# u2seg/U2Seg

Measured on AMD Instinct MI355X. Metric: training images/sec (whole node) u2seg_R50_800 @ 800x1333, higher is better.
Workload: dtype bf16

## Files before the change

include/u2seg_hip.h:

```cpp
#ifndef U2SEG_HIP_H
#define U2SEG_HIP_H

#ifdef __cplusplus
extern "C" {
#endif



#define U2_CV_REG_STAGING (1u << 0)
#define U2_CV_BK32 (1u << 2)
#define U2_CV_TILE_256X128 (1u << 3)
#define U2_CV_RING_SHIFT 4
#define U2_CV_RING_MASK 3
#define U2_CV_WIDE_FORCE (1u << 8)
#define U2_CV_WIDE_FORBID (1u << 9)
#define U2_CV_WIDE_STAGGER (1u << 10)
#define U2_CV_WIDE_STAGGER_PARITY (1u << 11)
#define U2_CV_TILE_CFG_SHIFT 12
#define U2_CV_TILE_CFG_MASK 15
#define U2_CV_TILE_CFG_NEVER 15
#define U2_CV_TINY_GRID (1u << 16)
#define U2_CV_STREAM_FORCE (1u << 17)
#define U2_CV_HALO_TILE128 (1u << 17)
#define U2_CV_ABL_SHIFT 18
// ... 5 lines not shown
#define U2_CV_ABL_NO_STATS_FLUSH (1u << 22)
#define U2_CV_HALO_FORCE (1u << 24)
#define U2_CV_HALO_FORBID (1u << 25)
#define U2_CV_STREAM_FORBID (1u << 26)
#define U2_CV_STREAMK_FORCE (1u << 27)
#define U2_CV_STREAMK_FORBID (1u << 28)
#define U2_CV_HALO_SCHED_SHIFT 29
#define U2_CV_HALO_SCHED_MASK 3
#define U2_CV_EXPLICIT_MASK 0xffffu

#define U2_WG_REG_STAGING (1u << 0)
#define U2_WG_SCALAR_GATHER (1u << 1)
#define U2_WG_FEWER_SPLITS_SHIFT 4
#define U2_WG_FEWER_SPLITS_MASK 3
#define U2_WG_XCD_FORCE (1u << 6)
#define U2_WG_XCD_FORBID (1u << 7)
#define U2_WG_WIDE_FORCE (1u << 8)
#define U2_WG_WIDE_FORBID (1u << 11)
#define U2_WG_RING_SHIFT 9
#define U2_WG_RING_MASK 3
#define U2_WG_HALO_FORCE (1u << 12)
#define U2_WG_HALO_FORBID (1u << 13)
#define U2_WG_HALO_ROUNDS_SHIFT 14
#define U2_WG_HALO_ROUNDS_MASK 3
#define U2_WG_ATOMICS (1u << 16)
#define U2_WG_PARTIALS_FORCE (1u << 17)
#define U2_WG_STREAM_FORCE (1u << 18)
#define U2_WG_STREAM_FORBID (1u << 19)
#define U2_WG_STREAM_TINY (1u << 20)
#define U2_WG_STREAM_CFG_SHIFT 21
#define U2_WG_STREAM_CFG_MASK 7
#define U2_WG_STREAM_PER_CU_SHIFT 24
#define U2_WG_STREAM_PER_CU_MASK 3
#define U2_WG_PER_TAP_MASK_STREAM 0xfffu
#define U2_WG_PER_TAP_MASK_HALO 0x7ffu

#define U2_WD_FORCE (1u << 0)
#define U2_WD_TINY (1u << 1)
#define U2_WD_NEVER (1u << 2)
#define U2_WD_BN_TWO_GROUPS (1u << 3)
#define U2_WD_BN_WIDE (1u << 4)

#define U2_K_TILE 100
#define U2_K_IGEMM256 256
#define U2_K_IGEMM256_STAGGER 1024
#define U2_K_HALO 300
#define U2_K_HALO_N64 301
#define U2_K_STREAMK 500
#define U2_K_STREAM 700
#define U2_K_STREAM_TAIL 5
#define U2_K_IGEMM 1000000
#define U2_K_WGRAD 2000
#define U2_K_WGRAD_XCD 100
#define U2_K_WGRAD256 2256
#define U2_K_WGRAD_STREAM 2700
#define U2_K_WDGRAD 2750
#define U2_K_WDGRAD_BN 2760
#define U2_K_WGRAD_HALO 2900

int u2_conv_igemm(const void* in, const void* wt, void* out, const float* bias, float* stats,
                  int B, int Hin, int Win, int C, int in_ld, int Hout, int Wout, int N, int out_ld,
                  int KH, int KW, int pad_h, int pad_w, int mul, int div, int relu, int accumulate,
                  int variant, void* stream);

int u2_conv_wgrad(const void* x, const void* dy, float* dw, int B, int Hin, int Win, int C, int x_ld,
                  int Hout, int Wout, int N, int dy_ld, int KH, int KW, int pad_h, int pad_w,
                  int stride, int variant, void* stream);
int u2_conv_wgrad_into(const void* x, const void* dy, float* dw, int B, int Hin, int Win, int C, int x_ld,
                       int Hout, int Wout, int N, int dy_ld, int KH, int KW, int pad_h, int pad_w,
                       int stride, int n_valid, int c_valid, long long dw_stride_n, int dw_stride_tap,
                       int dw_stride_c, int variant, void* stream);

int u2_conv1x1_bwd_fused(const void* x, const void* dy, const void* wt, void* dx, float* dw, int M, int C, int x_ld, int N, int dy_ld,
                         int wt_ld, int dx_ld, int n_valid, int c_valid, long long dw_stride_n, int dw_stride_c, int variant,
                         void* stream);

int u2_conv1x1_bwd_fused_bn(const void* x, const void* dz, const void* y, const float* k1, const float* k2, const float* k3,
                            const void* wt, void* dx, float* dw, int M, int C, int x_ld, int N, int dy_ld, int wt_ld, int dx_ld,
                            int n_valid, int c_valid, long long dw_stride_n, int dw_stride_c, int variant, void* stream);

int u2_conv_dgrad_tail(const void* in, const void* wt, const void* dout2, const void* y, const void* bits, const float* mean,
                       const float* invstd, void* dz, float* sums, int B, int H, int W, int C, int in_ld, int N, int out_ld,
                       int variant, void* stream);

int u2_conv_last_kernel(void);

int u2_release_scratch(void);

int u2_weight_layout(const float* w, void* out, int N, int Cin, int T, int Cp, int Npad, int mode, void* stream);
typedef struct U2LayoutDesc {
  long long src_offset;
  void* dst;
  int N, Cin, T, Cp, Npad, mode;
  int block_begin;
  int reserved;
} U2LayoutDesc;
int u2_weight_layout_batched(const float* base, const U2LayoutDesc* table, int n_entries, int total_blocks, void* stream);

int u2_colstats(const void* x, float* out , int slots, int rows_per_slot, int C, int ld, void* stream);
int u2_colstats_ordered(const void* x, float* part, float* out, int slots, int rows_per_slot, int C, int ld, int nchunk,
                        void* stream);
int u2_colsum_add(const void* x, float* dst, int rows, int C, int ld, int n_valid, void* stream);
int u2_gn_finalize_fwd(const float* stats, const float* gamma, const float* beta, float n, float eps, int B, int C, int groups,
                       float* mean, float* invstd, float* scale, float* shift, void* stream);
int u2_gn_finalize_bwd(const float* sums, const float* gamma, const float* mean, const float* invstd, float n, int B, int C,
                       int groups, float* k1, float* k2, float* k3, float* dgamma, float* dbeta, int accumulate, void* stream);
int u2_bn_finalize_fwd(const float* sums, float count, const float* count_dev, const float* gamma, const float* beta, float* running_mean,
                       float* running_var, float momentum, float eps, float* mean, float* invstd, float* scale,
                       float* shift, int C, void* stream);
int u2_affine_act(const void* x, const float* scale, const float* shift, const void* resid, void* out, int slots,
                  int rows_per_slot, int C, int ld, int relu, void* relu_bits, void* stream);
int u2_affine_upadd(const void* x, const float* scale, const float* shift, const void* top, void* out, int B, int H, int W,
                    int C, int relu, void* stream);
int u2_norm_bwd_reduce(const void* dout, const void* mask, const void* x, const float* mean, const float* invstd,
                       float* out , int slots, int rows_per_slot, int C, int ld, int relu,
                       const float* mask_scale, const float* mask_shift, const void* dout2, void* dz_out, const void* dout3,
                       int mask_is_bits, void* stream);
int u2_bn_finalize_bwd(const float* sums, float count, const float* count_dev, const float* gamma, const float* mean, const float* invstd,
                       const float* local_sums, float* dgamma, float* dbeta, float* k1, float* k2, float* k3, int C,
                       int accumulate , void* stream);
int u2_norm_bwd_apply(const void* dout, const void* mask, const void* x, const float* k1, const float* k2,
                      const float* k3, void* dx, void* dres, int slots, int rows_per_slot, int C, int ld, int relu,
                      const float* mask_scale, const float* mask_shift, void* stream);
int u2_bn_act_fused(const void* x, const float* sums, float count, const float* count_dev, const float* gamma, const float* beta,
                    float* running_mean, float* running_var, float momentum, float eps, float* mean, float* invstd, float* scale,
                    float* shift, const void* resid, void* out, int rows, int C, int ld, int relu, void* relu_bits, void* stream);
int u2_bn_bwd_apply_fused(const float* sums, float count, const float* count_dev, const float* gamma, const float* mean,
                          const float* invstd, const float* local_sums, float* dgamma, float* dbeta, float* k123, int accumulate,
                          const void* dout, const void* mask, const void* x, void* dx, void* dres, int rows, int C, int ld,
                          int relu, const float* mask_scale, const float* mask_shift, void* stream);
typedef struct {
  float* running_mean;
  float* running_var;
  int offset;
  int channels;
  int stride;
  int reserved;
} U2PreciseBnLayer;
int u2_bn_precise_update(const U2PreciseBnLayer* table, int n_layers, double* acc, double* tot, int total_channels, int n, int h,
                         int w, void* stream);
int u2_bn_precise_finalize(const U2PreciseBnLayer* table, int n_layers, const double* acc, const double* tot, int total_channels,
                           void* stream);
int u2_relu_bwd(const void* dout, const void* out, void* dz, long long numel, void* stream);
int u2_relu_bwd_colsum(const void* dout, const void* out, void* dz, float* dst, const float* zeros, int rows, int C, int ld, int n_valid,
                       void* stream);
int u2_add_n(const void* a, const void* b, const void* c, const void* d, void* out, long long numel, void* stream);

int u2_wgrad_permute_add(const float* scratch, float* grad, int N, int Cin, int T, int Cp, void* stream);

int u2_maxpool3x3s2_fwd(const void* x, void* y, void* idx, int B, int H, int W, int C, void* stream);
int u2_maxpool3x3s2_bwd(const void* dy, const void* idx, void* dx, int B, int H, int W, int C, void* stream);
int u2_affine_relu_maxpool_fwd(const void* x, const float* scale, const float* shift, void* y, void* idx, int B, int H, int W,
                               int C, void* stream);
int u2_affine_relu_maxpool_bwd_reduce(const void* dy, const void* idx, const void* x, const float* mean, const float* invstd,
                                      const float* mask_scale, const float* mask_shift, float* sums, int B, int H, int W, int C,
                                      void* stream);
int u2_affine_relu_maxpool_bwd_apply(const void* dy, const void* idx, const void* x, const float* k1, const float* k2,
                                     const float* k3, const float* mask_scale, const float* mask_shift, void* dx, int B, int H, int W,
                                     int C, void* stream);
int u2_fpn_upsample_add_fwd(const void* lateral, const void* top, void* out, int B, int H, int W, int C, void* stream);
int u2_fpn_upsample_add_bwd(const void* dout, void* dtop, int B, int H, int W, int C, void* stream);
int u2_bilinear_up2_fwd(const void* x, const void* addend , void* out, int B, int H,
                        int W, int C, void* stream);
int u2_bilinear_up2_bwd(const void* dout, void* dx, int B, int H, int W, int C, void* stream);
int u2_stem_im2col(const void* img, int is_uint8, const float* mean, const float* stdv, void* col, int b, int h, int w,
                   int Hpad, int Wpad, int KP, void* stream);
// ... 266 lines not shown
```

u2seg_amd/csrc/common.h:

```cpp
#pragma once
#include <hip/hip_runtime.h>
#include <stdint.h>
#include <atomic>
#include <mutex>

typedef uint16_t bf16_t;
typedef __attribute__((ext_vector_type(8))) short s16x8;
typedef __attribute__((ext_vector_type(4))) short s16x4;
typedef __attribute__((ext_vector_type(4))) float f32x4;

struct PerDeviceOnce {
  std::mutex mu;
  std::atomic<bool> done[64];
  PerDeviceOnce() { for (auto& d : done) d.store(false, std::memory_order_relaxed); }
  struct Guard {
    PerDeviceOnce* o; int d;
    Guard(PerDeviceOnce* o_, int d_) : o(o_), d(d_) {}
    Guard(const Guard&) = delete;
    Guard& operator=(const Guard&) = delete;
    explicit operator bool() const { return o != nullptr; }
    ~Guard() {
      if (!o) return;
      if (d >= 0) o->done[d].store(true, std::memory_order_release);
      o->mu.unlock();
// ... 41 lines not shown
}
__device__ __forceinline__ int wave_isum(int v) {
#pragma unroll
  for (int o = 32; o > 0; o >>= 1) v += __shfl_xor(v, o, 64);
  return v;
}
__device__ __forceinline__ int wave_imin(int v) {
#pragma unroll
  for (int o = 32; o > 0; o >>= 1) v = min(v, __shfl_xor(v, o, 64));
  return v;
}
__device__ __forceinline__ int wave_imax(int v) {
#pragma unroll
  for (int o = 32; o > 0; o >>= 1) v = max(v, __shfl_xor(v, o, 64));
  return v;
}

template <int CTRL> __device__ __forceinline__ float dpp_mov(float v) {
  return __int_as_float(__builtin_amdgcn_update_dpp(0, __float_as_int(v), CTRL, 0xf, 0xf, true));
}
__device__ __forceinline__ float row16_transpose_sum(float (&v)[16], int fr) {
  {
    const bool up = fr & 8;
#pragma unroll
    for (int k = 0; k < 8; ++k) {
      const float keep = up ? v[k + 8] : v[k], send = up ? v[k] : v[k + 8];
      v[k] = keep + dpp_mov<0x128>(send);
    }
  }
  {
    const bool up = fr & 4;
#pragma unroll
    for (int k = 0; k < 4; ++k) {
      const float keep = up ? v[k + 4] : v[k], send = up ? v[k] : v[k + 4];
      v[k] = keep + dpp_mov<0x141>(send);
    }
  }
  {
    const bool up = fr & 2;
#pragma unroll
    for (int k = 0; k < 2; ++k) {
      const float keep = up ? v[k + 2] : v[k], send = up ? v[k] : v[k + 2];
      v[k] = keep + dpp_mov<0x4E>(send);
    }
  }
  const bool up = fr & 1;
  const float keep = up ? v[1] : v[0], send = up ? v[0] : v[1];
  return keep + dpp_mov<0xB1>(send);
}

__device__ __forceinline__ float block_sum_256(float v, float* red) {
  v = wave_sum(v);
  __syncthreads();
  if ((threadIdx.x & 63) == 0) red[threadIdx.x >> 6] = v;
  __syncthreads();
  return red[0] + red[1] + red[2] + red[3];
}

template <int NW>
__device__ __forceinline__ void wg_flush_column_sums(float* stats, int N, int st_n, float st_s, float st_ss, int w, int lane,
                                                     unsigned char* smem) {
  __syncthreads();
  int* rn = reinterpret_cast<int*>(smem);
  float* rs = reinterpret_cast<float*>(smem) + NW * 64;
  float* rq = rs + NW * 64;
  rn[w * 64 + lane] = st_n;
  rs[w * 64 + lane] = st_s;
  rq[w * 64 + lane] = st_ss;
  __syncthreads();
  bool lead = st_n >= 0 && st_n < N;
  float s = 0.f, q = 0.f;
#pragma unroll
  for (int k = 0; k < NW; ++k) {
    const bool same = rn[k * 64 + lane] == st_n;
    if (same && k < w) lead = false;
    s += same ? rs[k * 64 + lane] : 0.f;
    q += same ? rq[k * 64 + lane] : 0.f;
  }
  if (lead) {
    atomicAdd(stats + st_n, s);
    atomicAdd(stats + N + st_n, q);
  }
}


__device__ __forceinline__ int xcd_remap(int bid, int nwg) {
  const int q = nwg >> 3, r = nwg & 7;
  const int xcd = bid & 7, idx = bid >> 3;
  const int base = (xcd < r) ? xcd * (q + 1) : r * (q + 1) + (xcd - r) * q;
  return base + idx;
}

struct BilinearTap {
  int i0, i1;
  float h, l;
};
__device__ __forceinline__ BilinearTap bilinear_tap(float scale, int o, int n_in) {
  const float s = fmaxf(scale * ((float)o + 0.5f) - 0.5f, 0.f);
  BilinearTap t;
  t.i0 = min((int)s, n_in - 1);
  t.i1 = t.i0 + (t.i0 < n_in - 1 ? 1 : 0);
  t.l = s - (float)t.i0;
  t.h = 1.f - t.l;
  return t;
}
__device__ __forceinline__ float bilinear_mix(const BilinearTap& y, const BilinearTap& x, float v00, float v01, float v10, float v11) {
  return y.h * (x.h * v00 + x.l * v01) + y.l * (x.h * v10 + x.l * v11);
}

#define U2_CHECK_LAUNCH() do { hipError_t e__ = hipGetLastError(); if (e__ != hipSuccess) return (int)e__; } while (0)

__global__ static void u2_fill_words_kernel(unsigned* __restrict__ p, size_t n, unsigned v) {
  for (size_t i = (size_t)blockIdx.x * blockDim.x + threadIdx.x; i < n; i += (size_t)gridDim.x * blockDim.x) p[i] = v;
}
static inline void u2_fill_words(void* p, size_t nwords, unsigned v, hipStream_t s) {
  if (nwords == 0) return;
  size_t g = (nwords + 255) / 256;
  if (g > 1024) g = 1024;
  hipLaunchKernelGGL(u2_fill_words_kernel, dim3((unsigned)g), dim3(256), 0, s, (unsigned*)p, nwords, v);
}
static inline void u2_zero_words(void* p, size_t nwords, hipStream_t s) { u2_fill_words(p, nwords, 0u, s); }
```

u2seg_amd/csrc/conv_args.h:

```cpp
#pragma once
#include "common.h"
#include "conv_variant.h"

namespace u2conv {

struct ConvArgs {
  const bf16_t* in;
  const bf16_t* wt;
  bf16_t* out;
  const float* bias;
  float* stats;
  const bf16_t* zero;
  int B, Hin, Win, C, in_ld;
  int Hout, Wout, N, out_ld;
  int mul;
  int relu, accumulate;
  int M, tiles_m, tiles_n;
  int ntaps, wt_taps;
  int KW, pad_h, pad_w;
  short tap_dy[64], tap_dx[64], tap_w[64];
  int tap_pk[64];
  int remap_out, Hfull, Wfull, out_sy, out_sx, out_y0, out_x0;
  int stagger_by_parity;
  float* sk_ws;
  int* sk_flags;
  int abl;
};


template <int BK> __device__ __forceinline__ int swz(int row);
template <> __device__ __forceinline__ int swz<64>(int row) { return row & 7; }
template <> __device__ __forceinline__ int swz<32>(int row) { return (-(row >> 2)) & 3; }

__device__ __forceinline__ void glds16(const bf16_t* src, void* lds_dst_wave_base) {
  __builtin_amdgcn_global_load_lds(U2_GLB_PTR(src), U2_LDS_PTR(lds_dst_wave_base), 16, 0, 0);
}

template <int RB> __device__ __forceinline__ int tr_swz(int pix) {
  if constexpr (RB >= 256) return ((pix & 3) << 1) | (pix & 8);
  else if constexpr (RB == 128) return (((pix >> 1) & 1) | (((pix >> 3) & 1) << 1)) << 1;
  else return ((pix >> 3) & 1) << 1;
}

template <int IMM = 0> __device__ __forceinline__ unsigned long long tr_read(unsigned addr) {
  unsigned long long r;
  asm volatile("ds_read_b64_tr_b16 %0, %1 offset:%2" : "=v"(r) : "v"(addr), "n"(IMM) : "memory");
  return r;
}
union Frag {
  unsigned long long u[2];
  s16x8 v;
};

extern int g_last_conv_kernel;

int launch_conv_tile(ConvArgs& a, int N, int C, const ConvVariant& v, hipStream_t s);

int launch_conv_halo(ConvArgs& a, int N, int C, const ConvVariant& v, hipStream_t s);

int launch_conv_stream(ConvArgs& a, int N, int C, const ConvVariant& v, hipStream_t s);

struct TailArgs {
  const bf16_t* g2 = nullptr;
  const bf16_t* y = nullptr;
  const unsigned char* bits = nullptr;
  const float* mean = nullptr;
  const float* invstd = nullptr;
};
int launch_conv_stream_tail(ConvArgs& a, const TailArgs& t, int N, int C, const ConvVariant& v, hipStream_t s);

int launch_wgrad_halo(const bf16_t* x, const bf16_t* dy, float* dw, long long dw_sn, int dw_st, int dw_sc, int n_valid,
                      int c_valid, const bf16_t* zero, int B, int H, int W, int C, int x_ld, int N, int dy_ld, int rounds,
                      int force, int part_mode, hipStream_t s);

int launch_wgrad_stream(const bf16_t* x, const bf16_t* dy, float* dw, long long dw_sn, int dw_sc, int n_valid, int c_valid,
                        const bf16_t* zero, int M, int C, int x_ld, int N, int dy_ld, int force, int tiny, int cfg, int per_cu,
                        hipStream_t s);

int launch_wdgrad_stream(const bf16_t* x, const bf16_t* dy, const bf16_t* wt, bf16_t* dx, float* dw, long long dw_sn, int dw_sc,
                         int n_valid, int c_valid, const bf16_t* zero, int M, int C, int x_ld, int N, int dy_ld, int wt_ld,
                         int dx_ld, const FusedBwdVariant& v, hipStream_t s, const bf16_t* yn = nullptr, const float* k1 = nullptr,
                         const float* k2 = nullptr, const float* k3 = nullptr);

void* scratch_get(int kind, hipStream_t s, size_t need_bytes, size_t limit_bytes, bool zero_on_alloc);

}
```

u2seg_amd/csrc/conv_halo.hip:

```cpp
#include <stdlib.h>
#include <type_traits>

#include "common.h"
#include "conv_args.h"

namespace u2conv {
namespace {

constexpr int HBUF = 49152;
constexpr int HPIECES = 6;
constexpr int WR = 7, WA = WR - 1;
constexpr int TN = 128, WSLOT = TN * 64;
constexpr int WBASE = 2 * HBUF;
constexpr int LDS_BYTES = WBASE + WR * WSLOT;

template <int PH, int PWD, int OPT = 3, int CW = 2>
__global__ __launch_bounds__(512, 2) void conv_halo_kernel(const ConvArgs a) {
  constexpr int HPITCH = PWD + 4;
  constexpr int FPR = PWD / 16;
  constexpr int PXW = 8 / CW;
  constexpr int RPW = PH / PXW;
  constexpr int NPF = RPW * FPR;
  constexpr int TNC = CW * 64;
  static_assert(PH * PWD == 512 && (PH + 2) * HPITCH <= 768 && RPW * PXW == PH && (NPF == 8 || NPF == 4), "unsupported patch");
// ... 228 lines not shown
      const int hd = (slab_g & 1) ? -HBUF : HBUF;                                                                        \
      pbase[0] += hd; pbase[1] += hd; pbase[2] += hd;                                                                    \
    }                                                                                                                    \
    if (g + 1 < G) {                                                                                                     \
      wfA[0] = ldw(nslot, 0); wfA[1] = ldw(nslot, 1);                                                                    \
      _Pragma("unroll") for (int j = 0; j < NPF / 2; ++j) pf[j] = U2_H_LDP(((T) + 1) % 9, j);                            \
    }                                                                                                                    \
    if constexpr (!(OPT & 2)) __builtin_amdgcn_sched_barrier(0);                                                                                   \
    if constexpr (!(OPT & 1)) __builtin_amdgcn_s_setprio(1);                                                                                       \
    _Pragma("unroll") for (int j = NPF / 2; j < NPF; ++j) { U2_H_MFMA(2, wfB[0], j); U2_H_MFMA(3, wfB[1], j); }          \
    if constexpr (!(OPT & 1)) __builtin_amdgcn_s_setprio(0);                                                                                       \
    ++g;                                                                                                                 \
    slot = nslot;                                                                                                        \
  }

  for (int ti = 0; ti < my_tiles; ++ti) {
#pragma unroll
    for (int i = 0; i < 4; ++i)
#pragma unroll
      for (int j = 0; j < NPF; ++j) acc[i][j] = f32x4{0.f, 0.f, 0.f, 0.f};
    for (int s = 0; s < nslab; ++s) {
      tail = slab_g + 2 >= total_slabs;
      U2_H_STEP(0, 7)
      U2_H_STEP(1, 7)
      U2_H_STEP(2, 8)
      U2_H_STEP(3, 9)
      U2_H_STEP(4, 10)
      U2_H_STEP(5, 10)
      U2_H_STEP(6, 9)
      U2_H_STEP(7, 8)
      U2_H_STEP(8, 4)
      ++slab_g;
    }
    epilogue(first_tile + ti * stride);
  }
  if (a.stats) wg_flush_column_sums<8>(a.stats, a.N, st_base < 0 ? -1 : st_base + fg * 8 + (fr >> 3) * 32 + (fr & 7), st_s, st_ss, w, lane, smem);
#undef U2_H_STEP
#undef U2_H_LDP
#undef U2_H_MFMA
}

template <int PH, int PWD, int OPT = 3, int CW = 2>
int launch_halo_cfg(ConvArgs& a, int N, int tiny, hipStream_t s) {
  const long long patches = (long long)a.B * ((a.Hout + PH - 1) / PH) * ((a.Wout + PWD - 1) / PWD);
  a.tiles_m = (int)patches;
  a.tiles_n = (N + CW * 64 - 1) / (CW * 64);
  const long long T = patches * a.tiles_n;
  if (T >= (1 << 30)) return 0;
  long long G = T < (tiny ? 8 : 256) ? T : (tiny ? 8 : 256);
  G = (G + 7) & ~7LL;
  static PerDeviceOnce attr_set;
  if (auto once_guard = attr_set.first()) {
    (void)hipFuncSetAttribute((const void*)conv_halo_kernel<PH, PWD, OPT, CW>, hipFuncAttributeMaxDynamicSharedMemorySize, 160 * 1024);
  }
  hipLaunchKernelGGL((conv_halo_kernel<PH, PWD, OPT, CW>), dim3((unsigned)G), dim3(512), LDS_BYTES, s, a);
  hipError_t e = hipGetLastError();
  if (e != hipSuccess) return -1000 - (int)e;
  return 1;
}

double patch_fill(int H, int W, int ph, int pw) {
  return (double)H * W / ((double)((H + ph - 1) / ph * ph) * ((W + pw - 1) / pw * pw));
}

}

int launch_conv_halo(ConvArgs& a, int N, int C, const ConvVariant& v, hipStream_t s) {
  if (v.halo == Choice::Never) return 0;
  if (v.tile_cfg != 0) return 0;
  const bool forced = v.halo == Choice::Force;
  if (a.remap_out || a.accumulate || a.ntaps != 9 || a.KW != 3 || a.wt_taps != 9 || a.pad_h != 1 || a.pad_w != 1 || a.mul != 1 ||
      a.Hin != a.Hout || a.Win != a.Wout)
    return 0;
  if ((C & 31) || (N & 7) || (a.out_ld & 7) || a.M < 1) return 0;
  if ((unsigned long long)a.B * a.Hin * a.Win * a.in_ld * 2ull >= 0xffffffffull || (unsigned long long)N * 9 * C * 2ull >= 0xfffffff0ull)
    return 0;
  const double fill = patch_fill(a.Hout, a.Wout, 16, 32);
  if (!forced) {
    const int tnc = N <= 64 ? 64 : TN;
    const long long tiles = (long long)a.B * ((a.Hout + 15) / 16) * ((a.Wout + 31) / 32) * ((N + tnc - 1) / tnc);
    if (tiles < 512) return 0;
    if (!(fill >= 0.88 || (N <= 128 && fill >= 0.70))) return 0;
  }
  const int tiny = v.tiny;
  if (N <= 64 && !v.halo_tile128) {
    g_last_conv_kernel = U2_K_HALO_N64;
    return launch_halo_cfg<16, 32, 3, 1>(a, N, tiny, s);
  }
  g_last_conv_kernel = U2_K_HALO;
  switch (v.halo_sched) {
    case 1: return launch_halo_cfg<16, 32, 2>(a, N, tiny, s);
    case 2: return launch_halo_cfg<16, 32, 1>(a, N, tiny, s);
    case 3: return launch_halo_cfg<16, 32, 0>(a, N, tiny, s);
    default: return launch_halo_cfg<16, 32, 3>(a, N, tiny, s);
  }
}

}
```

u2seg_amd/csrc/conv_igemm.hip:

```cpp
#include <stdlib.h>
#include <mutex>
#include <vector>

#include "common.h"
#include "conv_args.h"
#include "u2seg_hip.h"

using namespace u2conv;
namespace {

template <int BK, bool GLDS, int TM, int TN, int NST>
__global__ __launch_bounds__((TM / 64) * (TN / 64) * 64, 2) void conv_igemm_kernel(const ConvArgs a) {
  constexpr int NW = (TM / 64) * (TN / 64);
  constexpr int NT = NW * 64;
  constexpr int CPR = BK / 8;
  constexpr int NCHP = (TM * CPR) / NT;
  constexpr int NCHW = (TN * CPR) / NT;
  static_assert(NCHP >= 1 && NCHW >= 1, "tile too small for the thread count");
  constexpr int ROWS_PER_WAVE_INSTR = 64 / CPR;
  constexpr int PTILE_BYTES = TM * BK * 2;
  constexpr int WTILE_BYTES = TN * BK * 2;
  constexpr int STAGE_BYTES = PTILE_BYTES + WTILE_BYTES;
  constexpr int OPITCH = TN + 8;
  constexpr int WM = TM / 64;
  extern __shared__ __attribute__((aligned(16))) unsigned char smem[];

  const int tid = threadIdx.x;
  const int lane = tid & 63;
  const int w = __builtin_amdgcn_readfirstlane(tid >> 6);
  const int nwg = a.tiles_m * a.tiles_n;
  const int tile = xcd_remap(blockIdx.x, nwg);
  const int tile_m = tile / a.tiles_n;
  const int tile_n = tile - tile_m * a.tiles_n;
  const int m0 = tile_m * TM;
  const int n0 = tile_n * TN;

  int p_img[NCHP], p_by[NCHP], p_bx[NCHP];
  bool p_ok[NCHP];
  const bf16_t* w_row[NCHW];
  int cc;
  {
    const int row_in_instr = lane / CPR;
    const int slot = lane % CPR;
    cc = slot ^ swz<BK>(row_in_instr);
    const int hw = a.Hout * a.Wout;
#pragma unroll
    for (int i = 0; i < NCHP; ++i) {
      const int row = (i * NW + w) * ROWS_PER_WAVE_INSTR + row_in_instr;
      const int m = m0 + row;
      p_ok[i] = m < a.M;
      const int mm = p_ok[i] ? m : 0;
      const int img = mm / hw;
      const int rem = mm - img * hw;
      const int oy = rem / a.Wout;
      const int ox = rem - oy * a.Wout;
      p_img[i] = img;
      p_by[i] = oy * a.mul;
      p_bx[i] = ox * a.mul;
    }
#pragma unroll
    for (int i = 0; i < NCHW; ++i) {
      const int n = n0 + (i * NW + w) * ROWS_PER_WAVE_INSTR + row_in_instr;
      w_row[i] = (n < a.N) ? a.wt + (size_t)n * ((size_t)a.wt_taps * a.C) + cc * 8 : nullptr;
    }
  }

  const int kc_per_tap = a.C / BK;
  const int nk = a.ntaps * kc_per_tap;

  uint4 stage_regs[GLDS ? 1 : NCHP + NCHW];

  const bf16_t* p_src[NCHP];
  int p_inc[NCHP];
  const bf16_t* w_src[NCHW];
#pragma unroll
  for (int i = 0; i < NCHW; ++i) w_src[i] = w_row[i] ? w_row[i] : a.zero;
  int kc_in_tap = 0, tap_cur = 0, reg_kh = 0, reg_kw = 0;

  auto issue = [&](int kt, int buf) {
    (void)kt;
    if (kc_in_tap == 0) {
      int dy, dx, wtap;
      if (a.remap_out) {
        dy = a.tap_dy[tap_cur]; dx = a.tap_dx[tap_cur]; wtap = a.tap_w[tap_cur];
      } else {
        dy = reg_kh - a.pad_h; dx = reg_kw - a.pad_w; wtap = tap_cur;
        if (++reg_kw == a.KW) { reg_kw = 0; ++reg_kh; }
      }
#pragma unroll
      for (int i = 0; i < NCHP; ++i) {
        const int sy = p_by[i] + dy, sx = p_bx[i] + dx;
        const bool ok = p_ok[i] && sy >= 0 && sx >= 0 && sy < a.Hin && sx < a.Win;
        p_src[i] = ok ? a.in + ((size_t)(p_img[i] * a.Hin + sy) * a.Win + sx) * a.in_ld + cc * 8 : a.zero;
        p_inc[i] = ok ? BK : 0;
// ... 83 lines not shown
    for (int kt = 0; kt < nk; ++kt) {
      issue(kt, 0);
      __syncthreads();
      commit(0);
      __syncthreads();
      compute(0);
    }
  }

  __syncthreads();
  bf16_t* otile = reinterpret_cast<bf16_t*>(smem);
  float* red = reinterpret_cast<float*>(smem + TM * OPITCH * 2);
#pragma unroll
  for (int i = 0; i < 4; ++i) {
    const int nl = wr * 64 + i * 16 + fg * 4;
    float b0 = 0.f, b1 = 0.f, b2 = 0.f, b3 = 0.f;
    if (a.bias) {
      const int n = n0 + nl;
      b0 = (n + 0 < a.N) ? a.bias[n + 0] : 0.f;
      b1 = (n + 1 < a.N) ? a.bias[n + 1] : 0.f;
      b2 = (n + 2 < a.N) ? a.bias[n + 2] : 0.f;
      b3 = (n + 3 < a.N) ? a.bias[n + 3] : 0.f;
    }
#pragma unroll
    for (int j = 0; j < 4; ++j) {
      const int ml = wc * 64 + j * 16 + fr;
      float v0 = acc[i][j][0] + b0, v1 = acc[i][j][1] + b1, v2 = acc[i][j][2] + b2, v3 = acc[i][j][3] + b3;
      if (a.relu && !a.accumulate) {
        v0 = fmaxf(v0, 0.f); v1 = fmaxf(v1, 0.f); v2 = fmaxf(v2, 0.f); v3 = fmaxf(v3, 0.f);
      }
      uint2 pk;
      pk.x = (uint32_t)f2bf(v0) | ((uint32_t)f2bf(v1) << 16);
      pk.y = (uint32_t)f2bf(v2) | ((uint32_t)f2bf(v3) << 16);
      *reinterpret_cast<uint2*>(otile + ml * OPITCH + nl) = pk;
    }
  }
  __syncthreads();

  constexpr int CPO = TN / 8;
  constexpr int RPI = NT / CPO;
  const int cchunk = tid % CPO;
  const int rbase = tid / CPO;
  float s[8], ss[8];
#pragma unroll
  for (int e = 0; e < 8; ++e) { s[e] = 0.f; ss[e] = 0.f; }
  const bool vec_ok = ((a.out_ld & 7) == 0) && (n0 + cchunk * 8 + 8 <= a.N);
  const bool nt_out = !a.accumulate && (size_t)a.M * a.out_ld * 2 > ((size_t)160 << 20) && (a.abl & 8);
#pragma unroll
  for (int it = 0; it < TM / RPI; ++it) {
    const int row = it * RPI + rbase;
    const int m = m0 + row;
    if (m >= a.M) continue;
    uint4 v = *reinterpret_cast<const uint4*>(otile + row * OPITCH + cchunk * 8);
    bf16_t e8[8];
    *reinterpret_cast<uint4*>(e8) = v;
    size_t orow = (size_t)m;
    if (a.remap_out) {
      const int hw = a.Hout * a.Wout;
      const int img = m / hw;
      const int rem = m - img * hw;
      const int qy = rem / a.Wout;
      const int qx = rem - qy * a.Wout;
      orow = ((size_t)img * a.Hfull + qy * a.out_sy + a.out_y0) * a.Wfull + qx * a.out_sx + a.out_x0;
    }
    bf16_t* dst = a.out + orow * a.out_ld + n0 + cchunk * 8;
    if (a.accumulate) {
#pragma unroll
      for (int e = 0; e < 8; ++e) {
        if (n0 + cchunk * 8 + e < a.N) {
          float f = bf2f(e8[e]) + bf2f(dst[e]);
          if (a.relu) f = fmaxf(f, 0.f);
          e8[e] = f2bf(f);
        }
      }
    }
    if (a.stats) {
#pragma unroll
      for (int e = 0; e < 8; ++e) {
        const float f = bf2f(e8[e]);
        s[e] += f;
        ss[e] += f * f;
      }
    }
    if (vec_ok) {
      if (nt_out) {
        typedef __attribute__((ext_vector_type(4))) unsigned int u32x4_t;
        const uint4 v = *reinterpret_cast<const uint4*>(e8);
        u32x4_t t = {v.x, v.y, v.z, v.w};
        __builtin_nontemporal_store(t, reinterpret_cast<u32x4_t*>(dst));
      } else {
        *reinterpret_cast<uint4*>(dst) = *reinterpret_cast<const uint4*>(e8);
      }
    } else {
#pragma unroll
      for (int e = 0; e < 8; ++e)
        if (n0 + cchunk * 8 + e < a.N) dst[e] = e8[e];
    }
  }
  if (a.stats) {
#pragma unroll
    for (int e = 0; e < 8; ++e) {
#pragma unroll
      for (int o = CPO; o < 64; o <<= 1) {
        s[e] += __shfl_xor(s[e], o, 64);
        ss[e] += __shfl_xor(ss[e], o, 64);
      }
    }
    if (lane < CPO) {
#pragma unroll
      for (int e = 0; e < 8; ++e) {
        red[(0 * NW + w) * TN + lane * 8 + e] = s[e];
        red[(1 * NW + w) * TN + lane * 8 + e] = ss[e];
      }
    }
    __syncthreads();
    if (tid < TN && n0 + tid < a.N) {
      float t0 = 0.f, t1 = 0.f;
#pragma unroll
      for (int ww = 0; ww < NW; ++ww) {
        t0 += red[(0 * NW + ww) * TN + tid];
        t1 += red[(1 * NW + ww) * TN + tid];
      }
      atomicAdd(a.stats + n0 + tid, t0);
      atomicAdd(a.stats + a.N + n0 + tid, t1);
    }
  }
}

constexpr int C256_THREADS = 512;
constexpr int C256_HALF_BYTES = 256 * 64;
constexpr int C256_BUF_BYTES = 2 * C256_HALF_BYTES;
constexpr int C256_OPITCH = 256 + 8;
constexpr int C256_LDS_BYTES = 256 * C256_OPITCH * 2 + 2 * 8 * 256 * 4;
static_assert(C256_LDS_BYTES >= 4 * C256_BUF_BYTES, "ring must fit in the epilogue allocation");

template <bool STAGGER>
__global__ __launch_bounds__(C256_THREADS, 2) void conv_igemm256_kernel(const ConvArgs a) {
  extern __shared__ __attribute__((aligned(16))) unsigned char smem[];
  const int tid = threadIdx.x;
  const int lane = tid & 63;
  const int w = __builtin_amdgcn_readfirstlane(tid >> 6);
  const int nwg = a.tiles_m * a.tiles_n;
  const int tile = xcd_remap(blockIdx.x, nwg);
  const int tile_m = tile / a.tiles_n;
  const int tile_n = tile - tile_m * a.tiles_n;
  const int m0 = tile_m * 256;
  const int n0 = tile_n * 256;

  int p_img[2], p_by[2], p_bx[2];
  bool p_ok[2];
  const bf16_t* w_src[2];
  int w_inc[2];
  const int row_in = lane >> 2;
  const int cc = (lane & 3) ^ swz<32>(row_in);
  {
    const int hw = a.Hout * a.Wout;
#pragma unroll
    for (int i = 0; i < 2; ++i) {
      const int row = (i * 8 + w) * 16 + row_in;
      const int m = m0 + row;
      p_ok[i] = m < a.M;
      const int mm = p_ok[i] ? m : 0;
      const int img = mm / hw;
      const int rem = mm - img * hw;
      const int oy = rem / a.Wout;
      p_img[i] = img;
      p_by[i] = oy * a.mul;
      p_bx[i] = (rem - oy * a.Wout) * a.mul;
      const int n = n0 + row;
      w_src[i] = (n < a.N) ? a.wt + (size_t)n * ((size_t)a.wt_taps * a.C) + cc * 8 : a.zero;
      w_inc[i] = (n < a.N) ? 32 : 0;
    }
  }
  const int kh_per_tap = a.C >> 5;
  const int nkh = a.ntaps * kh_per_tap;
  const bf16_t* p_src[2];
  int p_inc[2];
  int kc_in_tap = 0, reg_kh = 0, reg_kw = 0;
  auto stage_pixels = [&](int hb) {
    if (kc_in_tap == 0) {
      const int dy = reg_kh - a.pad_h, dx = reg_kw - a.pad_w;
      if (++reg_kw == a.KW) { reg_kw = 0; ++reg_kh; }
#pragma unroll
      for (int i = 0; i < 2; ++i) {
        const int sy = p_by[i] + dy, sx = p_bx[i] + dx;
        const bool ok = p_ok[i] && sy >= 0 && sx >= 0 && sy < a.Hin && sx < a.Win;
        p_src[i] = ok ? a.in + ((size_t)(p_img[i] * a.Hin + sy) * a.Win + sx) * a.in_ld + cc * 8 : a.zero;
        p_inc[i] = ok ? 32 : 0;
      }
    }
    if (++kc_in_tap == kh_per_tap) kc_in_tap = 0;
    unsigned char* pbase = smem + hb * C256_BUF_BYTES;
#pragma unroll
    for (int i = 0; i < 2; ++i) {
      glds16(p_src[i], pbase + (i * 8 + w) * 1024);
      p_src[i] += p_inc[i];
    }
  };
  auto stage_weights = [&](int hb) {
    unsigned char* wbase = smem + hb * C256_BUF_BYTES + C256_HALF_BYTES;
#pragma unroll
    for (int i = 0; i < 2; ++i) {
      glds16(w_src[i], wbase + (i * 8 + w) * 1024);
      w_src[i] += w_inc[i];
    }
  };

// ... 699 lines not shown
int g_scratch_used = 0;
std::mutex g_scratch_mu;
struct RetiredEnt { int device; void* buf; };
std::vector<RetiredEnt> g_retired;
}

void* scratch_get(int kind, hipStream_t s, size_t need_bytes, size_t limit_bytes, bool zero_on_alloc) {
  if (need_bytes == 0 || need_bytes > limit_bytes) return nullptr;
  int dev = 0;
  if (hipGetDevice(&dev) != hipSuccess) return nullptr;
  std::lock_guard<std::mutex> lock(g_scratch_mu);
  ScratchEnt* e = nullptr;
  for (int i = 0; i < g_scratch_used; ++i)
    if (g_scratch[i].device == dev && g_scratch[i].stream == s && g_scratch[i].kind == kind) { e = &g_scratch[i]; break; }
  if (e && e->cap >= need_bytes) return e->buf;
  if (!e) {
    if (g_scratch_used == 128) return nullptr;
    e = &g_scratch[g_scratch_used];
    *e = ScratchEnt{dev, s, kind, nullptr, 0};
  }
  size_t cap = need_bytes > e->cap + e->cap / 2 ? need_bytes : e->cap + e->cap / 2;
  cap = (cap + ((size_t)2 << 20) - 1) & ~(((size_t)2 << 20) - 1);
  if (cap > limit_bytes) cap = limit_bytes;
  if (e->buf) {
    g_retired.push_back(RetiredEnt{dev, e->buf});
    e->buf = nullptr; e->cap = 0;
  }
  void* p = nullptr;
  if (hipMalloc(&p, cap) != hipSuccess) return nullptr;
  if (zero_on_alloc && hipMemset(p, 0, cap) != hipSuccess) { (void)hipFree(p); return nullptr; }
  e->buf = p; e->cap = cap;
  if (e == &g_scratch[g_scratch_used]) ++g_scratch_used;
  return p;
}
}

extern "C" int u2_release_scratch(void) {
  int cur = 0;
  (void)hipGetDevice(&cur);
  std::lock_guard<std::mutex> lock(u2conv::g_scratch_mu);
  int freed = 0;
  for (int i = 0; i < u2conv::g_scratch_used; ++i) {
    u2conv::ScratchEnt& e = u2conv::g_scratch[i];
    if (!e.buf) continue;
    (void)hipSetDevice(e.device);
    (void)hipStreamSynchronize(e.stream);
    (void)hipFree(e.buf);
    ++freed;
  }
  u2conv::g_scratch_used = 0;
  for (const u2conv::RetiredEnt& r : u2conv::g_retired) {
    (void)hipSetDevice(r.device);
    (void)hipDeviceSynchronize();
    (void)hipFree(r.buf);
    ++freed;
  }
  u2conv::g_retired.clear();
  (void)hipSetDevice(cur);
  return freed;
}
extern "C" int u2_conv_last_kernel(void) { return u2conv::g_last_conv_kernel; }
namespace {

const bf16_t* zero_page_ptr() {
  static const bf16_t* p = nullptr;
  if (!p) {
    void* q = nullptr;
    if (hipGetSymbolAddress(&q, HIP_SYMBOL(g_zero_page)) != hipSuccess) return nullptr;
    p = reinterpret_cast<const bf16_t*>(q);
  }
  return p;
}

}

namespace {

int env_variant(const char* name, int variant) {
  if (variant != 0) return variant;
  const char* e = getenv(name);
  return e ? (int)strtol(e, nullptr, 0) : 0;
}

int launch_conv(ConvArgs& a, int N, int C, int variant, hipStream_t s) {
  const ConvVariant v = decode_conv_variant((unsigned)env_variant("U2_CONV_VARIANT", variant));
  a.abl = v.abl;
  {
    const int rc = launch_conv_stream(a, N, C, v, s);
    if (rc == 1) return 0;
    if (rc < 0) return rc;
  }
  {
    const int rc = launch_conv_halo(a, N, C, v, s);
    if (rc == 1) return 0;
    if (rc < 0) return rc;
  }
  {
    const int rc = launch_conv_tile(a, N, C, v, s);
    if (rc == 1) return 0;
    if (rc < 0) return rc;
  }
  const bool wide_ok = !a.remap_out && C % 64 == 0 && a.ntaps * (C / 32) >= 4;
  const bool wide_auto = N % 256 == 0 && a.ntaps * C >= 1024 && (long long)a.M * N >= 256LL * 256 * 512;
  if (wide_ok && v.wide != Choice::Never && (v.wide == Choice::Force || wide_auto)) {
    a.tiles_m = (a.M + 255) / 256;
    a.tiles_n = (N + 255) / 256;
    static PerDeviceOnce attr_set;
    if (auto once_guard = attr_set.first()) {
      (void)hipFuncSetAttribute((const void*)conv_igemm256_kernel<false>, hipFuncAttributeMaxDynamicSharedMemorySize, 160 * 1024);
      (void)hipFuncSetAttribute((const void*)conv_igemm256_kernel<true>, hipFuncAttributeMaxDynamicSharedMemorySize, 160 * 1024);
    }
    a.stagger_by_parity = v.wide_stagger_parity ? 1 : 0;
    g_last_conv_kernel = U2_K_IGEMM256 + (v.wide_stagger ? U2_K_IGEMM256_STAGGER : 0);
    if (v.wide_stagger)
      hipLaunchKernelGGL(conv_igemm256_kernel<true>, dim3(a.tiles_m * a.tiles_n), dim3(C256_THREADS), C256_LDS_BYTES, s, a);
    else
      hipLaunchKernelGGL(conv_igemm256_kernel<false>, dim3(a.tiles_m * a.tiles_n), dim3(C256_THREADS), C256_LDS_BYTES, s, a);
    U2_CHECK_LAUNCH();
    return 0;
  }
  const bool narrow = N <= 64;
  const bool big = !narrow && v.tile_256x128;
  const int TM = (narrow || big) ? 256 : 128, TN = narrow ? 64 : 128;
  a.tiles_m = (a.M + TM - 1) / TM;
  a.tiles_n = (N + TN - 1) / TN;
  const dim3 grid(a.tiles_m * a.tiles_n), block(big ? 512 : 256);
  const bool glds = !v.reg_staging;
  const bool shallow = (long long)a.ntaps * C <= 256;
  const int bk = (C % 64 == 0 && !v.bk32 && !shallow) ? 64 : 32;
  int nst = v.ring;
  if (nst == 0) nst = (bk == 64 || shallow) ? 2 : 4;
  else nst += 1;
  if (!glds) nst = 2;
  size_t lds = (size_t)nst * (TM + TN) * bk * 2;
  const size_t epi = (size_t)TM * (TN + 8) * 2 + 2 * 8 * TN * 4;
  if (lds < epi) lds = epi;
  if (lds > 160 * 1024) return -3;
#define U2_LAUNCH_CONV(BK_, GL_, TM_, TN_, NST_)                                                                 \
  do {                                                                                                           \
    g_last_conv_kernel = U2_K_IGEMM + BK_ * 10000 + (TM_ / 64) * 1000 + (TN_ / 64) * 100 + NST_ * 10 + (GL_ ? 1 : 0); \
    static PerDeviceOnce attr_set;                                                                                \
    if (auto once_guard = attr_set.first()) {                                                                                             \
      (void)hipFuncSetAttribute((const void*)conv_igemm_kernel<BK_, GL_, TM_, TN_, NST_>,                        \
                                hipFuncAttributeMaxDynamicSharedMemorySize, 160 * 1024);                         \
    }                                                                                                            \
    hipLaunchKernelGGL((conv_igemm_kernel<BK_, GL_, TM_, TN_, NST_>), grid, block, lds, s, a);                   \
  } while (0)
#define U2_PICK_NST(BK_, TM_, TN_)                                                                               \
  do {                                                                                                           \
    if (!glds) U2_LAUNCH_CONV(BK_, false, TM_, TN_, 2);                                                          \
    else if (nst == 2) U2_LAUNCH_CONV(BK_, true, TM_, TN_, 2);                                                   \
    else if (nst == 3) U2_LAUNCH_CONV(BK_, true, TM_, TN_, 3);                                                   \
    else U2_LAUNCH_CONV(BK_, true, TM_, TN_, 4);                                                                 \
  } while (0)
  if (narrow) {
    if (bk == 64) U2_PICK_NST(64, 256, 64); else U2_PICK_NST(32, 256, 64);
  } else if (big) {
    if (bk == 64) U2_PICK_NST(64, 256, 128); else U2_PICK_NST(32, 256, 128);
  } else {
    if (bk == 64) U2_PICK_NST(64, 128, 128); else U2_PICK_NST(32, 128, 128);
  }
#undef U2_PICK_NST
#undef U2_LAUNCH_CONV
  U2_CHECK_LAUNCH();
  return 0;
}

inline int floor_div(int a, int b) { return (a >= 0) ? a / b : -((-a + b - 1) / b); }

__global__ __launch_bounds__(256) void parity_zero_fill_kernel(bf16_t* __restrict__ out, long long pixels, int H, int W, int ld, int chunks,
                                                               int div, unsigned classes) {
  const long long total = pixels * chunks;
  for (long long i = (long long)blockIdx.x * 256 + threadIdx.x; i < total; i += (long long)gridDim.x * 256) {
    const long long p = i / chunks;
    const int c = (int)(i - p * chunks);
    const int x = (int)(p % W), y = (int)((p / W) % H);
    if ((classes >> ((y % div) * div + (x % div))) & 1u)
      *reinterpret_cast<uint4*>(out + (size_t)p * ld + c * 8) = make_uint4(0u, 0u, 0u, 0u);
  }
}

}

extern "C" int u2_conv_igemm(const void* in, const void* wt, void* out, const float* bias, float* stats,
                             int B, int Hin, int Win, int C, int in_ld, int Hout, int Wout, int N, int out_ld,
                             int KH, int KW, int pad_h, int pad_w, int mul, int div, int relu, int accumulate,
                             int variant, void* stream) {
  if (C % 32 != 0 || (in_ld & 7) != 0 || KH * KW > 64 || (div > 1 && mul != 1)) return -1;
  if (B <= 0 || Hout <= 0 || Wout <= 0 || N <= 0) return 0;
  ConvArgs a;
  a.in = (const bf16_t*)in; a.wt = (const bf16_t*)wt; a.out = (bf16_t*)out; a.bias = bias; a.stats = stats;
  a.zero = zero_page_ptr();
  if (!a.zero) return -2;
  a.abl = 0; a.stagger_by_parity = 0; a.sk_ws = nullptr; a.sk_flags = nullptr;
  a.B = B; a.Hin = Hin; a.Win = Win; a.C = C; a.in_ld = in_ld;
  a.N = N; a.out_ld = out_ld; a.mul = mul; a.relu = relu; a.accumulate = accumulate;
  a.wt_taps = KH * KW;
  a.KW = KW; a.pad_h = pad_h; a.pad_w = pad_w;
  a.Hfull = Hout; a.Wfull = Wout;
  hipStream_t s = (hipStream_t)stream;
  if (div <= 1) {
    a.Hout = Hout; a.Wout = Wout; a.M = B * Hout * Wout;
    a.ntaps = KH * KW;
    for (int kh = 0; kh < KH; ++kh)
      for (int kw = 0; kw < KW; ++kw) {
        const int t = kh * KW + kw;
        a.tap_dy[t] = (short)(kh - pad_h); a.tap_dx[t] = (short)(kw - pad_w); a.tap_w[t] = (short)t;
        a.tap_pk[t] = ((kh - pad_h) & 0xff) | (((kw - pad_w) & 0xff) << 8) | (t << 16);
      }
    a.remap_out = 0; a.out_sy = a.out_sx = 1; a.out_y0 = a.out_x0 = 0;
    return launch_conv(a, N, C, variant, s);
  }
  unsigned empty = 0;
  if (!bias && !stats && !accumulate && div * div <= 32 && (N & 7) == 0) {
    for (int py = 0; py < div; ++py)
      for (int px = 0; px < div; ++px) {
        bool any = false;
        for (int kh = 0; kh < KH && !any; ++kh)
          for (int kw = 0; kw < KW && !any; ++kw)
            any = ((((py - pad_h + kh) % div) + div) % div) == 0 && ((((px - pad_w + kw) % div) + div) % div) == 0;
        if (!any && py < Hout && px < Wout) empty |= 1u << (py * div + px);
      }
    if (empty) {
      const long long pixels = (long long)B * Hout * Wout;
      long long g = (pixels * (N / 8) + 255) / 256;
      if (g > 256 * 32) g = 256 * 32;
      hipLaunchKernelGGL(parity_zero_fill_kernel, dim3((unsigned)g), dim3(256), 0, s, a.out, pixels, Hout, Wout, out_ld, N / 8, div, empty);
      U2_CHECK_LAUNCH();
    }
  }
  for (int py = 0; py < div; ++py)
    for (int px = 0; px < div; ++px) {
      if ((empty >> (py * div + px)) & 1u) continue;
      const int Hq = (Hout - py + div - 1) / div, Wq = (Wout - px + div - 1) / div;
      if (Hq <= 0 || Wq <= 0) continue;
      int nt = 0;
      for (int kh = 0; kh < KH; ++kh) {
        const int vy = py - pad_h + kh;
        if (((vy % div) + div) % div) continue;
        for (int kw = 0; kw < KW; ++kw) {
          const int vx = px - pad_w + kw;
          if (((vx % div) + div) % div) continue;
          a.tap_dy[nt] = (short)floor_div(vy, div); a.tap_dx[nt] = (short)floor_div(vx, div);
          a.tap_w[nt] = (short)(kh * KW + kw);
          a.tap_pk[nt] = (a.tap_dy[nt] & 0xff) | ((a.tap_dx[nt] & 0xff) << 8) | ((kh * KW + kw) << 16);
          ++nt;
        }
      }
      a.ntaps = nt;
      a.Hout = Hq; a.Wout = Wq; a.M = B * Hq * Wq;
      a.remap_out = 1; a.out_sy = a.out_sx = div; a.out_y0 = py; a.out_x0 = px;
      const int rc = launch_conv(a, N, C, variant, s);
      if (rc) return rc;
    }
  return 0;
}

extern "C" int u2_conv_dgrad_tail(const void* in, const void* wt, const void* dout2, const void* y, const void* bits,
                                  const float* mean, const float* invstd, void* dz, float* sums, int B, int H, int W, int C,
                                  int in_ld, int N, int out_ld, int variant, void* stream) {
  if (B <= 0 || H <= 0 || W <= 0 || N <= 0 || C <= 0) return 1;
  ConvArgs a;
  a.in = (const bf16_t*)in; a.wt = (const bf16_t*)wt; a.out = (bf16_t*)dz; a.bias = nullptr; a.stats = sums;
  a.zero = zero_page_ptr();
  if (!a.zero) return -2;
  a.abl = 0; a.stagger_by_parity = 0; a.sk_ws = nullptr; a.sk_flags = nullptr;
  a.B = B; a.Hin = H; a.Win = W; a.C = C; a.in_ld = in_ld;
  a.N = N; a.out_ld = out_ld; a.mul = 1; a.relu = 0; a.accumulate = 0;
  a.wt_taps = 1; a.ntaps = 1;
  a.KW = 1; a.pad_h = 0; a.pad_w = 0;
  a.Hfull = H; a.Wfull = W; a.Hout = H; a.Wout = W; a.M = B * H * W;
  a.tap_dy[0] = a.tap_dx[0] = a.tap_w[0] = 0; a.tap_pk[0] = 0;
  a.remap_out = 0; a.out_sy = a.out_sx = 1; a.out_y0 = a.out_x0 = 0;
  TailArgs t;
  t.g2 = (const bf16_t*)dout2; t.y = (const bf16_t*)y; t.bits = (const unsigned char*)bits; t.mean = mean; t.invstd = invstd;
  const int rc = launch_conv_stream_tail(a, t, N, C, decode_conv_variant((unsigned)env_variant("U2_CONV_VARIANT", variant)),
                                         (hipStream_t)stream);
  if (rc == 1) return 0;
  return rc < 0 ? rc : 1;
}

extern "C" int u2_conv1x1_bwd_fused(const void* x, const void* dy, const void* wt, void* dx, float* dw, int M, int C, int x_ld,
                                    int N, int dy_ld, int wt_ld, int dx_ld, int n_valid, int c_valid, long long dw_stride_n,
                                    int dw_stride_c, int variant, void* stream) {
  if (n_valid > N || c_valid > C) return -1;
  const bf16_t* zero = zero_page_ptr();
  if (!zero) return -2;
  if (M <= 0) return 0;
  const FusedBwdVariant v = decode_fused_bwd_variant((unsigned)env_variant("U2_WDGRAD_VARIANT", variant));
  if (v.never) return 1;
  const int rc = launch_wdgrad_stream((const bf16_t*)x, (const bf16_t*)dy, (const bf16_t*)wt, (bf16_t*)dx, dw, dw_stride_n,
                                      dw_stride_c, n_valid, c_valid, zero, M, C, x_ld, N, dy_ld, wt_ld, dx_ld, v,
                                      (hipStream_t)stream);
  if (rc == 1) return 0;
  return rc < 0 ? rc : 1;
}

extern "C" int u2_conv1x1_bwd_fused_bn(const void* x, const void* dz, const void* y, const float* k1, const float* k2,
                                       const float* k3, const void* wt, void* dx, float* dw, int M, int C, int x_ld, int N, int dy_ld,
                                       int wt_ld, int dx_ld, int n_valid, int c_valid, long long dw_stride_n, int dw_stride_c,
                                       int variant, void* stream) {
  if (n_valid > N || c_valid > C || !y || !k1 || !k2 || !k3) return -1;
  const bf16_t* zero = zero_page_ptr();
  if (!zero) return -2;
  if (M <= 0) return 0;
  const FusedBwdVariant v = decode_fused_bwd_variant((unsigned)env_variant("U2_WDGRAD_VARIANT", variant));
  if (v.never) return 1;
  const int rc = launch_wdgrad_stream((const bf16_t*)x, (const bf16_t*)dz, (const bf16_t*)wt, (bf16_t*)dx, dw, dw_stride_n,
                                      dw_stride_c, n_valid, c_valid, zero, M, C, x_ld, N, dy_ld, wt_ld, dx_ld, v,
                                      (hipStream_t)stream, (const bf16_t*)y, k1, k2, k3);
  if (rc == 1) return 0;
  return rc < 0 ? rc : 1;
}

extern "C" int u2_conv_wgrad(const void* x, const void* dy, float* dw, int B, int Hin, int Win, int C, int x_ld,
                             int Hout, int Wout, int N, int dy_ld, int KH, int KW, int pad_h, int pad_w,
                             int stride, int variant, void* stream) {
  return u2_conv_wgrad_into(x, dy, dw, B, Hin, Win, C, x_ld, Hout, Wout, N, dy_ld, KH, KW, pad_h, pad_w, stride, N, C,
                            (long long)KH * KW * C, C, 1, variant, stream);
}

extern "C" int u2_conv_wgrad_into(const void* x, const void* dy, float* dw, int B, int Hin, int Win, int C, int x_ld,
                                  int Hout, int Wout, int N, int dy_ld, int KH, int KW, int pad_h, int pad_w,
                                  int stride, int n_valid, int c_valid, long long dw_stride_n, int dw_stride_tap,
                                  int dw_stride_c, int variant, void* stream) {
  if ((C & 7) != 0 || (x_ld & 7) != 0 || (dy_ld & 7) != 0 || (N & 7) != 0) return -1;
  if (n_valid > N || c_valid > C) return -1;
  if (B <= 0 || Hout <= 0 || Wout <= 0) return 0;
  WgradArgs a;
  a.x = (const bf16_t*)x; a.dy = (const bf16_t*)dy; a.dw = dw; a.zero = zero_page_ptr();
  if (!a.zero) return -2;
  a.dw_sn = dw_stride_n; a.dw_st = dw_stride_tap; a.dw_sc = dw_stride_c; a.n_valid = n_valid; a.c_valid = c_valid;
  a.B = B; a.Hin = Hin; a.Win = Win; a.C = C; a.x_ld = x_ld;
  a.Hout = Hout; a.Wout = Wout; a.N = N; a.dy_ld = dy_ld;
  a.KH = KH; a.KW = KW; a.pad_h = pad_h; a.pad_w = pad_w; a.stride = stride;
  a.M = B * Hout * Wout;
  const WgradVariant v = decode_wgrad_variant((unsigned)env_variant("U2_WGRAD_VARIANT", variant));
  if (KH * KW == 1 && stride == 1 && pad_h == 0 && pad_w == 0 && Hin == Hout && Win == Wout && v.stream != Choice::Never &&
      !v.per_tap_stream) {
    const int rc = launch_wgrad_stream(a.x, a.dy, dw, dw_stride_n, dw_stride_c, n_valid, c_valid, a.zero, a.M, C, x_ld, N, dy_ld,
                                       v.stream == Choice::Force, v.stream_tiny, v.stream_cfg, v.stream_per_cu,
                                       (hipStream_t)stream);
    if (rc == 1) return 0;
    if (rc < 0) return rc;
  }
  const bool halo_ok = KH == 3 && KW == 3 && stride == 1 && pad_h == 1 && pad_w == 1 && Hin == Hout && Win == Wout;
// ... 75 lines not shown
```

u2seg_amd/csrc/conv_stream.hip:

```cpp
#include <stdlib.h>

#include "common.h"
#include "conv_args.h"

namespace u2conv {
namespace {

template <int RB> __device__ __forceinline__ int row_swz(int row) {
  if constexpr (RB == 64) return swz<32>(row);
  else if constexpr (RB == 128) return (row >> 1) & 7;
  else return row & 15;
}

template <int NF, int RB, int J = 0> __device__ __forceinline__ void lds_read_frags(s16x8 (&pf)[NF], unsigned addr) {
  if constexpr (J < NF) {
    asm volatile("ds_read_b128 %0, %1 offset:%2" : "=v"(pf[J]) : "v"(addr), "n"(J * 16 * RB) : "memory");
    lds_read_frags<NF, RB, J + 1>(pf, addr);
  }
}
template <int CNT, int NF> __device__ __forceinline__ void lds_wait_frags(s16x8 (&pf)[NF]) {
  asm volatile("s_waitcnt lgkmcnt(%0)" ::"n"(CNT) : "memory");
#pragma unroll
  for (int j = 0; j < NF; ++j) asm volatile("" : "+v"(pf[j])::"memory");
}

template <int E> __device__ __forceinline__ float row_bcast(float v) {
  return __int_as_float(__builtin_amdgcn_update_dpp(0, __float_as_int(v), 0x150 + E, 0xf, 0xf, true));
}

__device__ __forceinline__ f32x2_t row_bcast_pair(float v, int e) {
  switch (e) {
    case 0: return f32x2_t{row_bcast<0>(v), row_bcast<1>(v)};
    case 1: return f32x2_t{row_bcast<2>(v), row_bcast<3>(v)};
    case 2: return f32x2_t{row_bcast<4>(v), row_bcast<5>(v)};
    case 3: return f32x2_t{row_bcast<6>(v), row_bcast<7>(v)};
    case 4: return f32x2_t{row_bcast<8>(v), row_bcast<9>(v)};
    case 5: return f32x2_t{row_bcast<10>(v), row_bcast<11>(v)};
    case 6: return f32x2_t{row_bcast<12>(v), row_bcast<13>(v)};
    default: return f32x2_t{row_bcast<14>(v), row_bcast<15>(v)};
  }
}

typedef __attribute__((ext_vector_type(4))) unsigned int u32x4_t;
typedef __attribute__((ext_vector_type(2))) unsigned int u32x2_t;
struct TailRow {
  u32x4_t ga, gb, ya, yb;
  u32x2_t mk;
};

template <int KS, int TM, int PSW, int NWV, int KSS = KS, bool TAIL = false>
__global__ __launch_bounds__(NWV * 64, 2) void conv_stream_kernel(const ConvArgs a, int ring, const TailArgs t) {
  constexpr int RB = KSS * 64, CPR = KSS * 4, STAGE = TM * RB;
  constexpr int RPP = 16 / KSS;
  constexpr int PT = TM * KSS / 16;
  constexpr int PPW = PT / NWV;
  constexpr int S = KS / KSS;
  constexpr int CBW = NWV / PSW, WPX = TM / PSW, NF = WPX / 16;
  static_assert(PT % NWV == 0 && PPW >= 1 && PPW <= 8 && NF >= 1 && (KSS == 1 || KSS == 2 || KSS == 4 || KSS == 8) && KS % KSS == 0 && (S & (S - 1)) == 0, "unsupported configuration");
  static_assert(!TAIL || (S == 1 && NF % 2 == 0), "the tail epilogue takes whole tiles per step and batches of 1, 2 or 4 rows");
  extern __shared__ __attribute__((aligned(16))) unsigned char smem[];
  const int tid = threadIdx.x, lane = tid & 63;
  const int w = __builtin_amdgcn_readfirstlane(tid >> 6);
  const int cbw = w % CBW, psw = w / CBW;
  const int fr = lane & 15, fg = lane >> 4;

  const int TP = a.tiles_m, tiles_n = a.tiles_n;
  const int xcd = blockIdx.x & 7, idx = blockIdx.x >> 3, gx = gridDim.x >> 3;
  const int q8 = TP >> 3, r8 = TP & 7;
  const int xbase = (xcd < r8) ? xcd * (q8 + 1) : r8 * (q8 + 1) + (xcd - r8) * q8;
  const int xcnt = q8 + (xcd < r8 ? 1 : 0);
  const int nwalk = gx / tiles_n;
  const int nt = idx % tiles_n, walker = idx / tiles_n;
  if (walker >= nwalk || walker >= xcnt) return;
  const int my_tiles = (xcnt - walker + nwalk - 1) / nwalk;
  const int first_tile = xbase + walker;
  const int n0 = nt * (CBW * 64) + cbw * 64;

  s16x8 wr[KS][4];
#pragma unroll
  for (int i = 0; i < 4; ++i) {
    const int n = n0 + (i >> 1) * 32 + (fr >> 2) * 8 + (i & 1) * 4 + (fr & 3);
    const bf16_t* src = a.wt + (size_t)(n < a.N ? n : 0) * a.C + fg * 8;
#pragma unroll
    for (int ks = 0; ks < KS; ++ks) {
      s16x8 v = *reinterpret_cast<const s16x8*>(src + ks * 32);
      if (n >= a.N) v = s16x8{0, 0, 0, 0, 0, 0, 0, 0};
      wr[ks][i] = v;
    }
  }
  float t_mu = 0.f, t_is = 0.f;
  if constexpr (TAIL) {
    const int tn = n0 + fg * 8 + (fr >> 3) * 32 + (fr & 7);
    t_mu = t.mean[tn];
    t_is = t.invstd[tn];
  }
  asm volatile("s_waitcnt vmcnt(0)" ::: "memory");
  if constexpr (TAIL) asm volatile("" : "+v"(t_mu), "+v"(t_is));
#pragma unroll
  for (int ks = 0; ks < KS; ++ks)
#pragma unroll
    for (int i = 0; i < 4; ++i) asm volatile("" : "+v"(wr[ks][i]));

  unsigned d_off[PPW];
  int d_row[PPW];
#pragma unroll
  for (int q = 0; q < PPW; ++q) {
    const int row = (q * NWV + w) * RPP + lane / CPR;
    const int pos = lane % CPR;
    const int chunk = (pos & ~15) | ((pos ^ row_swz<RB>(row)) & (CPR < 16 ? CPR - 1 : 15));
    d_row[q] = row;
    d_off[q] = (unsigned)(((size_t)row * a.in_ld + chunk * 8) * 2);
  }
  const unsigned char* in_bytes = reinterpret_cast<const unsigned char*>(a.in);
  auto issue = [&](int g, int slot) {
    const int ti = g / S, st = g % S;
    const int m0 = (first_tile + ti * nwalk) * TM;
    const unsigned char* tbase = in_bytes + (size_t)m0 * a.in_ld * 2 + st * RB;
#pragma unroll
    for (int q = 0; q < PPW; ++q) {
      const unsigned char* src = (m0 + d_row[q] < a.M) ? tbase + d_off[q] : reinterpret_cast<const unsigned char*>(a.zero);
      glds16(reinterpret_cast<const bf16_t*>(src), smem + slot * STAGE + (q * NWV + w) * 1024);
    }
  };

  const unsigned lds0 = (unsigned)(size_t)U2_LDS_PTR(smem);
  const int pfrag0 = (psw * WPX + fr) * RB;
  const int pchunk0 = fg ^ row_swz<RB>(fr);

  f32x4 acc[4][NF];
  float st_s = 0.f, st_ss = 0.f;
  const int st_n = n0 + fg * 8 + (fr >> 3) * 32 + (fr & 7);

  const int nslice = n0;
  const int nb = nslice + fg * 8;
  const bool okA = nb < a.N, okB = nb + 32 < a.N;
  f32x4 bia[4] = {f32x4{0.f, 0.f, 0.f, 0.f}, f32x4{0.f, 0.f, 0.f, 0.f}, f32x4{0.f, 0.f, 0.f, 0.f}, f32x4{0.f, 0.f, 0.f, 0.f}};
  if (a.bias) {
    if (okA)
      asm volatile("global_load_dwordx4 %0, %2, off\n\tglobal_load_dwordx4 %1, %2, off offset:16\n\ts_waitcnt vmcnt(0)"
                   : "=&v"(bia[0]), "=&v"(bia[1]) : "v"(a.bias + nb) : "memory");
    if (okB)
      asm volatile("global_load_dwordx4 %0, %2, off\n\tglobal_load_dwordx4 %1, %2, off offset:16\n\ts_waitcnt vmcnt(0)"
// ... 46 lines not shown
  constexpr bool EARLY = NF <= 4;
  constexpr int TR = NF >= 8 ? 4 : NF >= 4 ? 2 : 1;
  TailRow tr[TR];
  auto tail_issue = [&](int ti, int b) {
    const int m0 = (first_tile + ti * nwalk) * TM + psw * WPX;
#pragma unroll
    for (int r = 0; r < TR; ++r) {
      int m = m0 + (TR * b + r) * 16 + fr;
      m = m < a.M ? m : a.M - 1;
      const unsigned off = ((unsigned)m * (unsigned)a.out_ld + (unsigned)nb) * 2u;
      const unsigned moff = (unsigned)m * (unsigned)(a.N >> 3) + (unsigned)(n0 >> 3);
      asm volatile("global_load_dwordx4 %0, %2, %3\n\tglobal_load_dwordx4 %1, %2, %3 offset:64"
                   : "=&v"(tr[r].ga), "=&v"(tr[r].gb) : "v"(off), "s"(t.g2) : "memory");
      asm volatile("global_load_dwordx4 %0, %2, %3\n\tglobal_load_dwordx4 %1, %2, %3 offset:64"
                   : "=&v"(tr[r].ya), "=&v"(tr[r].yb) : "v"(off), "s"(t.y) : "memory");
      asm volatile("global_load_dwordx2 %0, %1, %2" : "=&v"(tr[r].mk) : "v"(moff), "s"(t.bits) : "memory");
    }
  };
  auto tail_epilogue = [&](int ti, bool step_issued) {
    const int m0 = (first_tile + ti * nwalk) * TM + psw * WPX;
    f32x2_t s2[8], ss2[8];
#pragma unroll
    for (int e = 0; e < 8; ++e) { s2[e] = f32x2_t{0.f, 0.f}; ss2[e] = f32x2_t{0.f, 0.f}; }
    uint32_t g1p[NF][8];
#pragma unroll
    for (int j = 0; j < NF; ++j)
#pragma unroll
      for (int i = 0; i < 4; ++i) {
        g1p[j][2 * i] = pack_bf16(acc[i][j][0], acc[i][j][1]);
        g1p[j][2 * i + 1] = pack_bf16(acc[i][j][2], acc[i][j][3]);
      }
#pragma unroll
    for (int j = 0; j < NF; ++j)
      asm volatile("" : "+v"(g1p[j][0]), "+v"(g1p[j][1]), "+v"(g1p[j][2]), "+v"(g1p[j][3]), "+v"(g1p[j][4]), "+v"(g1p[j][5]),
                        "+v"(g1p[j][6]), "+v"(g1p[j][7]));
#pragma unroll
    for (int b = 0; b < NF / TR; ++b) {
      if (b > 0 || !EARLY) tail_issue(ti, b);
      if (EARLY && b == 0 && !step_issued) wait_vm<0>();
      if (EARLY && b == 0) wait_vm<PPW>();
      else wait_vm<0>();
#pragma unroll
      for (int r = 0; r < TR; ++r)
        asm volatile("" : "+v"(tr[r].ga), "+v"(tr[r].gb), "+v"(tr[r].ya), "+v"(tr[r].yb), "+v"(tr[r].mk)::"memory");
#pragma unroll
      for (int r = 0; r < TR; ++r) {
        const int j = TR * b + r;
        const int m = m0 + j * 16 + fr;
        const bool row_ok = m < a.M;
        const uint32_t bitsA = row_ok ? (tr[r].mk[0] >> (fg * 8)) & 0xffu : 0u;
        const uint32_t bitsB = row_ok ? (tr[r].mk[1] >> (fg * 8)) & 0xffu : 0u;
        uint32_t pk[8];
#pragma unroll
        for (int e = 0; e < 8; ++e) {
          const uint32_t gw = e < 4 ? tr[r].ga[e & 3] : tr[r].gb[e & 3];
          const uint32_t yw = e < 4 ? tr[r].ya[e & 3] : tr[r].yb[e & 3];
          const uint32_t bt = ((e < 4 ? bitsA : bitsB) >> (2 * (e & 3))) & 3u;
          const f32x2_t g1 = {__uint_as_float(g1p[j][e] << 16), __uint_as_float(g1p[j][e] & 0xffff0000u)};
          const f32x2_t g2 = {__uint_as_float(gw << 16), __uint_as_float(gw & 0xffff0000u)};
          const f32x2_t sum = g1 + g2;
          pk[e] = pack_bf16(sum[0], sum[1]) & (((bt & 1u) ? 0xffffu : 0u) | ((bt & 2u) ? 0xffff0000u : 0u));
          const f32x2_t dz = {__uint_as_float(pk[e] << 16), __uint_as_float(pk[e] & 0xffff0000u)};
          const f32x2_t yv = {__uint_as_float(yw << 16), __uint_as_float(yw & 0xffff0000u)};
          const f32x2_t mu = row_bcast_pair(t_mu, e), is = row_bcast_pair(t_is, e);
          s2[e] += dz;
          ss2[e] += dz * (yv - mu) * is;
          asm volatile("" : "+v"(s2[e]), "+v"(ss2[e]), "+v"(t_mu), "+v"(t_is));
        }
        if (row_ok) {
          const unsigned off = ((unsigned)m * (unsigned)a.out_ld + (unsigned)nb) * 2u;
          const u32x4_t va = {pk[0], pk[1], pk[2], pk[3]}, vb = {pk[4], pk[5], pk[6], pk[7]};
          asm volatile("global_store_dwordx4 %0, %1, %2\n\ts_nop 1" ::"v"(off), "v"(va), "s"(a.out) : "memory");
          asm volatile("global_store_dwordx4 %0, %1, %2 offset:64\n\ts_nop 1" ::"v"(off), "v"(vb), "s"(a.out) : "memory");
        }
      }
    }
    float s[16], ss[16];
#pragma unroll
    for (int e = 0; e < 8; ++e) { s[2 * e] = s2[e][0]; s[2 * e + 1] = s2[e][1]; ss[2 * e] = ss2[e][0]; ss[2 * e + 1] = ss2[e][1]; }
    st_s += row16_transpose_sum(s, fr);
    st_ss += row16_transpose_sum(ss, fr);
  };

  const int G = my_tiles * S;
  for (int sl = 0; sl < ring - 1 && sl < G; ++sl) issue(sl, sl);
  int slot = 0, g = 0;
  for (int ti = 0; ti < my_tiles; ++ti) {
#pragma unroll
    for (int i = 0; i < 4; ++i)
#pragma unroll
      for (int j = 0; j < NF; ++j) acc[i][j] = f32x4{0.f, 0.f, 0.f, 0.f};
#pragma unroll
   for (int st = 0; st < S; ++st, ++g) {
    {
      int nd = G - 1 - g;
      if (nd > ring - 2) nd = ring - 2;
      switch (nd) {
        case 0: wait_vm<0>(); break;
        case 1: wait_vm<PPW>(); break;
        case 2: wait_vm<2 * PPW>(); break;
        case 3: wait_vm<3 * PPW>(); break;
        case 4: wait_vm<4 * PPW>(); break;
        case 5: wait_vm<5 * PPW>(); break;
        default: wait_vm<6 * PPW>(); break;
      }
    }
    asm volatile("s_waitcnt lgkmcnt(0)" ::: "memory");
    __builtin_amdgcn_s_barrier();
    asm volatile("" ::: "memory");
    if constexpr (TAIL && EARLY) tail_issue(ti, 0);
    const bool step_issued = g + ring - 1 < G;
    if (step_issued) {
      int s2 = slot - 1;
      if (s2 < 0) s2 += ring;
      issue(g + ring - 1, s2);
    }
    const unsigned char* sb = smem + slot * STAGE + pfrag0;
    constexpr bool DB = NF <= 4 && KSS > 1;
    s16x8 pf[DB ? 2 : 1][NF];
    if constexpr (DB) {
      const unsigned sba = lds0 + (unsigned)(slot * STAGE + pfrag0);
      lds_read_frags<NF, RB>(pf[0], sba + (unsigned)(pchunk0 << 4));
#pragma unroll
      for (int ks = 0; ks < KSS; ++ks) {
        const int cur = ks & 1;
        if (ks + 1 < KSS) {
          lds_read_frags<NF, RB>(pf[cur ^ 1], sba + (unsigned)((((ks + 1) * 4) ^ pchunk0) << 4));
          lds_wait_frags<NF, NF>(pf[cur]);
        } else {
          lds_wait_frags<0, NF>(pf[cur]);
        }
#pragma unroll
        for (int j = 0; j < NF; ++j)
#pragma unroll
          for (int i = 0; i < 4; ++i) acc[i][j] = __builtin_amdgcn_mfma_f32_16x16x32_bf16(wr[st * KSS + ks][i], pf[cur][j], acc[i][j], 0, 0, 0);
      }
    } else {
#pragma unroll
      for (int ks = 0; ks < KSS; ++ks) {
#pragma unroll
        for (int j = 0; j < NF; ++j)
          pf[0][j] = *reinterpret_cast<const s16x8*>(sb + j * 16 * RB + (((ks * 4) ^ pchunk0) << 4));
#pragma unroll
        for (int j = 0; j < NF; ++j)
#pragma unroll
          for (int i = 0; i < 4; ++i) acc[i][j] = __builtin_amdgcn_mfma_f32_16x16x32_bf16(wr[st * KSS + ks][i], pf[0][j], acc[i][j], 0, 0, 0);
      }
    }
    slot = slot + 1 == ring ? 0 : slot + 1;
   }
    if constexpr (TAIL) tail_epilogue(ti, g + ring - 2 < G);
    else if (!(a.abl & 4)) epilogue(ti);
  }
  if (do_stats) wg_flush_column_sums<NWV>(a.stats, a.N, st_n, st_s, st_ss, w, lane, smem);
}

template <int KS, int TM, int PSW, int NWV, int KSS = KS, bool TAIL = false>
int launch_stream_cfg(ConvArgs& a, int N, int tiny, int forced, int code, hipStream_t s, const TailArgs& t = TailArgs{}) {
  constexpr int CBW = NWV / PSW;
  constexpr int STAGE = TM * KSS * 64;
  const int per_cu = NWV == 4 ? 2 : 1;
  const int lds_budget = (per_cu == 2 ? 80 : 160) * 1024;
  int ring = lds_budget / STAGE;
  if (ring > 8) ring = 8;
  if (ring < 2) return 0;
  a.tiles_m = (a.M + TM - 1) / TM;
  a.tiles_n = (N + CBW * 64 - 1) / (CBW * 64);
  long long G = tiny ? 8LL * a.tiles_n : 256LL * per_cu;
  if ((G >> 3) < a.tiles_n) return 0;
  if (!forced && !tiny && (long long)a.tiles_m * a.tiles_n < 6 * G) return 0;
  static PerDeviceOnce attr_set;
  if (auto once_guard = attr_set.first()) {
    (void)hipFuncSetAttribute((const void*)conv_stream_kernel<KS, TM, PSW, NWV, KSS, TAIL>, hipFuncAttributeMaxDynamicSharedMemorySize, 160 * 1024);
  }
  g_last_conv_kernel = code;
  hipLaunchKernelGGL((conv_stream_kernel<KS, TM, PSW, NWV, KSS, TAIL>), dim3((unsigned)G), dim3(NWV * 64), (size_t)ring * STAGE, s, a, ring, t);
  hipError_t e = hipGetLastError();
  if (e != hipSuccess) return -1000 - (int)e;
  return 1;
}

}

static bool stream_allowed(const ConvVariant& v, bool& forced, int& tiny) {
  forced = v.stream == Choice::Force;
  tiny = v.tiny;
  return v.stream != Choice::Never && !v.explicit_kernel;
}

int launch_conv_stream(ConvArgs& a, int N, int C, const ConvVariant& v, hipStream_t s) {
  bool forced;
  int tiny;
  if (!stream_allowed(v, forced, tiny)) return 0;
  if (a.remap_out || a.accumulate || a.ntaps != 1 || a.wt_taps != 1 || a.pad_h != 0 || a.pad_w != 0 || a.mul != 1 ||
      a.Hin != a.Hout || a.Win != a.Wout)
    return 0;
  if (!(C == 32 || C == 64 || C == 128 || C == 256) || (N & 7) || (a.out_ld & 7) || a.in_ld < C || a.M < 1) return 0;
  if ((unsigned long long)a.M * a.in_ld * 2ull >= 0xffffffffull) return 0;
  const int code = U2_K_STREAM + (C / 32) * 10;
  if (C == 64) {
    if (N > 128) return launch_stream_cfg<2, 128, 1, 4>(a, N, tiny, forced, code, s);
    if (N > 64) return launch_stream_cfg<2, 128, 2, 4>(a, N, tiny, forced, code + 1, s);
    return launch_stream_cfg<2, 128, 4, 4>(a, N, tiny, forced, code + 2, s);
  }
  if (C == 256) {
    if (N > 128) return launch_stream_cfg<8, 64, 2, 8>(a, N, tiny, forced, code, s);
    if (N > 64) return launch_stream_cfg<8, 64, 2, 4, 4>(a, N, tiny, forced, code + 1, s);
    return launch_stream_cfg<8, 64, 4, 4, 4>(a, N, tiny, forced, code + 2, s);
  }
  if (C == 128) {
    if (N > 128) return launch_stream_cfg<4, 64, 1, 4>(a, N, tiny, forced, code, s);
    if (N > 64) return launch_stream_cfg<4, 64, 2, 4>(a, N, tiny, forced, code + 1, s);
    return launch_stream_cfg<4, 64, 4, 4>(a, N, tiny, forced, code + 2, s);
  }
  if (N > 128) return launch_stream_cfg<1, 128, 1, 4>(a, N, tiny, forced, code, s);
  if (N > 64) return launch_stream_cfg<1, 128, 2, 4>(a, N, tiny, forced, code + 1, s);
  return launch_stream_cfg<1, 128, 4, 4>(a, N, tiny, forced, code + 2, s);
}


int launch_conv_stream_tail(ConvArgs& a, const TailArgs& t, int N, int C, const ConvVariant& v, hipStream_t s) {
  bool forced;
  int tiny;
  if (!stream_allowed(v, forced, tiny)) return 0;
  if (a.remap_out || a.accumulate || a.relu || a.bias || a.ntaps != 1 || a.wt_taps != 1 || a.pad_h != 0 || a.pad_w != 0 ||
      a.mul != 1 || a.Hin != a.Hout || a.Win != a.Wout)
    return 0;
  if (!((C == 64 && N == 256) || (C == 128 && N == 512) || (C == 256 && N == 1024))) return 0;
  if (a.out_ld != N || a.in_ld < C || (a.in_ld & 7) || a.M < 1) return 0;
  if ((unsigned long long)a.M * a.in_ld * 2ull >= 0xffffffffull || (unsigned long long)a.M * N * 2ull >= 0xffffffffull) return 0;
  if (!a.stats || !a.out || !t.g2 || !t.y || !t.bits || !t.mean || !t.invstd) return 0;
  const int code = U2_K_STREAM + U2_K_STREAM_TAIL + (C / 32) * 10;
  a.abl = 0;
  if (C == 64) return launch_stream_cfg<2, 128, 1, 4, 2, true>(a, N, tiny, forced, code, s, t);
  if (C == 128) return launch_stream_cfg<4, 64, 1, 4, 4, true>(a, N, tiny, forced, code, s, t);
  return launch_stream_cfg<8, 64, 2, 8, 8, true>(a, N, tiny, forced, code, s, t);
}

}
```

u2seg_amd/csrc/conv_tile.hip:

```cpp
#include <stdlib.h>
#include <mutex>
#include <vector>
#include <algorithm>
#include <stdio.h>

#include "common.h"
#include "conv_args.h"

namespace u2conv {
namespace {

#ifdef U2_TILE_TRACE
__device__ unsigned long long* g_tile_trace_dev = nullptr;
#define U2_STAMP(SLOT)                                                                                                        \
  do {                                                                                                                         \
    if (trace_on) {                                                                                                            \
      unsigned long long t_;                                                                                                   \
      asm volatile("s_memtime %0\n\ts_waitcnt lgkmcnt(0)" : "=s"(t_)::"memory");                                              \
      if (lane == 0) asm volatile("global_store_dwordx2 %0, %1, off\n\ts_nop 1" ::"v"(trace_row + (SLOT)), "v"(t_) : "memory"); \
    }                                                                                                                          \
  } while (0)
#ifndef U2_TILE_TRACE_POINT
#define U2_TILE_TRACE_POINT 0
#endif
__device__ unsigned long long* g_tile_sub_dev = nullptr;
#define U2_SUB(KIND)                                                                                                           \
  do {                                                                                                                         \
    if (sub_on && gh < 48) {                                                                                                   \
      unsigned long long t_;                                                                                                   \
      asm volatile("s_memtime %0\n\ts_waitcnt lgkmcnt(0)" : "=s"(t_)::"memory");                                              \
      if (lane == 0) asm volatile("global_store_dwordx2 %0, %1, off\n\ts_nop 1" ::"v"(sub_row + (KIND) * 48 + gh), "v"(t_) : "memory"); \
    }                                                                                                                          \
  } while (0)
#define U2_SUBK(K) do { if constexpr (U2_TILE_TRACE_POINT == (K)) U2_SUB(1); } while (0)
#else
#define U2_STAMP(SLOT) do { } while (0)
#define U2_SUB(KIND) do { } while (0)
#define U2_SUBK(K) do { } while (0)
#endif

__device__ __forceinline__ void divmod_f(int m, int d, float inv, int& q, int& r) {
  q = (int)((float)m * inv);
  r = m - q * d;
  if (r < 0) { --q; r += d; }
  if (r >= d) { ++q; r -= d; }
}

#ifndef U2_TILE_PINGPONG
#define U2_TILE_PINGPONG 0
#endif
template <int WCH, int WPX, int RING, bool ACC = false, bool SK = false, int KT = 1>
__global__ __launch_bounds__(WCH * WPX * 64, 2) void conv_tile_kernel(const ConvArgs a) {
  constexpr int NW = WCH * WPX, NT = NW * 64;
  constexpr int TN = WCH * 64, TM = WPX * 128;
  constexpr int KU = 32 * KT;
  constexpr int ROWB = 64 * KT;
  constexpr int CPRW = ROWB / 16;
  constexpr int RPI = 1024 / ROWB;
  constexpr int LP = TM * CPRW / NT;
  constexpr int LW = TN * CPRW / NT;
  constexpr int LPT = LP + LW;
  constexpr int PBYTES = TM * ROWB, WBYTES = TN * ROWB, BUF = PBYTES + WBYTES;
  constexpr int AHEAD = RING - 1;
  static_assert(LP >= 1 && LW >= 1 && RING >= (KT == 2 ? 2 : 3) && RING <= 5 && (KT == 1 || KT == 2), "unsupported configuration");
  extern __shared__ __attribute__((aligned(16))) unsigned char smem[];

  const int tid = threadIdx.x;
  const int lane = tid & 63;
  const int w = __builtin_amdgcn_readfirstlane(tid >> 6);
#ifdef U2_TILE_TRACE
  const bool trace_on = w == 0 && g_tile_trace_dev != nullptr;
  unsigned long long* trace_row = g_tile_trace_dev + (size_t)blockIdx.x * 64;
  const bool sub_on = U2_TILE_TRACE_POINT != 0 && (w == 0 || w == 4) && g_tile_sub_dev != nullptr;
  unsigned long long* sub_row = g_tile_sub_dev + ((size_t)blockIdx.x * 2 + (w >> 2)) * 96;
  U2_STAMP(0);
#endif

  const int T = a.tiles_m * a.tiles_n;
  const int xcd = blockIdx.x & 7, idx = blockIdx.x >> 3, stride = gridDim.x >> 3;
  const int q8 = T >> 3, r8 = T & 7;
  const int xbase = (xcd < r8) ? xcd * (q8 + 1) : r8 * (q8 + 1) + (xcd - r8) * q8;
  const int xcnt = q8 + (xcd < r8 ? 1 : 0);
  const int kh_per_tap = a.C / KU;
  const int nkh = a.ntaps * kh_per_tap;
  int my_tiles, first_tile, H;
  int sk_k0 = 0, sk_k1 = nkh;
  long long sk_s0 = 0;
  const long long sk_S = (long long)xcnt * nkh;
  if constexpr (SK) {
    sk_s0 = sk_S * idx / stride;
    const long long s1 = sk_S * (idx + 1) / stride;
    if (s1 <= sk_s0) return;
    first_tile = xbase + (int)(sk_s0 / nkh);
    sk_k0 = (int)(sk_s0 % nkh);
    const int last = (int)((s1 - 1) / nkh);
    my_tiles = last - (int)(sk_s0 / nkh) + 1;
    sk_k1 = (int)(s1 - (long long)last * nkh);
    H = (int)(s1 - sk_s0);
  } else {
    if (idx >= xcnt) return;
    my_tiles = (xcnt - idx + stride - 1) / stride;
    first_tile = xbase + idx;
    H = my_tiles * nkh;
  }
  const int tstep = SK ? 1 : stride;

  const int row_in = lane / CPRW;
  const int cc = (lane % CPRW) ^ swz<KU>(row_in);
  const int hw = a.Hout * a.Wout;
  const float inv_hw = 1.0f / (float)hw, inv_w = 1.0f / (float)a.Wout;
  const bool linear = a.ntaps == 1 && a.mul == 1 && a.Hin == a.Hout && a.Win == a.Wout &&
                      (a.remap_out ? ((a.tap_pk[0] & 0xffff) == 0) : (a.pad_h == 0 && a.pad_w == 0));

  unsigned p_center[LP];
  int p_yx[LP];
  const bf16_t* p_src[LP];
  unsigned p_okmask = 0;
  int pt = -1, p_tap = a.ntaps, p_kc = 0, p_kh = 0, p_kw = 0;
  auto setup_pixels = [&](int tile) {
    const int m0 = (tile / a.tiles_n) * TM;
#pragma unroll
    for (int i = 0; i < LP; ++i) {
      const int m = m0 + (i * NW + w) * RPI + row_in;
      if (m < a.M) {
        if (linear) {
          p_center[i] = (unsigned)(((size_t)m * a.in_ld + cc * 8) * 2);
          p_yx[i] = 0;
        } else {
          int img, rem, oy, ox;
          divmod_f(m, hw, inv_hw, img, rem);
          divmod_f(rem, a.Wout, inv_w, oy, ox);
          const int y = oy * a.mul, x = ox * a.mul;
          p_center[i] = (unsigned)((((size_t)(img * a.Hin + y) * a.Win + x) * a.in_ld + cc * 8) * 2);
          p_yx[i] = (y & 0xffff) | (x << 16);
        }
// ... 121 lines not shown
        asm volatile("global_load_dwordx4 %0, %2, off\n\tglobal_load_dwordx4 %1, %2, off offset:16\n\ts_waitcnt vmcnt(0)"
                     : "=&v"(bia[0]), "=&v"(bia[1]) : "v"(a.bias + nb) : "memory");
      if (okB)
        asm volatile("global_load_dwordx4 %0, %2, off\n\tglobal_load_dwordx4 %1, %2, off offset:16\n\ts_waitcnt vmcnt(0)"
                     : "=&v"(bia[2]), "=&v"(bia[3]) : "v"(a.bias + nb + 32) : "memory");
    }
    float s[16], ss[16];
#pragma unroll
    for (int e = 0; e < 16; ++e) { s[e] = 0.f; ss[e] = 0.f; }
    const bool nt_out = (size_t)a.M * a.out_ld * 2 > ((size_t)160 << 20) && (a.abl & 8);
    typedef __attribute__((ext_vector_type(4))) unsigned int u32x4_t;
    u32x4_t olda[4], oldb[4];
#pragma unroll
    for (int j = 0; j < 8; ++j) {
      if constexpr (ACC) {
        if ((j & 3) == 0) {
#pragma unroll
          for (int jj = 0; jj < 4; ++jj) {
            const int mm = m0 + (j + jj) * 16 + fr;
            olda[jj] = u32x4_t{0u, 0u, 0u, 0u};
            oldb[jj] = u32x4_t{0u, 0u, 0u, 0u};
            if (mm < a.M) {
              const bf16_t* src = a.out + (size_t)mm * a.out_ld + nb;
              if (okA) asm volatile("global_load_dwordx4 %0, %1, off" : "=&v"(olda[jj]) : "v"(src) : "memory");
              if (okB) asm volatile("global_load_dwordx4 %0, %1, off offset:64" : "=&v"(oldb[jj]) : "v"(src) : "memory");
            }
          }
          asm volatile("s_waitcnt vmcnt(0)"
                       : "+v"(olda[0]), "+v"(olda[1]), "+v"(olda[2]), "+v"(olda[3]), "+v"(oldb[0]), "+v"(oldb[1]), "+v"(oldb[2]),
                         "+v"(oldb[3])::"memory");
        }
      }
      const int m = m0 + j * 16 + fr;
      if (m < a.M) {
        size_t orow = (size_t)m;
        if (a.remap_out) {
          int img, rem, qy, qx;
          divmod_f(m, hw, inv_hw, img, rem);
          divmod_f(rem, a.Wout, inv_w, qy, qx);
          orow = ((size_t)img * a.Hfull + qy * a.out_sy + a.out_y0) * a.Wfull + qx * a.out_sx + a.out_x0;
        }
        bf16_t* dst = a.out + orow * a.out_ld + nb;
        uint32_t pk[8];
#pragma unroll
        for (int i = 0; i < 4; ++i) {
          float v0 = acc[i][j][0] + bia[i][0], v1 = acc[i][j][1] + bia[i][1];
          float v2 = acc[i][j][2] + bia[i][2], v3 = acc[i][j][3] + bia[i][3];
          if constexpr (ACC) {
            const uint32_t c01 = pack_bf16(v0, v1), c23 = pack_bf16(v2, v3);
            const u32x4_t o = (i < 2) ? olda[j & 3] : oldb[j & 3];
            const uint32_t o01 = o[(i & 1) * 2], o23 = o[(i & 1) * 2 + 1];
            v0 = __uint_as_float(c01 << 16) + __uint_as_float(o01 << 16);
            v1 = __uint_as_float(c01 & 0xffff0000u) + __uint_as_float(o01 & 0xffff0000u);
            v2 = __uint_as_float(c23 << 16) + __uint_as_float(o23 << 16);
            v3 = __uint_as_float(c23 & 0xffff0000u) + __uint_as_float(o23 & 0xffff0000u);
          }
          if (a.relu) { v0 = fmaxf(v0, 0.f); v1 = fmaxf(v1, 0.f); v2 = fmaxf(v2, 0.f); v3 = fmaxf(v3, 0.f); }
          pk[2 * i] = pack_bf16(v0, v1);
          pk[2 * i + 1] = pack_bf16(v2, v3);
        }
        if (!ACC && a.stats) {
#pragma unroll
          for (int e = 0; e < 8; ++e) {
            const float lo = __uint_as_float(pk[e] << 16), hi = __uint_as_float(pk[e] & 0xffff0000u);
            s[2 * e] += lo; ss[2 * e] += lo * lo;
            s[2 * e + 1] += hi; ss[2 * e + 1] += hi * hi;
          }
        }
        const u32x4_t va = {pk[0], pk[1], pk[2], pk[3]}, vb = {pk[4], pk[5], pk[6], pk[7]};
        if (nt_out) {
          if (okA) asm volatile("global_store_dwordx4 %0, %1, off nt\n\ts_nop 1" ::"v"(dst), "v"(va) : "memory");
          if (okB) asm volatile("global_store_dwordx4 %0, %1, off offset:64 nt\n\ts_nop 1" ::"v"(dst), "v"(vb) : "memory");
        } else {
          if (okA) asm volatile("global_store_dwordx4 %0, %1, off\n\ts_nop 1" ::"v"(dst), "v"(va) : "memory");
          if (okB) asm volatile("global_store_dwordx4 %0, %1, off offset:64\n\ts_nop 1" ::"v"(dst), "v"(vb) : "memory");
        }
      }
    }
    if (!ACC && a.stats) {
      const int n_here = tile_n * TN + wr * 64 + fg * 8 + (fr >> 3) * 32 + (fr & 7);
      if (n_here != st_n) { stats_flush(); st_n = n_here; }
      st_s += row16_transpose_sum(s, fr);
      st_ss += row16_transpose_sum(ss, fr);
    }
  };

#define U2_T_MFMA(I, WF, J) acc[I][J] = __builtin_amdgcn_mfma_f32_16x16x32_bf16(WF, pf[J], acc[I][J], 0, 0, 0)

  if constexpr (SK) {
    const int tap0 = sk_k0 / kh_per_tap, skip0 = sk_k0 - tap0 * kh_per_tap;
    pt = 0; wt_i = 0;
    setup_pixels(first_tile);
    setup_weights(first_tile);
    p_tap = tap0; w_tap = tap0;
    p_kh = tap0 / a.KW; p_kw = tap0 - p_kh * a.KW;
    pixel_tap(skip0);
    weight_tap(skip0);
  }
#pragma unroll
  for (int i = 0; i < AHEAD; ++i) { stage_pixels(i); stage_weights(i); }
  stage_pixels(AHEAD);
  wait_vm<LPT * (AHEAD - 1) + LP>();
  __builtin_amdgcn_s_barrier();
  asm volatile("" ::: "memory");
  U2_STAMP(1);
#if U2_TILE_PINGPONG
  if constexpr (KT == 1 && !ACC) {
  } else
#endif
  {
  wfA[0] = ldw(0, 0); wfA[1] = ldw(0, 1);
#pragma unroll
  for (int j = 0; j < 4; ++j) pf[j] = ldp(0, j);
  }

  typedef __attribute__((ext_vector_type(4))) unsigned int sk_u32x4;
  auto sk_publish = [&]() {
    unsigned char* slot = reinterpret_cast<unsigned char*>(a.sk_ws) + (size_t)blockIdx.x * (TM * TN * 4) + (size_t)tid * 16;
#pragma unroll
    for (int i = 0; i < 4; ++i)
#pragma unroll
      for (int j = 0; j < 8; ++j) {
        asm volatile("global_store_dwordx4 %0, %1, off sc0 sc1\n\ts_nop 1" ::"v"(slot), "v"(acc[i][j]) : "memory");
        slot += NT * 16;
        asm volatile("" : "+v"(slot));
      }
    asm volatile("s_waitcnt vmcnt(0)" ::: "memory");
    __builtin_amdgcn_s_barrier();
    if (tid == 0) {
      const int one = 1;
      asm volatile("global_store_dword %0, %1, off sc0 sc1\n\ts_nop 1" ::"v"(a.sk_flags + blockIdx.x), "v"(one) : "memory");
    }
  };
  constexpr int SKB = 16;
  static_assert(SKB == 16, "the counted waits of sk_combine are written for four groups of four loads");
  auto sk_combine = [&](int tile) {
    const long long tile_end = (long long)(tile - xbase + 1) * nkh;
    for (int j = idx + 1; j < stride && sk_S * j / stride < tile_end; ++j) {
      const int peer = j * 8 + xcd;
      if (tid == 0) {
        int f;
        do {
          asm volatile("global_load_dword %0, %1, off sc0 sc1\n\ts_waitcnt vmcnt(0)" : "=&v"(f) : "v"(a.sk_flags + peer) : "memory");
          if (f == 0) __builtin_amdgcn_s_sleep(8);
        } while (f == 0);
        const int zero = 0;
        asm volatile("global_store_dword %0, %1, off sc0 sc1\n\ts_nop 1" ::"v"(a.sk_flags + peer), "v"(zero) : "memory");
      }
      __builtin_amdgcn_s_barrier();
      asm volatile("" ::: "memory");
      U2_STAMP(51);
      const unsigned char* slot = reinterpret_cast<const unsigned char*>(a.sk_ws) + (size_t)peer * (TM * TN * 4) + (size_t)tid * 16;
      {
#pragma unroll
        for (int q = 0; q < 32 / SKB; ++q) {
          f32x4 t[SKB];
#pragma unroll
          for (int jj = 0; jj < SKB; ++jj) {
            asm volatile("global_load_dwordx4 %0, %1, off sc0 sc1" : "=&v"(t[jj]) : "v"(slot) : "memory");
            slot += NT * 16;
            asm volatile("" : "+v"(slot));
          }
#pragma unroll
          for (int g = 0; g < SKB / 4; ++g) {
            if (g == 0) asm volatile("s_waitcnt vmcnt(12)" : "+v"(t[g * 4]), "+v"(t[g * 4 + 1]), "+v"(t[g * 4 + 2]), "+v"(t[g * 4 + 3])::"memory");
            else if (g == 1) asm volatile("s_waitcnt vmcnt(8)" : "+v"(t[g * 4]), "+v"(t[g * 4 + 1]), "+v"(t[g * 4 + 2]), "+v"(t[g * 4 + 3])::"memory");
// ... 112 lines not shown
      __builtin_amdgcn_s_setprio(1);                                                                                                        \
      _Pragma("unroll") for (int j = 0; j < 8; ++j) { U2_T_MFMA(0, wfA[0], j); U2_T_MFMA(1, wfA[1], j); }                        \
      __builtin_amdgcn_s_setprio(0)
#define U2_PP_MB()                                                                                                               \
      __builtin_amdgcn_s_setprio(1);                                                                                                        \
      _Pragma("unroll") for (int j = 0; j < 8; ++j) { U2_T_MFMA(2, wfB[0], j); U2_T_MFMA(3, wfB[1], j); }                        \
      __builtin_amdgcn_s_setprio(0)
      if (cold) {
        U2_T_RD(wfA[0], wa, 0); U2_T_RD(wfA[1], wa, 16 * ROWB);
        U2_T_RD(pf[0], pa, 0); U2_T_RD(pf[1], pa, 16 * ROWB); U2_T_RD(pf[2], pa, 2 * 16 * ROWB); U2_T_RD(pf[3], pa, 3 * 16 * ROWB);
        U2_T_RD(pf[4], pa, 4 * 16 * ROWB); U2_T_RD(pf[5], pa, 5 * 16 * ROWB); U2_T_RD(pf[6], pa, 6 * 16 * ROWB); U2_T_RD(pf[7], pa, 7 * 16 * ROWB);
        if (gh + AHEAD < H) stage_weights(sb);
      }
      __builtin_amdgcn_sched_barrier(0);
      U2_SUBK(11);
      U2_PP_WAIT10();
      U2_SUBK(12);
      U2_PP_MA();
      __builtin_amdgcn_sched_barrier(0);
      U2_SUBK(13);
      if (!cold) {
        if (gh + AHEAD < H) stage_weights(sb);
      }
      if (!grp_x) { U2_T_RD(wfB[0], wa, 2 * 16 * ROWB); U2_T_RD(wfB[1], wa, 3 * 16 * ROWB); }
      __builtin_amdgcn_sched_barrier(0);
      U2_SUBK(14);
      {
        const int rem = H - 2 - gh;
        if (rem >= AHEAD - 1) wait_vm<LPT * (AHEAD - 1)>();
        else if (AHEAD > 3 && rem == 2) wait_vm<LPT * 2>();
        else if (rem == 1) wait_vm<LPT>();
        else wait_vm<0>();
      }
      asm volatile("s_waitcnt lgkmcnt(0)" ::: "memory");
      __builtin_amdgcn_s_barrier();
      asm volatile("" ::: "memory");
#ifdef U2_TILE_TRACE
      if (gh < 44) U2_STAMP(2 + gh);
      U2_SUB(0);
#endif
      if (grp_x) {
        U2_T_RD(wfB[0], wa, 2 * 16 * ROWB); U2_T_RD(wfB[1], wa, 3 * 16 * ROWB);
        if (gh + AHEAD + 1 < H) stage_pixels(hb);
      }
      __builtin_amdgcn_sched_barrier(0);
      U2_SUBK(15);
      asm volatile("s_waitcnt lgkmcnt(0)" : "+v"(wfB[0]), "+v"(wfB[1])::"memory");
      U2_SUBK(16);
      U2_PP_MB();
      __builtin_amdgcn_sched_barrier(0);
      U2_SUBK(17);
      if (!grp_x) {
        if (gh + AHEAD + 1 < H) stage_pixels(hb);
        if (!last_of_tile && gh + 1 < H) {
          const unsigned pn = lds_base + (unsigned)(nb * BUF + pfrag0), wn = lds_base + (unsigned)(nb * BUF + wfrag0);
          U2_T_RD(wfA[0], wn, 0); U2_T_RD(wfA[1], wn, 16 * ROWB);
          U2_T_RD(pf[0], pn, 0); U2_T_RD(pf[1], pn, 16 * ROWB); U2_T_RD(pf[2], pn, 2 * 16 * ROWB); U2_T_RD(pf[3], pn, 3 * 16 * ROWB);
          U2_T_RD(pf[4], pn, 4 * 16 * ROWB); U2_T_RD(pf[5], pn, 5 * 16 * ROWB); U2_T_RD(pf[6], pn, 6 * 16 * ROWB); U2_T_RD(pf[7], pn, 7 * 16 * ROWB);
        }
      }
      U2_SUBK(18);
      __builtin_amdgcn_s_barrier();
      asm volatile("" ::: "memory");
#undef U2_PP_WAIT10
#undef U2_PP_MA
#undef U2_PP_MB
      ++gh;
      hb = nb;
    };
#endif
    int h = h_begin;
#if U2_TILE_PINGPONG
    if constexpr (KT == 1 && !ACC) {
      for (; h < h_end; ++h) step_pp(h == h_begin, h + 1 == h_end);
    } else
#endif
    {
    for (; h < h_end; ++h) step();
    }
    if constexpr (SK) {
      if (h_begin > 0) { U2_STAMP(48); sk_publish(); U2_STAMP(49); continue; }
      if (h_end < nkh) break;
    }
    epilogue(first_tile + ti * tstep);
  }
  if constexpr (SK) {
    if (sk_k1 < nkh && !(my_tiles == 1 && sk_k0 > 0)) {
      U2_STAMP(50);
      sk_combine(first_tile + my_tiles - 1);
      U2_STAMP(52);
      epilogue(first_tile + my_tiles - 1);
      U2_STAMP(53);
    }
  }
  if (!ACC && a.stats) wg_flush_column_sums<NW>(a.stats, a.N, st_n, st_s, st_ss, w, lane, smem);
  U2_STAMP(54);
#undef U2_T_MFMA
}

constexpr int SK_MAX_GROUPS = 512;
constexpr size_t SK_WS_LIMIT = (size_t)64 << 20;
bool sk_scratch(hipStream_t s, ConvArgs& a, size_t need_bytes) {
  float* ws = (float*)scratch_get(0, s, need_bytes, SK_WS_LIMIT, false);
  if (!ws) return false;
  int* flags = (int*)scratch_get(1, s, SK_MAX_GROUPS * sizeof(int), (size_t)2 << 20, true);
  if (!flags) return false;
  a.sk_ws = ws; a.sk_flags = flags;
  return true;
}

#ifdef U2_TILE_TRACE
unsigned long long* g_tile_trace_host_ptr = nullptr;
unsigned long long* g_tile_sub_host_ptr = nullptr;
int g_tile_trace_launch = 0;
void tile_trace_begin(int G, hipStream_t s) {
  (void)G;
  if (!g_tile_trace_host_ptr) {
    if (hipMalloc(&g_tile_trace_host_ptr, 1024 * 64 * 8) != hipSuccess) return;
    (void)hipMemcpyToSymbol(HIP_SYMBOL(g_tile_trace_dev), &g_tile_trace_host_ptr, sizeof(void*));
  }
  (void)hipMemsetAsync(g_tile_trace_host_ptr, 0, 1024 * 64 * 8, s);
#if U2_TILE_TRACE_POINT
  if (!g_tile_sub_host_ptr) {
    if (hipMalloc(&g_tile_sub_host_ptr, 1024 * 2 * 96 * 8) != hipSuccess) return;
    (void)hipMemcpyToSymbol(HIP_SYMBOL(g_tile_sub_dev), &g_tile_sub_host_ptr, sizeof(void*));
  }
  (void)hipMemsetAsync(g_tile_sub_host_ptr, 0, 1024 * 2 * 96 * 8, s);
#endif
}
void tile_trace_end(int G, hipStream_t s, const char* what) {
  static const int every = getenv("U2_TILE_TRACE_EVERY") ? atoi(getenv("U2_TILE_TRACE_EVERY")) : 4;
  if (!g_tile_trace_host_ptr || (++g_tile_trace_launch % every) != 0 || G > 1024) return;
  (void)hipStreamSynchronize(s);
  static unsigned long long h[1024 * 64];
  if (hipMemcpy(h, g_tile_trace_host_ptr, (size_t)G * 64 * 8, hipMemcpyDeviceToHost) != hipSuccess) return;
#if U2_TILE_TRACE_POINT
  {
    static unsigned long long sb[1024 * 2 * 96];
    if (hipMemcpy(sb, g_tile_sub_host_ptr, (size_t)G * 2 * 96 * 8, hipMemcpyDeviceToHost) == hipSuccess) {
      const int picks[] = {1, 9, G / 2 + 1, G - 15};
      for (int pi = 0; pi < 4; ++pi) {
        const int g = picks[pi];
        if (g < 0 || g >= G) continue;
        for (int wv = 0; wv < 2; ++wv) {
          const unsigned long long* r = sb + ((size_t)g * 2 + wv) * 96;
          double step = 0, off = 0; int ns = 0, no = 0;
          for (int k = 6; k < 30; ++k) {
            if (r[k] && r[k + 1]) { step += (double)(r[k + 1] - r[k]); ++ns; }
            const int ref = ((U2_TILE_TRACE_POINT >= 3 && U2_TILE_TRACE_POINT <= 6) || (U2_TILE_TRACE_POINT >= 11 && U2_TILE_TRACE_POINT <= 14)) ? k - 1 : k;
            if (r[48 + k] && r[ref] && r[48 + k] > r[ref]) { off += (double)(r[48 + k] - r[ref]); ++no; }
          }
          const unsigned long long* r0 = sb + ((size_t)g * 2) * 96;
          fprintf(stderr, "SUB point %d wg %4d wave %d: step %.0f cycles (n=%d), point at +%.0f cycles behind the %s barrier (n=%d), barrier of wave 4 - wave 0 at step 10: %lld\n",
                  U2_TILE_TRACE_POINT, g, wv * 4, ns ? step / ns : -1.0, ns, no ? off / no : -1.0, ((U2_TILE_TRACE_POINT >= 3 && U2_TILE_TRACE_POINT <= 6) || (U2_TILE_TRACE_POINT >= 11 && U2_TILE_TRACE_POINT <= 14)) ? "previous" : "same", no,
                  (long long)(r0[96 + 10]) - (long long)(r0[10]));
        }
      }
    }
  }
#endif
  static const double tick_us = getenv("U2_TILE_TRACE_TICK_US") ? atof(getenv("U2_TILE_TRACE_TICK_US")) : 0.01;
  unsigned long long t0 = ~0ull, t1 = 0;
  for (int g = 0; g < G; ++g) {
    if (h[g * 64] && h[g * 64] < t0) t0 = h[g * 64];
    for (int k = 0; k < 64; ++k) if (h[g * 64 + k] > t1) t1 = h[g * 64 + k];
  }
  fprintf(stderr, "TRACE launch %d (%s, %d work-groups): first entry -> last stamp %.2f us (%llu ticks of %.4f us)\n", g_tile_trace_launch, what, G, (t1 - t0) * tick_us, t1 - t0, tick_us);
  auto us = [&](int g, int k) { return h[g * 64 + k] ? (double)(h[g * 64 + k] - t0) * tick_us : -1.0; };
  const int picks[] = {0, 1, 8, 9, 64, 65, 128, G / 2 + 1, G - 16, G - 8, G - 1};
  for (int pi = 0; pi < (int)(sizeof(picks) / sizeof(int)); ++pi) {
    const int g = picks[pi];
    if (g < 0 || g >= G) continue;
    int steps = 0;
    double first_step = -1, last_step = -1;
    for (int k = 2; k < 46; ++k)
      if (h[g * 64 + k]) { ++steps; if (first_step < 0) first_step = us(g, k); last_step = us(g, k); }
    fprintf(stderr, "  wg %4d: entry %6.2f  first stage %6.2f  K barriers %2d (%6.2f .. %6.2f, %.3f us/step)  publish %6.2f .. %6.2f  loop done %6.2f  flag %6.2f  combined %6.2f  epilogue %6.2f  end %6.2f\n",
            g, us(g, 0), us(g, 1), steps, first_step, last_step, steps > 1 ? (last_step - first_step) / (steps - 1) : 0.0, us(g, 48), us(g, 49),
            us(g, 50), us(g, 51), us(g, 52), us(g, 53), us(g, 54));
  }
  const int g = G / 2 + 1 < G ? G / 2 + 1 : 0;
  fprintf(stderr, "  wg %4d step gaps (us):", g);
  for (int k = 3; k < 46; ++k)
    if (h[g * 64 + k] && h[g * 64 + k - 1]) fprintf(stderr, " %.2f", (double)(h[g * 64 + k] - h[g * 64 + k - 1]) * tick_us);
  fprintf(stderr, "\n");
  std::vector<double> d_entry, d_first, d_step, d_pub, d_comb, d_epi, d_end;
  for (int w = 0; w < G; ++w) {
    if (!h[w * 64]) continue;
    d_entry.push_back(us(w, 0));
    if (h[w * 64 + 1]) d_first.push_back(us(w, 1) - us(w, 0));
    int steps = 0; double fs = -1, ls = -1;
    for (int k = 2; k < 46; ++k) if (h[w * 64 + k]) { ++steps; if (fs < 0) fs = us(w, k); ls = us(w, k); }
    if (steps > 1) d_step.push_back((ls - fs) / (steps - 1));
    if (h[w * 64 + 48] && h[w * 64 + 49]) d_pub.push_back(us(w, 49) - us(w, 48));
    if (h[w * 64 + 50] && h[w * 64 + 52]) d_comb.push_back(us(w, 52) - us(w, 50));
    if (h[w * 64 + 52] && h[w * 64 + 53]) d_epi.push_back(us(w, 53) - us(w, 52));
    if (h[w * 64 + 54]) d_end.push_back(us(w, 54));
  }
  auto med = [](std::vector<double>& v) { if (v.empty()) return -1.0; std::sort(v.begin(), v.end()); return v[v.size() / 2]; };
  auto mx = [](std::vector<double>& v) { return v.empty() ? -1.0 : *std::max_element(v.begin(), v.end()); };
  const double e_max = mx(d_entry), end_med = med(d_end), end_max = mx(d_end);
  fprintf(stderr, "  medians: entry %.2f (last %.2f)  entry->first stage %.2f  us/step %.3f  publish %.2f (n=%zu)  combine %.2f (n=%zu, max %.2f)  epilogue %.2f  end %.2f (last %.2f)\n",
          med(d_entry), e_max, med(d_first), med(d_step), med(d_pub), d_pub.size(), med(d_comb), d_comb.size(), mx(d_comb), med(d_epi), end_med, end_max);
}
#endif

template <int WCH, int WPX, int RING, bool ACC = false, int KT = 1>
int launch_cfg(ConvArgs& a, int N, int per_cu, int tiny_grid, hipStream_t s, int sk = 0) {
  constexpr int TN = WCH * 64, TM = WPX * 128;
  constexpr int LDS = RING * (TM + TN) * 64 * KT;
  a.tiles_m = (a.M + TM - 1) / TM;
  a.tiles_n = (N + TN - 1) / TN;
  const long long T = (long long)a.tiles_m * a.tiles_n;
  if (T >= (1 << 30)) return 0;
  long long cap = tiny_grid ? (sk == 2 ? 24 : 8) : 256LL * per_cu;
  if constexpr (!ACC) {
    const long long nkh = (long long)a.ntaps * (a.C / (32 * KT));
    const long long rounds = (T + cap - 1) / cap;
    const double util = (double)T / (double)(rounds * cap);
    const bool want = sk == 2 || (sk == 1 && WCH == 4 && WPX == 2 && T >= 8 && nkh * KT >= 32 && (util < 0.7 || (util < 0.9 && T >= 512) || (nkh * KT >= 128 && T >= 512)));
    long long Gs = cap;
    while (Gs > 8 && (T / 8) * nkh / (Gs / 8) < RING + 1) Gs -= 8;
    if (want && Gs <= SK_MAX_GROUPS && (T / 8) * nkh / (Gs / 8) >= RING + 1 && sk_scratch(s, a, (size_t)Gs * TM * TN * 4)) {
      static PerDeviceOnce attr_set_sk;
      if (auto once_guard = attr_set_sk.first()) {
        (void)hipFuncSetAttribute((const void*)conv_tile_kernel<WCH, WPX, RING, false, true, KT>, hipFuncAttributeMaxDynamicSharedMemorySize, 160 * 1024);
      }
      g_last_conv_kernel += U2_K_STREAMK - U2_K_TILE;
#ifdef U2_TILE_TRACE
      tile_trace_begin((int)Gs, s);
#endif
      hipLaunchKernelGGL((conv_tile_kernel<WCH, WPX, RING, false, true, KT>), dim3((unsigned)Gs), dim3(WCH * WPX * 64), LDS, s, a);
      hipError_t e = hipGetLastError();
      if (e != hipSuccess) return -1000 - (int)e;
#ifdef U2_TILE_TRACE
      tile_trace_end((int)Gs, s, "stream-K");
#endif
      return 1;
    }
  }
  long long G = T < cap ? T : cap;
  G = (G + 7) & ~7LL;
  static PerDeviceOnce attr_set;
  if (auto once_guard = attr_set.first()) {
    (void)hipFuncSetAttribute((const void*)conv_tile_kernel<WCH, WPX, RING, ACC, false, KT>, hipFuncAttributeMaxDynamicSharedMemorySize, 160 * 1024);
  }
#ifdef U2_TILE_TRACE
  tile_trace_begin((int)G, s);
#endif
  hipLaunchKernelGGL((conv_tile_kernel<WCH, WPX, RING, ACC, false, KT>), dim3((unsigned)G), dim3(WCH * WPX * 64), LDS, s, a);
  hipError_t e = hipGetLastError();
  if (e != hipSuccess) return -1000 - (int)e;
#ifdef U2_TILE_TRACE
  tile_trace_end((int)G, s, "whole tiles");
#endif
  return 1;
}

}

int launch_conv_tile(ConvArgs& a, int N, int C, const ConvVariant& v, hipStream_t s) {
  int sel = v.tile_cfg;
  const int tiny = v.tiny;
  const int sk = (int)v.streamk;
  if (sel == U2_CV_TILE_CFG_NEVER) return 0;
  if ((C & 31) || (N & 7) || (a.out_ld & 7) || a.ntaps < 1 || a.M >= (1 << 24) || a.M < 1) return 0;
  if (a.accumulate && (a.stats || a.remap_out || (sel != 0 && sel != 4) || N < 128)) return 0;
  if ((unsigned long long)a.B * a.Hin * a.Win * a.in_ld * 2ull >= 0xffffffffull || (unsigned long long)N * a.wt_taps * C * 2ull >= 0xfffffff0ull) return 0;
  const int nkh = a.ntaps * (C >> 5);
  if (sel == 0) {

    const long long K = (long long)a.ntaps * C;
    if (a.accumulate) sel = 4;
    const long long t256 = (long long)((a.M + 255) / 256) * ((N + 255) / 256);
    if (sel == 4) {
    } else if (N <= 128) {
      if (a.M >= 100000 && !(a.ntaps > 1 && K >= 2048)) sel = 3;
    } else if (a.ntaps > 1) {
      if (t256 >= 2048) sel = 2;
      else if (t256 >= 768) sel = 1;
      else if (t256 >= 180 && t256 <= 256 && K >= 2048) sel = 1;
      else if (t256 > 256 && t256 < 768 && K >= 2048) sel = 1;
      else if (t256 >= 96 && K >= 8192) sel = 1;
      else if (N >= 512 && t256 >= 128 && K >= 4096 && a.M >= 16000) sel = 1;
    } else {
      if (N >= 4096) sel = 1;
      else if (a.M < 10000 && N <= 1024) sel = 0;
      else if (K >= 2048) sel = 2;
      else if (K >= 1024 && N >= 256 && t256 > 256 && t256 < 768) sel = 1;
      else sel = 4;
    }
    if (sel == 0) return 0;
  }
  if (sel > 7) return 0;
  if (sel == 7) {
    if ((C & 63) || a.accumulate) return 0;
    const int nks = a.ntaps * (C >> 6);
    const long long T7 = (long long)((a.M + 255) / 256) * ((N + 255) / 256);
    if (nks * (T7 < 256 ? 1 : T7 / 256) < 3) return 0;
    g_last_conv_kernel = U2_K_TILE + 7;
    return launch_cfg<4, 2, 2, false, 2>(a, N, 1, tiny, s, sk);
  }
  int ring = (sel == 2) ? 5 : (sel == 1 || sel == 5 || sel == 6) ? 4 : 3;
  if (nkh < ring) {
    if (v.tile_cfg != 0) return 0;
    if (a.accumulate && N <= 128) return 0;
    sel = (N <= 128) ? 3 : 4;
    ring = 3;
    const int TN = sel == 3 ? 128 : 256, TM = sel == 3 ? 256 : 128;
    const long long T = (long long)((a.M + TM - 1) / TM) * ((N + TN - 1) / TN);
    const long long min_tiles = (T >> 3) / 64;
    if (nkh * min_tiles < ring) return 0;
  }
  g_last_conv_kernel = U2_K_TILE + sel;
  switch (sel) {
    case 1: return launch_cfg<4, 2, 4>(a, N, 1, tiny, s, sk);
    case 2: return launch_cfg<4, 2, 5>(a, N, 1, tiny, s, sk);
    case 3: return launch_cfg<2, 2, 3>(a, N, 2, tiny, s, sk);
    case 4: return a.accumulate ? launch_cfg<4, 1, 3, true>(a, N, 2, tiny, s) : launch_cfg<4, 1, 3>(a, N, 2, tiny, s, sk);
    case 5: return launch_cfg<2, 2, 4>(a, N, 1, tiny, s);
    case 6: return launch_cfg<1, 4, 4>(a, N, 1, tiny, s);
    default: return 0;
  }
}

}
```

u2seg_amd/layers/deferred.py:

```python
import torch

BN_APPLY = "bn_apply"
ROI_GATHER = "roi_gather"
TAIL = "tail"
KINDS = (BN_APPLY, ROI_GATHER, TAIL)
SLOTS = 64

_entries = {}
_count = dict.fromkeys(KINDS, 0)
_pools = {}


def _key(t):
    return (t.device.index, t.data_ptr())


def post(kind, device, shape, payload):
    pool = _pools.get(device.index)
    if pool is None:
        pool = _pools[device.index] = [torch.zeros(SLOTS, dtype=torch.bfloat16, device=device), 0]
    for _ in range(SLOTS):
        slot = pool[0][pool[1] : pool[1] + 1]
        pool[1] = (pool[1] + 1) % SLOTS
        if _key(slot) not in _entries:
            ph = slot.expand(shape)
            _entries[_key(slot)] = (kind, ph, payload)
            _count[kind] += 1
            return ph
    raise RuntimeError("%d deferred gradients were not consumed by their consumers" % sum(drain().values()))


def holds(kind, grad, posted=None):
    if not _count[kind]:
        return False
    ent = _entries.get(_key(grad))
    return ent is not None and ent[0] == kind and (posted is None or ent[1] is posted)


def take(kind, grad):
    if not _count[kind] or not holds(kind, grad):
        return None
    _count[kind] -= 1
    return _entries.pop(_key(grad))[2]


def pending():
    return dict(_count)


def drain():
    dropped = pending()
    _entries.clear()
    _count.update(dict.fromkeys(KINDS, 0))
    return dropped
```

u2seg_amd/layers/functional.py:

```python
import collections
import ctypes
import math

import functools
import os

import torch
import torch.distributed as dist
from torch.autograd import Function

from .. import _hip
from . import deferred

BF16 = torch.bfloat16


def ceil32(n):
    return (n + 31) // 32 * 32


def _world():
    return dist.get_world_size() if dist.is_available() and dist.is_initialized() else 1


# ... 175 lines not shown


def issue_deferred_piece(n=1):
    while n > 0 and _deferred_pieces:
        _deferred_pieces.pop(0)()
        n -= 1


def flush_deferred():
    issue_deferred_piece(len(_deferred_pieces))


def clear_deferred():
    del _deferred_pieces[:]


def join_all_streams():
    join_wgrad_stream()
    for (dev, _index), s in _aux_streams.items():
        torch.cuda.current_stream(dev).wait_stream(s)


def producer_streams(device):
    device = _cuda_device(device)
    out = [s for dev, s in _side_streams.items() if _cuda_device(dev) == device]
    out += [s for (dev, _index), s in _aux_streams.items() if dev == device]
    return out


def join_wgrad_stream(device=None):
    for dev, s in _side_streams.items():
        if device is None or dev == torch.device(device):
            _side_dirty[dev] = False
            torch.cuda.current_stream(dev).wait_stream(s)


def _run_wgrad(device, operands, launch):
    if not _WGRAD_SIDE:
        launch()
        return
    main = torch.cuda.current_stream(device)
    side = _side_stream(device)
    side.wait_stream(main)
    with torch.cuda.stream(side):
        launch()
    for t in operands:
        t.record_stream(side)
    _side_dirty[device] = True

    def _join():
        if _side_dirty.get(device):
            _side_dirty[device] = False
            torch.cuda.current_stream(device).wait_stream(side)

    torch.autograd.Variable._execution_engine.queue_callback(_join)


_DET_STATS = False


def set_deterministic_stats(on):
    global _DET_STATS
    _DET_STATS = bool(on)


def _fixed_order_stats(out, n):
    o = out[..., :n].float().reshape(-1, n)
    packed = torch.cat([o.sum(0), (o * o).sum(0), o.new_zeros(1)])
    st = packed[: 2 * n].view(2, n)
    st._u2_packed = packed
    return st


def _stats_buffer(n, device):
    packed = zeros_f32((2 * n + 1,), device)
    st = packed[: 2 * n].view(2, n)
    st._u2_packed = packed
    return st


class _Conv2dFn(Function):

    @staticmethod
    def forward(ctx, x, weight, bias, stride, pad, relu, want_stats, param_ref=None, round_bias=True, tail=None):
        _check_act(x)
        ctx.tail = tail
        param = param_ref[0] if param_ref is not None else None
        wgrad_dst = param_ref[1] if param_ref is not None and len(param_ref) > 1 else None
        n, cin, kh, kw = weight.shape
        b, h, w_, cp = x.shape
        assert cin <= cp
        ho = (h + 2 * pad - kh) // stride + 1
        wo = (w_ + 2 * pad - kw) // stride + 1
        npad = ceil32(n)
        wk = weight_fwd_layout(weight, cp, param)
        alloc = torch.zeros if npad != n else torch.empty
        out = alloc((b, ho, wo, npad), dtype=BF16, device=x.device)
        stats = _stats_buffer(n, x.device) if want_stats else None
        bias_f = None
        if bias is not None:
            bias_f = _conv_bias(bias, round_bias)
        ctx.variant = _conv_variant()
        _hip.call("u2_conv_igemm", x, wk, out, bias_f, None if _DET_STATS else stats, b, h, w_, cp, cp, ho, wo, n, npad, kh, kw,
                  pad, pad, stride, 1, int(relu), 0, ctx.variant)
        if want_stats and _DET_STATS:
            stats = _fixed_order_stats(out, n)
        ctx.save_for_backward(x, weight, out if relu else None)
        ctx.cfg = (stride, pad, relu, bias is not None)
        ctx.wgrad_dst = wgrad_dst if (kh * kw == 1 and wgrad_dst is not None) else None
        ctx.arena = None
        if wgrad_dst is not None and wgrad_dst.numel() == weight.numel() and wgrad_dst.is_contiguous():
            ctx.arena = wgrad_dst if tuple(wgrad_dst.shape) == tuple(weight.shape) else wgrad_dst.view(weight.shape)
        ctx.param = param
        bdst = param_ref[2] if param_ref is not None and len(param_ref) > 2 and bias is not None else None
        ctx.bias_dst = bdst if bdst is not None and bdst.is_contiguous() and bdst.dtype == torch.float32 and bdst.numel() == n else None
        ctx.set_materialize_grads(False)
        if want_stats:
            ctx.mark_non_differentiable(stats)
        return out, stats

    @staticmethod
    def backward(ctx, dout, _dstats):
        if dout is None:
            return (None,) * 10
        x, weight, out = ctx.saved_tensors
        stride, pad, relu, has_bias = ctx.cfg
        need_dx, need_dw, need_db = ctx.needs_input_grad[:3]
        geom = (*x.shape, *weight.shape, *dout.shape[1:], stride, pad)
        lazy = deferred.take(deferred.BN_APPLY, dout)
        if lazy is not None:
            dx, dout = _conv_bwd_lazy_bn(ctx, geom, x, weight, *lazy)
            if dx is not None:
                return (dx,) + (None,) * 9
        dout = dout.contiguous()
        dz, bias_done = _conv_bwd_relu(ctx, geom, dout, out) if relu else (dout, False)
        dx, fused = _conv_bwd_data(ctx, geom, x, weight, dz) if need_dx else (None, False)
        dw = _conv_bwd_weight(ctx, geom, x, weight, dz) if need_dw and not fused else None
        db = _conv_bwd_bias(ctx, geom, dz) if has_bias and need_db and not bias_done else None
        return (dx, dw, db) + (None,) * 7


def _conv_bwd_lazy_bn(ctx, geom, x, weight, lz_dz, lz_y, lz_k):
    b, h, w_, cp, n, cin, kh, kw, ho, wo, npad, stride, pad = geom
    m = b * h * w_
    assert not ctx.cfg[2] and not ctx.cfg[3] and kh == 1 and kw == 1 and stride == 1 and pad == 0
    wd = weight_dgrad_layout(weight, cp, npad, ctx.param)
    dx = torch.empty_like(x)
    if ctx.wgrad_dst is not None and ctx.needs_input_grad[0] and ctx.needs_input_grad[1] and _hip.call_status(
            "u2_conv1x1_bwd_fused_bn", x, lz_dz, lz_y, lz_k[2], lz_k[3], lz_k[4], wd, dx, ctx.wgrad_dst, m, cp, cp, npad, npad,
            npad, cp, n, cin, cin, 1, 0) == 0:
        return dx, None
    dout = torch.empty_like(lz_y)
    _hip.call("u2_norm_bwd_apply", lz_dz, None, lz_y, lz_k[2], lz_k[3], lz_k[4], dout, None, 1, m, npad, npad, 0, None, None)
    return None, dout


def _conv_bwd_relu(ctx, geom, dout, out):
    b, h, w_, cp, n, cin, kh, kw, ho, wo, npad, stride, pad = geom
    dz = torch.empty_like(dout)
    if ctx.bias_dst is not None and ctx.needs_input_grad[2]:
        _hip.call("u2_relu_bwd_colsum", dout, out, dz, ctx.bias_dst, zeros_f32((npad,), dout.device), b * ho * wo, npad, npad, n)
        return dz, True
    _hip.call("u2_relu_bwd", dout, out, dz, b * ho * wo * npad)
    return dz, False


def _conv_bwd_data(ctx, geom, x, weight, dz):
    b, h, w_, cp, n, cin, kh, kw, ho, wo, npad, stride, pad = geom
    dst = ctx.wgrad_dst
    if dst is not None and ctx.needs_input_grad[1] and kh == 1 and kw == 1 and stride == 1 and pad == 0 and n > 128 \
            and b * h * w_ >= FUSED_BWD_MIN_PIXELS:
        assert dst.is_contiguous() and dst.dtype == torch.float32 and dst.numel() == n * cin
        wd = weight_dgrad_layout(weight, cp, npad, ctx.param)
        dx = torch.empty_like(x)
        if _hip.call_status("u2_conv1x1_bwd_fused", x, dz, wd, dx, dst, b * h * w_, cp, cp, npad, npad, npad, cp, n, cin, cin, 1,
                            0) == 0:
            return dx, True
    dx = _tail_launch(ctx, geom, dz, x, weight)
    if dx is not None:
        return dx, False
    dx = torch.empty_like(x)
    if ho == 1 and wo == 1 and pad == 0 and h == kh and w_ == kw and kh * kw > 1:
        wt = weight_fc_dgrad_layout(weight, cp, npad, ctx.param)
        _hip.call("u2_conv_igemm", dz, wt, dx, None, None, 1, b, 1, npad, npad, b, 1, kh * kw * cp, kh * kw * cp,
                  1, 1, 0, 0, 1, 1, 0, 0, ctx.variant)
    else:
        wd = weight_dgrad_layout(weight, cp, npad, ctx.param)
        _hip.call("u2_conv_igemm", dz, wd, dx, None, None, b, ho, wo, npad, npad, h, w_, cp, cp, kh, kw,
                  kh - 1 - pad, kw - 1 - pad, 1, stride, 0, 0, ctx.variant)
    return dx, False


def _conv_bwd_weight(ctx, geom, x, weight, dz):
    b, h, w_, cp, n, cin, kh, kw, ho, wo, npad, stride, pad = geom
    dst, arena = ctx.wgrad_dst, ctx.arena

    def scratch():
        dwk = zeros_f32((npad, kh * kw, cp), x.device)
        _hip.call("u2_conv_wgrad", x, dz, dwk, b, h, w_, cp, cp, ho, wo, npad, npad, kh, kw, pad, pad, stride, 0)
        return dwk

    if dst is not None:
        assert dst.is_contiguous() and dst.dtype == torch.float32 and dst.numel() == n * cin

        def launch():
            _hip.call("u2_conv_wgrad_into", x, dz, dst, b, h, w_, cp, cp, ho, wo, npad, npad, kh, kw, pad, pad, stride,
                      n, cin, cin, 1, 1, 0)
    elif arena is not None and _WGRAD_SIDE:
        def launch():
            dwk = scratch()
            if kh * kw * (cp + 1) * 4 <= 64 * 1024 and arena.is_contiguous():
                _hip.call("u2_wgrad_permute_add", dwk, arena, n, cin, kh * kw, cp)
            else:
                arena.add_(dwk[:n, :, :cin].view(n, kh, kw, cin).permute(0, 3, 1, 2))
    else:
        return scratch()[:n, :, :cin].view(n, kh, kw, cin).permute(0, 3, 1, 2)
    _run_wgrad(x.device, (x, dz), launch)
    return None


def _conv_bwd_bias(ctx, geom, dz):
    b, h, w_, cp, n, cin, kh, kw, ho, wo, npad, stride, pad = geom
    if ctx.bias_dst is not None:
        _hip.call("u2_colsum_add", dz, ctx.bias_dst, b * ho * wo, npad, npad, n)
        return None
    sums = zeros_f32((1, 2, npad), dz.device)
    _hip.call("u2_colstats", dz, sums, 1, b * ho * wo, npad, npad)
    return sums[0, 0, :n]


def _tail_launch(ctx, geom, dz, x, weight):
    tail = ctx.tail
    if tail is None or not TAIL_BWD_FUSE or tail.g2 is None or tail.result is not None:
        return None
    b, h, w_, cp, n, cin, kh, kw, ho, wo, npad, stride, pad = geom
    if ctx.cfg[2] or kh != 1 or kw != 1 or stride != 1 or pad != 0 or tuple(tail.g2.shape) != tuple(x.shape) \
            or tuple(tail.y.shape) != tuple(x.shape) or not tail.g2.is_contiguous() or npad != n:
        return None
    wd = weight_dgrad_layout(weight, cp, n, ctx.param)
    dzt = torch.empty_like(tail.y)
    sums = zeros_f32((2, cp), x.device)
    if _hip.call_status("u2_conv_dgrad_tail", dz, wd, tail.g2, tail.y, tail.bits, tail.mean, tail.invstd, dzt, sums, b, h, w_, n, n,
                        cp, cp, ctx.variant) != 0:
        return None
    ph = deferred.post(deferred.TAIL, x.device, x.shape, tail)
    tail.result = (dzt, sums)
    return ph


def _conv_bias(bias, round_bias):
    step_cache = getattr(bias, "_u2_step_bias", None)
    if step_cache is not None and round_bias:
        v = step_cache.get("v")
        if v is None:
            v = step_cache["v"] = bias.detach().bfloat16().float().contiguous()
        return v
    stamp = getattr(bias, "_u2_stamp", None)
    if stamp is None or not round_bias:
        return (bias.detach().bfloat16().float() if round_bias else bias.detach().float()).contiguous()
    ent = bias.__dict__.get("_u2_bias_rounded")
    if ent is None:
        ent = [torch.empty(bias.shape, dtype=torch.float32, device=bias.device), -1, -1]
        bias.__dict__["_u2_bias_rounded"] = ent
        reg = getattr(bias, "_u2_layout_register", None)
        if reg is not None and bias.dim() == 1:
            reg(bias, (bias.numel(), 1, 1, 1, 0, 3), ent)
    if ent[1] != bias._version or ent[2] != stamp[0]:
        ent[0].copy_(bias.detach().bfloat16().float())
        ent[1], ent[2] = bias._version, stamp[0]
    return ent[0]


def grad_slot(param):
    return getattr(param, "_u2_grad", None) if torch.is_grad_enabled() and param.requires_grad else None


def conv2d(x, weight, bias=None, stride=1, pad=0, relu=False, want_stats=False, param=None, round_bias=True):
    if param is None and isinstance(weight, torch.nn.Parameter):
        param = weight
    slot = grad_slot(param) if param is not None else None
    bslot = grad_slot(bias) if isinstance(bias, torch.nn.Parameter) else None
    tail = getattr(x, "_u2_tail", None) if TAIL_BWD_FUSE and torch.is_grad_enabled() else None
    if tail is not None and not (bias is None and not relu and stride == 1 and pad == 0 and tuple(weight.shape[2:]) == (1, 1)
                                 and (weight.shape[0], x.shape[3]) in _TAIL_SHAPES and weight.shape[1] == x.shape[3]
                                 and getattr(x, "_u2_twin", None) is not None):
        tail = None
    out, stats = _Conv2dFn.apply(x, weight, bias, stride, pad, relu, want_stats,
                                 (param, slot, bslot) if param is not None else None, round_bias, tail)
    if LAZY_BN_APPLY and want_stats and slot is not None and bias is None and not relu and stride == 1 and pad == 0 \
            and x.requires_grad and tuple(weight.shape[2:]) == (1, 1) and 128 < weight.shape[0] <= 256 and x.shape[3] <= 64 \
            and x.shape[0] * x.shape[1] * x.shape[2] >= FUSED_BWD_MIN_PIXELS:
        out._u2_lazy_ok = True
    return (out, stats) if want_stats else out


def conv2d_add_(x, weight, bias, out, stride=1, pad=0, relu=False, param=None):
    assert not torch.is_grad_enabled()
    _check_act(x)
    _check_act(out)
    n, cin, kh, kw = weight.shape
    b, h, w_, cp = x.shape
    ho = (h + 2 * pad - kh) // stride + 1
    wo = (w_ + 2 * pad - kw) // stride + 1
    npad = ceil32(n)
    assert tuple(out.shape) == (b, ho, wo, npad) and npad == n, "the accumulating epilogue has no padded output channels"
    wk = weight_fwd_layout(weight, cp, param)
    bias_f = bias.detach().float().contiguous() if bias is not None else None
    _hip.call("u2_conv_igemm", x, wk, out, bias_f, None, b, h, w_, cp, cp, ho, wo, n, npad, kh, kw, pad, pad, stride, 1, int(relu),
              1, _conv_variant())
    return out


def linear(x2d, weight, bias=None, relu=False):
    r, k = x2d.shape
    n = weight.shape[0]
    param = weight if isinstance(weight, torch.nn.Parameter) else None
    out = conv2d(x2d.view(1, r, 1, k), weight.view(n, weight.shape[1], 1, 1), bias, 1, 0, relu, False, param)
    return out.view(r, -1)


class _StemConvFn(Function):

    KP = 160

    @staticmethod
    def forward(ctx, weight, images, pixel_mean, pixel_std, hpad, wpad):
        n = weight.shape[0]
        b = len(images)
        ho, wo = (hpad + 6 - 7) // 2 + 1, (wpad + 6 - 7) // 2 + 1
        kp = _StemConvFn.KP
        col = torch.empty((b * ho * wo, kp), dtype=BF16, device=weight.device)
        is_u8 = images[0].dtype == torch.uint8
        for img in images:
            assert img.is_cuda and img.is_contiguous() and img.shape[0] == 3
            assert img.dtype == (torch.uint8 if is_u8 else torch.float32), "one pixel type per batch"
        ptrs = (ctypes.c_void_p * b)(*[img.data_ptr() for img in images])
        hs = (ctypes.c_int * b)(*[img.shape[1] for img in images])
        ws = (ctypes.c_int * b)(*[img.shape[2] for img in images])
        _hip.call("u2_stem_im2col_batch", ptrs, hs, ws, b, int(is_u8), pixel_mean, pixel_std, col, hpad, wpad, kp)
        wk = torch.zeros((n, 1, kp), dtype=BF16, device=weight.device)
        wk[:, 0, :147] = weight.detach().permute(0, 2, 3, 1).reshape(n, 147)
        out = torch.empty((b, ho, wo, n), dtype=BF16, device=weight.device)
        stats = _stats_buffer(n, weight.device)
        m = b * ho * wo
        _hip.call("u2_conv_igemm", col, wk, out, None, None if _DET_STATS else stats, 1, m, 1, kp, kp, m, 1, n, n, 1, 1, 0, 0, 1,
                  1, 0, 0, 0)
        if _DET_STATS:
            stats = _fixed_order_stats(out, n)
        ctx.save_for_backward(col)
        ctx.n = n
        ctx.mark_non_differentiable(stats)
        return out, stats

    @staticmethod
    def backward(ctx, dout, _ds):
        (col,) = ctx.saved_tensors
        n, kp = ctx.n, _StemConvFn.KP
        dout = dout.contiguous()
        m = col.shape[0]
        dwk = zeros_f32((n, 1, kp), col.device)
        _hip.call("u2_conv_wgrad", col, dout, dwk, 1, m, 1, kp, kp, m, 1, n, n, 1, 1, 0, 0, 1, 0)
        dw = dwk[:, 0, :147].view(n, 7, 7, 3).permute(0, 3, 1, 2)
        return dw, None, None, None, None, None


def stem_conv(weight, images, pixel_mean, pixel_std, hpad, wpad):
    return _StemConvFn.apply(weight, images, pixel_mean, pixel_std, hpad, wpad)


class _BatchNormActFn(Function):

    @staticmethod
    def forward(ctx, y, stats, gamma, beta, running_mean, running_var, residual, relu, momentum, eps, grad_dst=None,
                twin=False, sync=True, res_up=False, lazy_ok=None, tail=None, res_tail=None):
        _check_act(y)
        b, h, w, c = y.shape
        m = b * h * w
        ctx.lazy_ok = lazy_ok
        world = _world() if sync else 1
        count, count_dev = float(m), None
        if world > 1:
            packed = getattr(stats, "_u2_packed", None)
            if packed is None or packed.numel() != 2 * c + 1:
                packed = torch.cat([stats.reshape(-1).float(), stats.new_zeros(1, dtype=torch.float32)])
            packed[2 * c :].fill_(float(m))
            dist.all_reduce(packed)
            stats, count_dev = packed[: 2 * c].view(2, c), packed[2 * c :]
        mean = torch.empty(c, dtype=torch.float32, device=y.device)
        invstd, scale, shift = torch.empty_like(mean), torch.empty_like(mean), torch.empty_like(mean)
        out = torch.empty_like(y)
        bits = None
        if res_up:
            assert residual is not None and not relu and tuple(residual.shape) == (b, h // 2, w // 2, c)
            _hip.call("u2_bn_finalize_fwd", stats, count, count_dev, gamma, beta, running_mean, running_var, momentum, eps, mean,
                      invstd, scale, shift, c)
            _hip.call("u2_affine_upadd", y, scale, shift, residual.contiguous(), out, b, h, w, c, 0)
        else:
            cpr = c // 8
            if relu and residual is not None and c % 8 == 0 and cpr <= 256 and 256 % cpr == 0:
                bits = torch.empty((m, cpr), dtype=torch.uint8, device=y.device)
            _hip.call("u2_bn_act_fused", y, stats, count, count_dev, gamma, beta, running_mean, running_var, momentum, eps, mean,
# ... 591 lines not shown
        gs = [g.contiguous() for g in grads if g is not None]
        if not gs and lazy is None:
            return None, None
        while len(gs) > (2 if lazy is not None else 1):
            part, gs = gs[:4], gs[4:]
            if part[0].dtype != BF16 or part[0].numel() % 8:
                total = part[0]
                for g in part[1:]:
                    total = total + g
            else:
                total = torch.empty_like(part[0])
                part = part + [None] * (4 - len(part))
                _hip.call("u2_add_n", part[0], part[1], part[2], part[3], total, total.numel())
            gs.insert(0, total)
        if lazy is not None:
            shared, level = lazy
            _roi_sets_join(shared["pend"])
            if any(g.dtype != BF16 for g in gs):
                gs = [g.to(BF16) for g in gs]
            out = _roi_gather(shared["shapes"], shared["scales"], shared["pend"], shared["device"], level, gs)[0]
            return out, None
        return gs[0], None


def fan_out(x, k):
    if k <= 1 or not (torch.is_grad_enabled() and x.requires_grad):
        return (x,) * max(k, 1)
    outs = _FanOutFn.apply(x, k)
    for o in outs:
        o._u2_fan = True
    return outs


class RoiGradTap:

    def __init__(self, feats, scales_hint=None):
        self.shapes = [tuple(f.shape) for f in feats]
        self.pending = []
        self.scales = None
        self.ids = None
        self.defer = False


class _RoiGradTapFn(Function):
    @staticmethod
    def forward(ctx, state, *feats):
        ctx.state = state
        ctx.set_materialize_grads(False)
        return tuple(f.detach() for f in feats)

    @staticmethod
    def backward(ctx, *gfeats):
        st = ctx.state
        grads = list(gfeats)
        pend, st.pending = st.pending, []
        if st.defer and ROI_SUM_FOLD and pend and len(pend) <= 4 and all(g is None for g in grads) and pend[0].dout.is_cuda:
            dev = pend[0].dout.device
            shared = {"shapes": st.shapes, "scales": st.scales, "pend": pend, "device": dev}
            return (None, *[deferred.post(deferred.ROI_GATHER, dev, shape, (shared, l)) for l, shape in enumerate(st.shapes)])
        _roi_sets_join(pend)
        for i in range(0, len(pend), 4):
            gbuf = _roi_gather(st.shapes, st.scales, pend[i : i + 4], pend[i].dout.device)
            grads = [g if old is None else old + g for old, g in zip(grads, gbuf)]
        return (None, *grads)


def roi_grad_tap(feats):
    state = RoiGradTap(feats)
    state.defer = all(getattr(f, "_u2_fan", False) for f in feats)
    outs = _RoiGradTapFn.apply(state, *feats)
    state.ids = [id(o) for o in outs]
    for o in outs:
        o._u2_roi_tap = state
    return list(outs)


FUSED_BWD_MIN_PIXELS = int(os.environ.get("U2_FUSED_BWD_MIN_PIXELS", "200000"))
LAZY_BN_APPLY = os.environ.get("U2_LAZY_BN_APPLY", "1") != "0"
ROI_SUM_FOLD = os.environ.get("U2_ROI_SUM_FOLD", "1") != "0"
TAIL_BWD_FUSE = os.environ.get("U2_TAIL_BWD_FUSE", "1") != "0"
_TAIL_SHAPES = ((64, 256), (128, 512), (256, 1024))


def set_tail_bwd_fuse(on):
    global TAIL_BWD_FUSE
    TAIL_BWD_FUSE = bool(on)


class _TailState:
    y = bits = mean = invstd = g2 = result = None


def _tail_take(tail, dout, dout2, dout3, y):
    hits = [i for i, g in enumerate((dout, dout2, dout3)) if g is not None and deferred.holds(deferred.TAIL, g)]
    pending = tail is not None and tail.result is not None
    if not hits and not pending:
        if tail is not None:
            tail.g2 = None
        return None
    posted = deferred.take(deferred.TAIL, dout) if hits == [0] else None
    ok = pending and posted is tail and dout2 is not None and dout3 is None and tail.g2 is not None \
        and dout2.data_ptr() == tail.g2.data_ptr() and tuple(dout2.shape) == tuple(y.shape) and tuple(dout.shape) == tuple(y.shape)
    if not ok:
        n = deferred.drain()[deferred.TAIL] + (1 if posted is not None else 0)
        if tail is not None:
            tail.g2 = tail.result = None
        raise RuntimeError("a residual tail's gradient formed by the next block's conv1 did not arrive as posted (placeholder in "
                           "positions %s, result pending: %s): a further consumer of the block output, or a changed gradient; "
                           "%d deferred tail gradients dropped - set U2_TAIL_BWD_FUSE=0 for such graphs" % (hits, pending, n))
    done = tail.result
    tail.g2 = tail.result = None
    return done


class _LazyLink:
    posted = None


def _lazy_guard(link, grad):
    posted, link.posted = link.posted, None
    if posted is not None and not deferred.holds(deferred.BN_APPLY, grad, posted):
        raise RuntimeError("a convolution output with a deferred batch-norm gradient has a second consumer (autograd summed "
                           "the placeholder with another gradient); %d deferred gradients dropped - set U2_LAZY_BN_APPLY=0 "
                           "for graphs that re-use conv outputs" % sum(deferred.drain().values()))
    return None


def _drain_deferred():
    global _UP2_BWD_LAST
    _UP2_BWD_LAST = None
    return deferred.drain()


def reset_deferred_gradients(strict=True):
    n = sum(_drain_deferred().values())
    if n and strict:
        raise RuntimeError("%d deferred gradients of an earlier backward pass were never consumed" % n)


def assert_no_deferred_gradients():
    left = _drain_deferred()
    if any(left.values()):
        raise RuntimeError("%d deferred batch-norm gradients were not consumed by their convolutions, %d deferred ROIAlign "
                           "gathers not by their fan-out nodes, %d residual-tail gradients not by their tails"
                           % (left[deferred.BN_APPLY], left[deferred.ROI_GATHER], left[deferred.TAIL]))


ROI_ORDER_MIN = int(os.environ.get("U2_ROI_ORDER_MIN", "1000000000"))


def _roi_process_order(rois, levels, nimg, nlevels):
    key = (levels.long() * nimg + rois[:, 0].long()) * 4096 + (rois[:, 2] * (0.25 / 8)).long().clamp_(0, 4095)
    return torch.argsort(key).to(torch.int32)


class _ROIAlignFn(Function):

    @staticmethod
    def forward(ctx, rois, levels, out_size, scales, grad_scale, tap, *feats):
        nl = len(feats)
        for f in feats:
            _check_act(f)
        c = feats[0].shape[3]
        r = rois.shape[0]
        ptrs = (ctypes.c_void_p * nl)(*[f.data_ptr() for f in feats])
        hs, ws, sc = _level_arrays([f.shape for f in feats], scales)
        out = torch.empty((r, out_size, out_size, c), dtype=BF16, device=rois.device)
        order = _roi_process_order(rois, levels, feats[0].shape[0], nl) if r >= ROI_ORDER_MIN else None
        _hip.call("u2_roi_align_fwd", ptrs, hs, ws, sc, nl, rois.contiguous(), levels.contiguous(), order, out, r, c, out_size,
                  out_size)
        ctx.save_for_backward(rois, levels)
        ctx.cfg = (out_size, scales, grad_scale, [tuple(f.shape) for f in feats])
        ctx.tap = tap
        return out

    @staticmethod
    def backward(ctx, dout):
        rois, levels = ctx.saved_tensors
        out_size, scales, grad_scale, shapes = ctx.cfg
        nl = len(shapes)
        b = shapes[0][0]
        r, c = rois.shape[0], shapes[0][3]
        none = (None,) * 6
        if ROI_ALIGN_BWD_ATOMIC:
            hs, ws, sc = _level_arrays(shapes, scales)
            gbuf = [torch.zeros(s, dtype=torch.float32, device=dout.device) for s in shapes]
            ptrs = (ctypes.c_void_p * nl)(*[g.data_ptr() for g in gbuf])
            _hip.call("u2_roi_align_bwd", ptrs, hs, ws, sc, nl, rois.contiguous(), levels.contiguous(), dout.contiguous(),
                      r, c, out_size, out_size, float(grad_scale))
            return (*none, *[g.to(BF16) for g in gbuf])
        order, seg = _roi_group(rois, levels, b, nl)
        entry = _RoiSet(rois, order, seg, dout, out_size, grad_scale)
        tap = ctx.tap
        if tap is not None:
            tap.scales = scales
            if dout.is_cuda:
                ev = torch.cuda.Event()
                ev.record()
                entry = entry._replace(event=ev)
            tap.pending.append(entry)
            return (*none, *([None] * nl))
        return (*none, *_roi_gather(shapes, scales, [entry], dout.device))


ROI_ALIGN_BWD_ATOMIC = False


def roi_align(feats, rois, levels, out_size, scales, grad_scale=1.0):
    tap = getattr(feats[0], "_u2_roi_tap", None)
    if tap is not None and (ROI_ALIGN_BWD_ATOMIC or tap.ids != [id(f) for f in feats]):
        tap = None
    return _ROIAlignFn.apply(rois, levels, out_size, tuple(scales), grad_scale, tap, *feats)


def assign_levels(boxes, min_level, max_level, canonical_size=224, canonical_level=4):
    n = boxes.shape[0]
    lv = torch.empty(n, dtype=torch.int32, device=boxes.device)
    _hip.call("u2_assign_levels", boxes.contiguous(), lv, n, min_level, max_level, float(canonical_size), canonical_level)
    return lv


def mask_crop(masks_u8, rois, size):
    r = rois.shape[0]
    out = torch.empty((r, size, size), dtype=torch.uint8, device=rois.device)
    _hip.call("u2_mask_crop", masks_u8.contiguous(), rois.contiguous(), out, r, masks_u8.shape[1], masks_u8.shape[2], size)
    return out


# ... 176 lines not shown
```

u2seg_amd/modeling/roi_heads.py:

```python
import contextlib
import math

import os

import torch
from torch import nn

from ..config import configurable
from ..layers import Conv2d, ConvTranspose2d, Linear, ShapeSpec, c2_msra_fill, c2_xavier_fill
from ..layers import functional as F
from ..structures import BitMasks, Boxes, Instances
from ..utils.events import MASK_SLOT as _MASK_SLOT
from ..utils.events import get_event_storage, has_event_storage
from ..utils.events import stage_counters as _stage_counters
from ..utils.events import step_counters as _step_counters
from ..utils.registry import Registry
from .batched import BatchList, PaddedTargets, check_finite, device_constant, device_upload, image_index, proposals_from_list
from .sampling import subsample_labels

ROI_HEADS_REGISTRY = Registry("ROI_HEADS")
ROI_BOX_HEAD_REGISTRY = Registry("ROI_BOX_HEAD")
ROI_MASK_HEAD_REGISTRY = Registry("ROI_MASK_HEAD")

_SCALE_CLAMP = math.log(1000.0 / 16)


class ROIPooler(nn.Module):

    def __init__(self, output_size, scales, sampling_ratio, pooler_type="ROIAlignV2", canonical_box_size=224,
                 canonical_level=4):
        super().__init__()
        assert pooler_type == "ROIAlignV2" and sampling_ratio == 0
        self.output_size = output_size if isinstance(output_size, int) else output_size[0]
        self.scales = tuple(scales)
        min_level = -(math.log2(scales[0]))
        max_level = -(math.log2(scales[-1]))
        assert math.isclose(min_level, int(min_level)) and math.isclose(max_level, int(max_level))
        self.min_level, self.max_level = int(min_level), int(max_level)
        assert len(scales) == self.max_level - self.min_level + 1
        self.canonical_level, self.canonical_box_size = canonical_level, canonical_box_size

    def forward(self, x, box_lists, grad_scale=1.0):
        dev = x[0].device
        if isinstance(box_lists, torch.Tensor):
            nb, ns = box_lists.shape[:2]
            boxes = box_lists.reshape(-1, 4)
            idx = torch.arange(nb, device=dev, dtype=torch.float32)[:, None].expand(nb, ns).reshape(-1)
        else:
            sizes = [len(b) for b in box_lists]
            boxes = torch.cat([b.tensor for b in box_lists], dim=0)
            idx = image_index(sizes, dev)
        rois = torch.cat([idx[:, None], boxes], dim=1).contiguous()
        if len(self.scales) == 1:
            levels = torch.zeros(rois.shape[0], dtype=torch.int32, device=dev)
        else:
            levels = F.assign_levels(boxes, self.min_level, self.max_level, self.canonical_box_size, self.canonical_level)
        if rois.shape[0] == 0:
            return torch.zeros((0, self.output_size, self.output_size, x[0].shape[3]), dtype=x[0].dtype, device=dev)
        return F.roi_align(x, rois, levels, self.output_size, self.scales, grad_scale)


@ROI_BOX_HEAD_REGISTRY.register()
class FastRCNNConvFCHead(nn.Module):

    @configurable
    def __init__(self, input_shape, *, conv_dims, fc_dims, conv_norm=""):
        super().__init__()
        assert len(conv_dims) == 0 and len(fc_dims) > 0 and conv_norm == ""
        self._in = (input_shape.channels, input_shape.height, input_shape.width)
        self.fcs = []
        dim = input_shape.channels * input_shape.height * input_shape.width
        for k, fc_dim in enumerate(fc_dims):
            fc = Linear(dim, fc_dim)
            self.add_module("fc{}".format(k + 1), fc)
            self.fcs.append(fc)
            dim = fc_dim
        self._out_dim = dim
        for layer in self.fcs:
            c2_xavier_fill(layer)

    @classmethod
    def from_config(cls, cfg, input_shape):
        num_conv, conv_dim = cfg.MODEL.ROI_BOX_HEAD.NUM_CONV, cfg.MODEL.ROI_BOX_HEAD.CONV_DIM
        num_fc, fc_dim = cfg.MODEL.ROI_BOX_HEAD.NUM_FC, cfg.MODEL.ROI_BOX_HEAD.FC_DIM
        return {"input_shape": input_shape, "conv_dims": [conv_dim] * num_conv, "fc_dims": [fc_dim] * num_fc,
                "conv_norm": cfg.MODEL.ROI_BOX_HEAD.NORM}

    def forward(self, x):
        c, h, w = self._in
        fc1 = self.fcs[0]
        y = F.conv2d(x, fc1.weight.view(fc1.out_features, c, h, w), fc1.bias, 1, 0, relu=True, param=fc1.weight)
        y = y.view(y.shape[0], -1)
        for fc in self.fcs[1:]:
            y = fc(y, relu=True)
        return y

    @property
    def output_shape(self):
        return ShapeSpec(channels=self._out_dim)


def build_box_head(cfg, input_shape):
    return ROI_BOX_HEAD_REGISTRY.get(cfg.MODEL.ROI_BOX_HEAD.NAME)(cfg, input_shape)


class FastRCNNOutputLayers(nn.Module):

    @configurable
    def __init__(self, input_shape, *, box2box_weights, num_classes, test_score_thresh=0.0, test_nms_thresh=0.5,
                 test_topk_per_image=100, cls_agnostic_bbox_reg=False, smooth_l1_beta=0.0,
                 box_reg_loss_type="smooth_l1", loss_weight=1.0):
        super().__init__()
        if isinstance(input_shape, int):
            input_shape = ShapeSpec(channels=input_shape)
        self.num_classes = num_classes
        input_size = input_shape.channels * (input_shape.width or 1) * (input_shape.height or 1)
        self.cls_score = Linear(input_size, num_classes + 1)
        num_bbox_reg_classes = 1 if cls_agnostic_bbox_reg else num_classes
        assert cls_agnostic_bbox_reg, "the U2Seg configs use class-agnostic box regression"
        self.bbox_pred = Linear(input_size, num_bbox_reg_classes * 4)
        nn.init.normal_(self.cls_score.weight, std=0.01)
        nn.init.normal_(self.bbox_pred.weight, std=0.001)
        for layer in [self.cls_score, self.bbox_pred]:
            nn.init.constant_(layer.bias, 0)
        self.box2box_weights = tuple(box2box_weights)
        assert box_reg_loss_type == "smooth_l1" and smooth_l1_beta == 0.0
        self.test_score_thresh, self.test_nms_thresh = test_score_thresh, test_nms_thresh
        self.test_topk_per_image = test_topk_per_image
        if isinstance(loss_weight, float):
            loss_weight = {"loss_cls": loss_weight, "loss_box_reg": loss_weight}
        self.loss_weight = loss_weight

    @classmethod
    def from_config(cls, cfg, input_shape):
        return {
            "input_shape": input_shape,
            "box2box_weights": cfg.MODEL.ROI_BOX_HEAD.BBOX_REG_WEIGHTS,
            "num_classes": cfg.MODEL.ROI_HEADS.NUM_CLASSES,
            "cls_agnostic_bbox_reg": cfg.MODEL.ROI_BOX_HEAD.CLS_AGNOSTIC_BBOX_REG,
            "smooth_l1_beta": cfg.MODEL.ROI_BOX_HEAD.SMOOTH_L1_BETA,
            "test_score_thresh": cfg.MODEL.ROI_HEADS.SCORE_THRESH_TEST,
            "test_nms_thresh": cfg.MODEL.ROI_HEADS.NMS_THRESH_TEST,
            "test_topk_per_image": cfg.TEST.DETECTIONS_PER_IMAGE,
            "box_reg_loss_type": cfg.MODEL.ROI_BOX_HEAD.BBOX_REG_LOSS_TYPE,
            "loss_weight": {"loss_box_reg": cfg.MODEL.ROI_BOX_HEAD.BBOX_REG_LOSS_WEIGHT},
        }

    def forward(self, x):
        return self.cls_score(x), self.bbox_pred(x)

    def losses(self, predictions, proposals):
        scores, deltas = predictions
        if isinstance(proposals, BatchList) and proposals.stacked and proposals.gt_boxes is not None:
            gt_classes = proposals.gt_classes.reshape(-1)
            proposal_boxes, gt_boxes = proposals.boxes.reshape(-1, 4), proposals.gt_boxes.reshape(-1, 4)
        else:
            gt_classes = torch.cat([p.gt_classes for p in proposals], dim=0) if len(proposals) else torch.empty(0)
            proposal_boxes = torch.cat([p.proposal_boxes.tensor for p in proposals], dim=0)
            gt_boxes = torch.cat([(p.gt_boxes if p.has("gt_boxes") else p.proposal_boxes).tensor for p in proposals], dim=0)
        r = gt_classes.numel()
        if r == 0:
            z = scores.float().sum() * 0.0
            return {"loss_cls": z, "loss_box_reg": deltas.float().sum() * 0.0}
        loss_cls = F.softmax_cross_entropy(scores, gt_classes, self.num_classes + 1, _stage_counters())
        loss_box = F.box_reg_l1_loss(deltas, proposal_boxes, gt_boxes, gt_classes, self.num_classes,
                                     self.box2box_weights, max(r, 1.0))
        losses = {"loss_cls": loss_cls, "loss_box_reg": loss_box}
        return {k: v * self.loss_weight.get(k, 1.0) for k, v in losses.items()}

    def predict_boxes(self, predictions, proposals, stacked=False):
        _, deltas = predictions
        num_prop = [len(p) for p in proposals]
        if isinstance(proposals, BatchList) and proposals.stacked:
            proposal_boxes = proposals.boxes.reshape(-1, 4)
        else:
# ... 556 lines not shown
```

Measured before the change: 285.6.

## Fuse ReLU backward gating and bias-grad column sums into consumer conv dgrad epilogue

Adds a gated variant of the implicit-GEMM and stream conv kernels. The data-gradient output of a consumer conv is masked by the producer's ReLU output (gate > 0), and the bias-gradient column sums are accumulated in the same epilogue. The Python side tracks the producer/consumer pair and posts the already-gated gradient as a deferred result, so the producer's backward skips its separate ReLU-backward and bias-reduction pass. The aim is to save a full read/write of the activation gradient. In exchange it adds template instantiations, extra gate loads and atomics in the epilogue, and graph bookkeeping that raises an error if a conv output has more than one consumer.

Measured after the change: 287.5 (median of 2 runs). Within noise of the previous version (+0.7%).

```diff
diff --git a/include/u2seg_hip.h b/include/u2seg_hip.h
--- a/include/u2seg_hip.h
+++ b/include/u2seg_hip.h
@@ -111,6 +111,10 @@
 int u2_conv_dgrad_tail(const void* in, const void* wt, const void* dout2, const void* y, const void* bits, const float* mean,
                        const float* invstd, void* dz, float* sums, int B, int H, int W, int C, int in_ld, int N, int out_ld,
                        int variant, void* stream);
+
+int u2_conv_igemm_gated(const void* in, const void* wt, void* out, const void* gate, int gate_ld, float* colsum_dst, int n_sum,
+                        int B, int Hin, int Win, int C, int in_ld, int Hout, int Wout, int N, int out_ld, int KH, int KW,
+                        int pad_h, int pad_w, int mul, int div, int accumulate, int variant, void* stream);
 
 int u2_conv_last_kernel(void);
 
diff --git a/u2seg_amd/csrc/common.h b/u2seg_amd/csrc/common.h
--- a/u2seg_amd/csrc/common.h
+++ b/u2seg_amd/csrc/common.h
@@ -147,7 +147,25 @@
     atomicAdd(stats + N + st_n, q);
   }
 }
-
+template <int NW>
+__device__ __forceinline__ void wg_flush_column_sum1(float* dst, int n_sum, int st_n, float st_s, int w, int lane,
+                                                     unsigned char* smem) {
+  __syncthreads();
+  int* rn = reinterpret_cast<int*>(smem);
+  float* rs = reinterpret_cast<float*>(smem) + NW * 64;
+  rn[w * 64 + lane] = st_n;
+  rs[w * 64 + lane] = st_s;
+  __syncthreads();
+  bool lead = st_n >= 0 && st_n < n_sum;
+  float s = 0.f;
+#pragma unroll
+  for (int k = 0; k < NW; ++k) {
+    const bool same = rn[k * 64 + lane] == st_n;
+    if (same && k < w) lead = false;
+    s += same ? rs[k * 64 + lane] : 0.f;
+  }
+  if (lead) atomicAdd(dst + st_n, s);
+}
 
 __device__ __forceinline__ int xcd_remap(int bid, int nwg) {
   const int q = nwg >> 3, r = nwg & 7;
diff --git a/u2seg_amd/csrc/conv_args.h b/u2seg_amd/csrc/conv_args.h
--- a/u2seg_amd/csrc/conv_args.h
+++ b/u2seg_amd/csrc/conv_args.h
@@ -25,7 +25,16 @@
   float* sk_ws;
   int* sk_flags;
   int abl;
+  const bf16_t* gate;
+  float* colsum;
+  int gate_ld, n_sum;
 };
+
+constexpr int U2_LAUNCH_NO_GATE = 2;
+
+__device__ __forceinline__ uint32_t gate_keep_mask(uint32_t g) {
+  return (__uint_as_float(g << 16) > 0.f ? 0xffffu : 0u) | (__uint_as_float(g & 0xffff0000u) > 0.f ? 0xffff0000u : 0u);
+}
 
 
 template <int BK> __device__ __forceinline__ int swz(int row);
diff --git a/u2seg_amd/csrc/conv_halo.hip b/u2seg_amd/csrc/conv_halo.hip
--- a/u2seg_amd/csrc/conv_halo.hip
+++ b/u2seg_amd/csrc/conv_halo.hip
@@ -334,6 +334,7 @@
     if (tiles < 512) return 0;
     if (!(fill >= 0.88 || (N <= 128 && fill >= 0.70))) return 0;
   }
+  if (a.gate) return U2_LAUNCH_NO_GATE;
   const int tiny = v.tiny;
   if (N <= 64 && !v.halo_tile128) {
     g_last_conv_kernel = U2_K_HALO_N64;
diff --git a/u2seg_amd/csrc/conv_igemm.hip b/u2seg_amd/csrc/conv_igemm.hip
--- a/u2seg_amd/csrc/conv_igemm.hip
+++ b/u2seg_amd/csrc/conv_igemm.hip
@@ -9,7 +9,7 @@
 using namespace u2conv;
 namespace {
 
-template <int BK, bool GLDS, int TM, int TN, int NST>
+template <int BK, bool GLDS, int TM, int TN, int NST, bool GATE = false>
 __global__ __launch_bounds__((TM / 64) * (TN / 64) * 64, 2) void conv_igemm_kernel(const ConvArgs a) {
   constexpr int NW = (TM / 64) * (TN / 64);
   constexpr int NT = NW * 64;
@@ -259,6 +259,15 @@
         ss[e] += f * f;
       }
     }
+    if constexpr (GATE) {
+      if (n0 + cchunk * 8 >= a.N) continue;
+      const uint4 g = *reinterpret_cast<const uint4*>(a.gate + (size_t)m * a.gate_ld + n0 + cchunk * 8);
+      uint4 v8 = *reinterpret_cast<const uint4*>(e8);
+      v8.x &= gate_keep_mask(g.x); v8.y &= gate_keep_mask(g.y); v8.z &= gate_keep_mask(g.z); v8.w &= gate_keep_mask(g.w);
+      *reinterpret_cast<uint4*>(e8) = v8;
+#pragma unroll
+      for (int e = 0; e < 8; ++e) s[e] += bf2f(e8[e]);
+    }
     if (vec_ok) {
       if (nt_out) {
         typedef __attribute__((ext_vector_type(4))) unsigned int u32x4_t;
@@ -300,6 +309,25 @@
       }
       atomicAdd(a.stats + n0 + tid, t0);
       atomicAdd(a.stats + a.N + n0 + tid, t1);
+    }
+  }
+  if constexpr (GATE) {
+    if (a.n_sum > 0) {
+#pragma unroll
+      for (int e = 0; e < 8; ++e)
+#pragma unroll
+        for (int o = CPO; o < 64; o <<= 1) s[e] += __shfl_xor(s[e], o, 64);
+      if (lane < CPO) {
+#pragma unroll
+        for (int e = 0; e < 8; ++e) red[w * TN + lane * 8 + e] = s[e];
+      }
+      __syncthreads();
+      if (tid < TN && n0 + tid < a.n_sum) {
+        float t0 = 0.f;
+#pragma unroll
+        for (int ww = 0; ww < NW; ++ww) t0 += red[ww * TN + tid];
+        atomicAdd(a.colsum + n0 + tid, t0);
+      }
     }
   }
 }
@@ -1165,27 +1193,33 @@
   return e ? (int)strtol(e, nullptr, 0) : 0;
 }
 
+constexpr int GATE_DECLINED = -7777;
+
 int launch_conv(ConvArgs& a, int N, int C, int variant, hipStream_t s) {
   const ConvVariant v = decode_conv_variant((unsigned)env_variant("U2_CONV_VARIANT", variant));
   a.abl = v.abl;
   {
     const int rc = launch_conv_stream(a, N, C, v, s);
     if (rc == 1) return 0;
+    if (rc == U2_LAUNCH_NO_GATE) return GATE_DECLINED;
     if (rc < 0) return rc;
   }
   {
     const int rc = launch_conv_halo(a, N, C, v, s);
     if (rc == 1) return 0;
+    if (rc == U2_LAUNCH_NO_GATE) return GATE_DECLINED;
     if (rc < 0) return rc;
   }
   {
     const int rc = launch_conv_tile(a, N, C, v, s);
     if (rc == 1) return 0;
+    if (rc == U2_LAUNCH_NO_GATE) return GATE_DECLINED;
     if (rc < 0) return rc;
   }
   const bool wide_ok = !a.remap_out && C % 64 == 0 && a.ntaps * (C / 32) >= 4;
   const bool wide_auto = N % 256 == 0 && a.ntaps * C >= 1024 && (long long)a.M * N >= 256LL * 256 * 512;
   if (wide_ok && v.wide != Choice::Never && (v.wide == Choice::Force || wide_auto)) {
+    if (a.gate) return GATE_DECLINED;
     a.tiles_m = (a.M + 255) / 256;
     a.tiles_n = (N + 255) / 256;
     static PerDeviceOnce attr_set;
@@ -1219,22 +1253,26 @@
   const size_t epi = (size_t)TM * (TN + 8) * 2 + 2 * 8 * TN * 4;
   if (lds < epi) lds = epi;
   if (lds > 160 * 1024) return -3;
-#define U2_LAUNCH_CONV(BK_, GL_, TM_, TN_, NST_)                                                                 \
+  if (a.gate && (!glds || v.ring != 0 || a.remap_out)) return GATE_DECLINED;
+#define U2_LAUNCH_CONV(BK_, GL_, TM_, TN_, NST_, GATE_)                                                          \
   do {                                                                                                           \
     g_last_conv_kernel = U2_K_IGEMM + BK_ * 10000 + (TM_ / 64) * 1000 + (TN_ / 64) * 100 + NST_ * 10 + (GL_ ? 1 : 0); \
     static PerDeviceOnce attr_set;                                                                                \
     if (auto once_guard = attr_set.first()) {                                                                                             \
-      (void)hipFuncSetAttribute((const void*)conv_igemm_kernel<BK_, GL_, TM_, TN_, NST_>,                        \
+      (void)hipFuncSetAttribute((const void*)conv_igemm_kernel<BK_, GL_, TM_, TN_, NST_, GATE_>,                 \
                                 hipFuncAttributeMaxDynamicSharedMemorySize, 160 * 1024);                         \
     }                                                                                                            \
-    hipLaunchKernelGGL((conv_igemm_kernel<BK_, GL_, TM_, TN_, NST_>), grid, block, lds, s, a);                   \
+    hipLaunchKernelGGL((conv_igemm_kernel<BK_, GL_, TM_, TN_, NST_, GATE_>), grid, block, lds, s, a);            \
   } while (0)
 #define U2_PICK_NST(BK_, TM_, TN_)                                                                               \
   do {                                                                                                           \
-    if (!glds) U2_LAUNCH_CONV(BK_, false, TM_, TN_, 2);                                                          \
-    else if (nst == 2) U2_LAUNCH_CONV(BK_, true, TM_, TN_, 2);                                                   \
-    else if (nst == 3) U2_LAUNCH_CONV(BK_, true, TM_, TN_, 3);                                                   \
-    else U2_LAUNCH_CONV(BK_, true, TM_, TN_, 4);                                                                 \
+    if (a.gate) {                                                                                                \
+      if (nst == 2) U2_LAUNCH_CONV(BK_, true, TM_, TN_, 2, true);                                                \
+      else U2_LAUNCH_CONV(BK_, true, TM_, TN_, 4, true);                                                         \
+    } else if (!glds) U2_LAUNCH_CONV(BK_, false, TM_, TN_, 2, false);                                            \
+    else if (nst == 2) U2_LAUNCH_CONV(BK_, true, TM_, TN_, 2, false);                                            \
+    else if (nst == 3) U2_LAUNCH_CONV(BK_, true, TM_, TN_, 3, false);                                            \
+    else U2_LAUNCH_CONV(BK_, true, TM_, TN_, 4, false);                                                          \
   } while (0)
   if (narrow) {
     if (bk == 64) U2_PICK_NST(64, 256, 64); else U2_PICK_NST(32, 256, 64);
@@ -1263,16 +1301,22 @@
   }
 }
 
-}
-
-extern "C" int u2_conv_igemm(const void* in, const void* wt, void* out, const float* bias, float* stats,
-                             int B, int Hin, int Win, int C, int in_ld, int Hout, int Wout, int N, int out_ld,
-                             int KH, int KW, int pad_h, int pad_w, int mul, int div, int relu, int accumulate,
-                             int variant, void* stream) {
+
+struct GateArgs {
+  const bf16_t* gate = nullptr;
+  float* colsum = nullptr;
+  int gate_ld = 0, n_sum = 0;
+};
+
+int conv_igemm_entry(const void* in, const void* wt, void* out, const float* bias, float* stats,
+                     int B, int Hin, int Win, int C, int in_ld, int Hout, int Wout, int N, int out_ld,
+                     int KH, int KW, int pad_h, int pad_w, int mul, int div, int relu, int accumulate,
+                     int variant, void* stream, const GateArgs& g) {
   if (C % 32 != 0 || (in_ld & 7) != 0 || KH * KW > 64 || (div > 1 && mul != 1)) return -1;
   if (B <= 0 || Hout <= 0 || Wout <= 0 || N <= 0) return 0;
   ConvArgs a;
   a.in = (const bf16_t*)in; a.wt = (const bf16_t*)wt; a.out = (bf16_t*)out; a.bias = bias; a.stats = stats;
+  a.gate = g.gate; a.colsum = g.colsum; a.gate_ld = g.gate_ld; a.n_sum = g.n_sum;
   a.zero = zero_page_ptr();
   if (!a.zero) return -2;
   a.abl = 0; a.stagger_by_parity = 0; a.sk_ws = nullptr; a.sk_flags = nullptr;
@@ -1338,6 +1382,30 @@
     }
   return 0;
 }
+}
+
+extern "C" int u2_conv_igemm(const void* in, const void* wt, void* out, const float* bias, float* stats,
+                             int B, int Hin, int Win, int C, int in_ld, int Hout, int Wout, int N, int out_ld,
+                             int KH, int KW, int pad_h, int pad_w, int mul, int div, int relu, int accumulate,
+                             int variant, void* stream) {
+  return conv_igemm_entry(in, wt, out, bias, stats, B, Hin, Win, C, in_ld, Hout, Wout, N, out_ld, KH, KW, pad_h, pad_w, mul, div,
+                          relu, accumulate, variant, stream, GateArgs{});
+}
+
+extern "C" int u2_conv_igemm_gated(const void* in, const void* wt, void* out, const void* gate, int gate_ld, float* colsum_dst,
+                                   int n_sum, int B, int Hin, int Win, int C, int in_ld, int Hout, int Wout, int N, int out_ld,
+                                   int KH, int KW, int pad_h, int pad_w, int mul, int div, int accumulate, int variant,
+                                   void* stream) {
+  if (!gate || n_sum < 0 || n_sum > N || (colsum_dst && n_sum < 1)) return -1;
+  if (C % 32 != 0 || (in_ld & 7) != 0 || KH * KW > 64 || (div > 1 && mul != 1)) return -1;
+  if (B <= 0 || Hout <= 0 || Wout <= 0 || N <= 0) return 1;
+  if (div > 1 || (N & 7) || (out_ld & 7) || (gate_ld & 7) || gate_ld < N || ((size_t)gate & 15) || ((size_t)out & 15)) return 1;
+  GateArgs g;
+  g.gate = (const bf16_t*)gate; g.colsum = colsum_dst; g.gate_ld = gate_ld; g.n_sum = colsum_dst ? n_sum : 0;
+  const int rc = conv_igemm_entry(in, wt, out, nullptr, nullptr, B, Hin, Win, C, in_ld, Hout, Wout, N, out_ld, KH, KW, pad_h, pad_w,
+                                  mul, div, 0, accumulate, variant, stream, g);
+  return rc == GATE_DECLINED ? 1 : rc;
+}
 
 extern "C" int u2_conv_dgrad_tail(const void* in, const void* wt, const void* dout2, const void* y, const void* bits,
                                   const float* mean, const float* invstd, void* dz, float* sums, int B, int H, int W, int C,
@@ -1345,6 +1413,7 @@
   if (B <= 0 || H <= 0 || W <= 0 || N <= 0 || C <= 0) return 1;
   ConvArgs a;
   a.in = (const bf16_t*)in; a.wt = (const bf16_t*)wt; a.out = (bf16_t*)dz; a.bias = nullptr; a.stats = sums;
+  a.gate = nullptr; a.colsum = nullptr; a.gate_ld = 0; a.n_sum = 0;
   a.zero = zero_page_ptr();
   if (!a.zero) return -2;
   a.abl = 0; a.stagger_by_parity = 0; a.sk_ws = nullptr; a.sk_flags = nullptr;
diff --git a/u2seg_amd/csrc/conv_stream.hip b/u2seg_amd/csrc/conv_stream.hip
--- a/u2seg_amd/csrc/conv_stream.hip
+++ b/u2seg_amd/csrc/conv_stream.hip
@@ -48,7 +48,7 @@
   u32x2_t mk;
 };
 
-template <int KS, int TM, int PSW, int NWV, int KSS = KS, bool TAIL = false>
+template <int KS, int TM, int PSW, int NWV, int KSS = KS, bool TAIL = false, bool GATE = false>
 __global__ __launch_bounds__(NWV * 64, 2) void conv_stream_kernel(const ConvArgs a, int ring, const TailArgs t) {
   constexpr int RB = KSS * 64, CPR = KSS * 4, STAGE = TM * RB;
   constexpr int RPP = 16 / KSS;
@@ -58,6 +58,7 @@
   constexpr int CBW = NWV / PSW, WPX = TM / PSW, NF = WPX / 16;
   static_assert(PT % NWV == 0 && PPW >= 1 && PPW <= 8 && NF >= 1 && (KSS == 1 || KSS == 2 || KSS == 4 || KSS == 8) && KS % KSS == 0 && (S & (S - 1)) == 0, "unsupported configuration");
   static_assert(!TAIL || (S == 1 && NF % 2 == 0), "the tail epilogue takes whole tiles per step and batches of 1, 2 or 4 rows");
+  static_assert(!GATE || (!TAIL && NF % 4 == 0), "the gated epilogue takes batches of four rows");
   extern __shared__ __attribute__((aligned(16))) unsigned char smem[];
   const int tid = threadIdx.x, lane = tid & 63;
   const int w = __builtin_amdgcn_readfirstlane(tid >> 6);
@@ -270,6 +271,61 @@
     st_ss += row16_transpose_sum(ss, fr);
   };
 
+  auto gate_epilogue = [&](int ti) {
+    const int m0 = (first_tile + ti * nwalk) * TM + psw * WPX;
+    uint32_t g1p[NF][8];
+#pragma unroll
+    for (int j = 0; j < NF; ++j)
+#pragma unroll
+      for (int i = 0; i < 4; ++i) {
+        g1p[j][2 * i] = pack_bf16(acc[i][j][0], acc[i][j][1]);
+        g1p[j][2 * i + 1] = pack_bf16(acc[i][j][2], acc[i][j][3]);
+      }
+#pragma unroll
+    for (int j = 0; j < NF; ++j)
+      asm volatile("" : "+v"(g1p[j][0]), "+v"(g1p[j][1]), "+v"(g1p[j][2]), "+v"(g1p[j][3]), "+v"(g1p[j][4]), "+v"(g1p[j][5]),
+                        "+v"(g1p[j][6]), "+v"(g1p[j][7]));
+    float s[16];
+#pragma unroll
+    for (int e = 0; e < 16; ++e) s[e] = 0.f;
+#pragma unroll
+    for (int b = 0; b < NF / 4; ++b) {
+      u32x4_t ga[4], gb[4];
+#pragma unroll
+      for (int jj = 0; jj < 4; ++jj) {
+        const int mm = m0 + (4 * b + jj) * 16 + fr;
+        ga[jj] = u32x4_t{0u, 0u, 0u, 0u};
+        gb[jj] = u32x4_t{0u, 0u, 0u, 0u};
+        if (mm < a.M) {
+          const bf16_t* gsrc = a.gate + (size_t)mm * a.gate_ld + nb;
+          if (okA) asm volatile("global_load_dwordx4 %0, %1, off" : "=&v"(ga[jj]) : "v"(gsrc) : "memory");
+          if (okB) asm volatile("global_load_dwordx4 %0, %1, off offset:64" : "=&v"(gb[jj]) : "v"(gsrc) : "memory");
+        }
+      }
+      asm volatile("s_waitcnt vmcnt(0)"
+                   : "+v"(ga[0]), "+v"(ga[1]), "+v"(ga[2]), "+v"(ga[3]), "+v"(gb[0]), "+v"(gb[1]), "+v"(gb[2]), "+v"(gb[3])::"memory");
+#pragma unroll
+      for (int jj = 0; jj < 4; ++jj) {
+        const int j = 4 * b + jj;
+        const int m = m0 + j * 16 + fr;
+        if (m < a.M) {
+          uint32_t pk[8];
+#pragma unroll
+          for (int e = 0; e < 8; ++e) {
+            pk[e] = g1p[j][e] & gate_keep_mask(e < 4 ? ga[jj][e & 3] : gb[jj][e & 3]);
+            s[2 * e] += __uint_as_float(pk[e] << 16);
+            s[2 * e + 1] += __uint_as_float(pk[e] & 0xffff0000u);
+          }
+          bf16_t* dst = a.out + (size_t)m * a.out_ld + nb;
+          const u32x4_t va = {pk[0], pk[1], pk[2], pk[3]}, vb = {pk[4], pk[5], pk[6], pk[7]};
+          if (okA) asm volatile("global_store_dwordx4 %0, %1, off\n\ts_nop 1" ::"v"(dst), "v"(va) : "memory");
+          if (okB) asm volatile("global_store_dwordx4 %0, %1, off offset:64\n\ts_nop 1" ::"v"(dst), "v"(vb) : "memory");
+        }
+      }
+    }
+    if (a.n_sum > 0) st_s += row16_transpose_sum(s, fr);
+  };
+
   const int G = my_tiles * S;
   for (int sl = 0; sl < ring - 1 && sl < G; ++sl) issue(sl, sl);
   int slot = 0, g = 0;
@@ -338,12 +394,16 @@
     slot = slot + 1 == ring ? 0 : slot + 1;
    }
     if constexpr (TAIL) tail_epilogue(ti, g + ring - 2 < G);
+    else if constexpr (GATE) gate_epilogue(ti);
     else if (!(a.abl & 4)) epilogue(ti);
   }
   if (do_stats) wg_flush_column_sums<NWV>(a.stats, a.N, st_n, st_s, st_ss, w, lane, smem);
-}
-
-template <int KS, int TM, int PSW, int NWV, int KSS = KS, bool TAIL = false>
+  if constexpr (GATE) {
+    if (a.n_sum > 0) wg_flush_column_sum1<NWV>(a.colsum, a.n_sum, st_n, st_s, w, lane, smem);
+  }
+}
+
+template <int KS, int TM, int PSW, int NWV, int KSS = KS, bool TAIL = false, bool GATE = false>
 int launch_stream_cfg(ConvArgs& a, int N, int tiny, int forced, int code, hipStream_t s, const TailArgs& t = TailArgs{}) {
   constexpr int CBW = NWV / PSW;
   constexpr int STAGE = TM * KSS * 64;
@@ -357,12 +417,13 @@
   long long G = tiny ? 8LL * a.tiles_n : 256LL * per_cu;
   if ((G >> 3) < a.tiles_n) return 0;
   if (!forced && !tiny && (long long)a.tiles_m * a.tiles_n < 6 * G) return 0;
+  if (a.gate && !GATE) return U2_LAUNCH_NO_GATE;
   static PerDeviceOnce attr_set;
   if (auto once_guard = attr_set.first()) {
-    (void)hipFuncSetAttribute((const void*)conv_stream_kernel<KS, TM, PSW, NWV, KSS, TAIL>, hipFuncAttributeMaxDynamicSharedMemorySize, 160 * 1024);
+    (void)hipFuncSetAttribute((const void*)conv_stream_kernel<KS, TM, PSW, NWV, KSS, TAIL, GATE>, hipFuncAttributeMaxDynamicSharedMemorySize, 160 * 1024);
   }
   g_last_conv_kernel = code;
-  hipLaunchKernelGGL((conv_stream_kernel<KS, TM, PSW, NWV, KSS, TAIL>), dim3((unsigned)G), dim3(NWV * 64), (size_t)ring * STAGE, s, a, ring, t);
+  hipLaunchKernelGGL((conv_stream_kernel<KS, TM, PSW, NWV, KSS, TAIL, GATE>), dim3((unsigned)G), dim3(NWV * 64), (size_t)ring * STAGE, s, a, ring, t);
   hipError_t e = hipGetLastError();
   if (e != hipSuccess) return -1000 - (int)e;
   return 1;
@@ -401,6 +462,7 @@
     if (N > 64) return launch_stream_cfg<4, 64, 2, 4>(a, N, tiny, forced, code + 1, s);
     return launch_stream_cfg<4, 64, 4, 4>(a, N, tiny, forced, code + 2, s);
   }
+  if (N > 128 && a.gate) return launch_stream_cfg<1, 128, 1, 4, 1, false, true>(a, N, tiny, forced, code, s);
   if (N > 128) return launch_stream_cfg<1, 128, 1, 4>(a, N, tiny, forced, code, s);
   if (N > 64) return launch_stream_cfg<1, 128, 2, 4>(a, N, tiny, forced, code + 1, s);
   return launch_stream_cfg<1, 128, 4, 4>(a, N, tiny, forced, code + 2, s);
diff --git a/u2seg_amd/csrc/conv_tile.hip b/u2seg_amd/csrc/conv_tile.hip
--- a/u2seg_amd/csrc/conv_tile.hip
+++ b/u2seg_amd/csrc/conv_tile.hip
@@ -49,8 +49,9 @@
 #ifndef U2_TILE_PINGPONG
 #define U2_TILE_PINGPONG 0
 #endif
-template <int WCH, int WPX, int RING, bool ACC = false, bool SK = false, int KT = 1>
+template <int WCH, int WPX, int RING, bool ACC = false, bool SK = false, int KT = 1, bool GATE = false>
 __global__ __launch_bounds__(WCH * WPX * 64, 2) void conv_tile_kernel(const ConvArgs a) {
+  static_assert(!(GATE && SK), "the stream-K owner epilogue has no gated form");
   constexpr int NW = WCH * WPX, NT = NW * 64;
   constexpr int TN = WCH * 64, TM = WPX * 128;
   constexpr int KU = 32 * KT;
@@ -338,6 +339,89 @@
       if (n_here != st_n) { stats_flush(); st_n = n_here; }
       st_s += row16_transpose_sum(s, fr);
       st_ss += row16_transpose_sum(ss, fr);
+    }
+  };
+
+  auto gate_flush = [&]() {
+    if (st_n >= 0 && st_n < a.n_sum) asm volatile("global_atomic_add_f32 %0, %1, off\n\ts_nop 1" ::"v"(a.colsum + st_n), "v"(st_s) : "memory");
+    st_s = 0.f;
+  };
+  auto gate_epilogue = [&](int tile) {
+    typedef __attribute__((ext_vector_type(4))) unsigned int u32x4_t;
+    const int tile_m = tile / a.tiles_n, tile_n = tile - tile_m * a.tiles_n;
+    const int m0 = tile_m * TM + wc * 128;
+    const int nb = tile_n * TN + wr * 64 + fg * 8;
+    const bool okA = nb < a.N, okB = nb + 32 < a.N;
+    uint32_t g1p[8][8];
+#pragma unroll
+    for (int j = 0; j < 8; ++j)
+#pragma unroll
+      for (int i = 0; i < 4; ++i) {
+        g1p[j][2 * i] = pack_bf16(acc[i][j][0], acc[i][j][1]);
+        g1p[j][2 * i + 1] = pack_bf16(acc[i][j][2], acc[i][j][3]);
+      }
+#pragma unroll
+    for (int j = 0; j < 8; ++j)
+      asm volatile("" : "+v"(g1p[j][0]), "+v"(g1p[j][1]), "+v"(g1p[j][2]), "+v"(g1p[j][3]), "+v"(g1p[j][4]), "+v"(g1p[j][5]),
+                        "+v"(g1p[j][6]), "+v"(g1p[j][7]));
+    float s[16];
+#pragma unroll
+    for (int e = 0; e < 16; ++e) s[e] = 0.f;
+#pragma unroll
+    for (int b = 0; b < 2; ++b) {
+      u32x4_t ga[4], gb[4], olda[4], oldb[4];
+#pragma unroll
+      for (int jj = 0; jj < 4; ++jj) {
+        const int mm = m0 + (4 * b + jj) * 16 + fr;
+        ga[jj] = u32x4_t{0u, 0u, 0u, 0u};
+        gb[jj] = u32x4_t{0u, 0u, 0u, 0u};
+        olda[jj] = u32x4_t{0u, 0u, 0u, 0u};
+        oldb[jj] = u32x4_t{0u, 0u, 0u, 0u};
+        if (mm < a.M) {
+          const bf16_t* gsrc = a.gate + (size_t)mm * a.gate_ld + nb;
+          if (okA) asm volatile("global_load_dwordx4 %0, %1, off" : "=&v"(ga[jj]) : "v"(gsrc) : "memory");
+          if (okB) asm volatile("global_load_dwordx4 %0, %1, off offset:64" : "=&v"(gb[jj]) : "v"(gsrc) : "memory");
+          if constexpr (ACC) {
+            const bf16_t* osrc = a.out + (size_t)mm * a.out_ld + nb;
+            if (okA) asm volatile("global_load_dwordx4 %0, %1, off" : "=&v"(olda[jj]) : "v"(osrc) : "memory");
+            if (okB) asm volatile("global_load_dwordx4 %0, %1, off offset:64" : "=&v"(oldb[jj]) : "v"(osrc) : "memory");
+          }
+        }
+      }
+      asm volatile("s_waitcnt vmcnt(0)"
+                   : "+v"(ga[0]), "+v"(ga[1]), "+v"(ga[2]), "+v"(ga[3]), "+v"(gb[0]), "+v"(gb[1]), "+v"(gb[2]), "+v"(gb[3])::"memory");
+      if constexpr (ACC)
+        asm volatile("" : "+v"(olda[0]), "+v"(olda[1]), "+v"(olda[2]), "+v"(olda[3]), "+v"(oldb[0]), "+v"(oldb[1]), "+v"(oldb[2]),
+                          "+v"(oldb[3])::"memory");
+#pragma unroll
+      for (int jj = 0; jj < 4; ++jj) {
+        const int j = 4 * b + jj;
+        const int m = m0 + j * 16 + fr;
+        if (m < a.M) {
+          uint32_t pk[8];
+#pragma unroll
+          for (int e = 0; e < 8; ++e) {
+            pk[e] = g1p[j][e];
+            if constexpr (ACC) {
+              const uint32_t o = e < 4 ? olda[jj][e & 3] : oldb[jj][e & 3];
+              pk[e] = pack_bf16(__uint_as_float(pk[e] << 16) + __uint_as_float(o << 16),
+                                __uint_as_float(pk[e] & 0xffff0000u) + __uint_as_float(o & 0xffff0000u));
+            }
+            pk[e] &= gate_keep_mask(e < 4 ? ga[jj][e & 3] : gb[jj][e & 3]);
+            s[2 * e] += __uint_as_float(pk[e] << 16);
+            s[2 * e + 1] += __uint_as_float(pk[e] & 0xffff0000u);
+          }
+          bf16_t* dst = a.out + (size_t)m * a.out_ld + nb;
+          const u32x4_t va = {pk[0], pk[1], pk[2], pk[3]}, vb = {pk[4], pk[5], pk[6], pk[7]};
+          if (okA) asm volatile("global_store_dwordx4 %0, %1, off\n\ts_nop 1" ::"v"(dst), "v"(va) : "memory");
+          if (okB) asm volatile("global_store_dwordx4 %0, %1, off offset:64\n\ts_nop 1" ::"v"(dst), "v"(vb) : "memory");
+        }
+      }
+    }
+    if (a.n_sum > 0) {
+      const int n_here = tile_n * TN + wr * 64 + fg * 8 + (fr >> 3) * 32 + (fr & 7);
+      if (n_here != st_n) { gate_flush(); st_n = n_here; }
+      st_s += row16_transpose_sum(s, fr);
     }
   };
 
@@ -616,7 +700,8 @@
       if (h_begin > 0) { U2_STAMP(48); sk_publish(); U2_STAMP(49); continue; }
       if (h_end < nkh) break;
     }
-    epilogue(first_tile + ti * tstep);
+    if constexpr (GATE) gate_epilogue(first_tile + ti * tstep);
+    else epilogue(first_tile + ti * tstep);
   }
   if constexpr (SK) {
     if (sk_k1 < nkh && !(my_tiles == 1 && sk_k0 > 0)) {
@@ -628,6 +713,9 @@
     }
   }
   if (!ACC && a.stats) wg_flush_column_sums<NW>(a.stats, a.N, st_n, st_s, st_ss, w, lane, smem);
+  if constexpr (GATE) {
+    if (a.n_sum > 0) wg_flush_column_sum1<NW>(a.colsum, a.n_sum, st_n, st_s, w, lane, smem);
+  }
   U2_STAMP(54);
 #undef U2_T_MFMA
 }
@@ -739,7 +827,7 @@
 }
 #endif
 
-template <int WCH, int WPX, int RING, bool ACC = false, int KT = 1>
+template <int WCH, int WPX, int RING, bool ACC = false, int KT = 1, bool GATE = false>
 int launch_cfg(ConvArgs& a, int N, int per_cu, int tiny_grid, hipStream_t s, int sk = 0) {
   constexpr int TN = WCH * 64, TM = WPX * 128;
   constexpr int LDS = RING * (TM + TN) * 64 * KT;
@@ -755,7 +843,9 @@
     const bool want = sk == 2 || (sk == 1 && WCH == 4 && WPX == 2 && T >= 8 && nkh * KT >= 32 && (util < 0.7 || (util < 0.9 && T >= 512) || (nkh * KT >= 128 && T >= 512)));
     long long Gs = cap;
     while (Gs > 8 && (T / 8) * nkh / (Gs / 8) < RING + 1) Gs -= 8;
-    if (want && Gs <= SK_MAX_GROUPS && (T / 8) * nkh / (Gs / 8) >= RING + 1 && sk_scratch(s, a, (size_t)Gs * TM * TN * 4)) {
+    const bool sk_fits = want && Gs <= SK_MAX_GROUPS && (T / 8) * nkh / (Gs / 8) >= RING + 1;
+    if (GATE && sk_fits) return U2_LAUNCH_NO_GATE;
+    if (!GATE && sk_fits && sk_scratch(s, a, (size_t)Gs * TM * TN * 4)) {
       static PerDeviceOnce attr_set_sk;
       if (auto once_guard = attr_set_sk.first()) {
         (void)hipFuncSetAttribute((const void*)conv_tile_kernel<WCH, WPX, RING, false, true, KT>, hipFuncAttributeMaxDynamicSharedMemorySize, 160 * 1024);
@@ -777,12 +867,12 @@
   G = (G + 7) & ~7LL;
   static PerDeviceOnce attr_set;
   if (auto once_guard = attr_set.first()) {
-    (void)hipFuncSetAttribute((const void*)conv_tile_kernel<WCH, WPX, RING, ACC, false, KT>, hipFuncAttributeMaxDynamicSharedMemorySize, 160 * 1024);
+    (void)hipFuncSetAttribute((const void*)conv_tile_kernel<WCH, WPX, RING, ACC, false, KT, GATE>, hipFuncAttributeMaxDynamicSharedMemorySize, 160 * 1024);
   }
 #ifdef U2_TILE_TRACE
   tile_trace_begin((int)G, s);
 #endif
-  hipLaunchKernelGGL((conv_tile_kernel<WCH, WPX, RING, ACC, false, KT>), dim3((unsigned)G), dim3(WCH * WPX * 64), LDS, s, a);
+  hipLaunchKernelGGL((conv_tile_kernel<WCH, WPX, RING, ACC, false, KT, GATE>), dim3((unsigned)G), dim3(WCH * WPX * 64), LDS, s, a);
   hipError_t e = hipGetLastError();
   if (e != hipSuccess) return -1000 - (int)e;
 #ifdef U2_TILE_TRACE
@@ -832,6 +922,7 @@
     const int nks = a.ntaps * (C >> 6);
     const long long T7 = (long long)((a.M + 255) / 256) * ((N + 255) / 256);
     if (nks * (T7 < 256 ? 1 : T7 / 256) < 3) return 0;
+    if (a.gate) return U2_LAUNCH_NO_GATE;
     g_last_conv_kernel = U2_K_TILE + 7;
     return launch_cfg<4, 2, 2, false, 2>(a, N, 1, tiny, s, sk);
   }
@@ -847,6 +938,14 @@
     if (nkh * min_tiles < ring) return 0;
   }
   g_last_conv_kernel = U2_K_TILE + sel;
+  if (a.gate) {
+    if (a.remap_out) return U2_LAUNCH_NO_GATE;
+    switch (sel) {
+      case 1: return launch_cfg<4, 2, 4, false, 1, true>(a, N, 1, tiny, s, sk);
+      case 4: return a.accumulate ? launch_cfg<4, 1, 3, true, 1, true>(a, N, 2, tiny, s) : launch_cfg<4, 1, 3, false, 1, true>(a, N, 2, tiny, s, sk);
+      default: return U2_LAUNCH_NO_GATE;
+    }
+  }
   switch (sel) {
     case 1: return launch_cfg<4, 2, 4>(a, N, 1, tiny, s, sk);
     case 2: return launch_cfg<4, 2, 5>(a, N, 1, tiny, s, sk);
diff --git a/u2seg_amd/layers/deferred.py b/u2seg_amd/layers/deferred.py
--- a/u2seg_amd/layers/deferred.py
+++ b/u2seg_amd/layers/deferred.py
@@ -3,7 +3,9 @@
 BN_APPLY = "bn_apply"
 ROI_GATHER = "roi_gather"
 TAIL = "tail"
-KINDS = (BN_APPLY, ROI_GATHER, TAIL)
+RELU_GATE = "relu_gate"
+KINDS = (BN_APPLY, ROI_GATHER, TAIL, RELU_GATE)
+_BASE_KINDS = 3
 SLOTS = 64
 
 _entries = {}
@@ -45,7 +47,7 @@
 
 
 def pending():
-    return dict(_count)
+    return {k: n for i, (k, n) in enumerate(_count.items()) if i < _BASE_KINDS or n}
 
 
 def drain():
diff --git a/u2seg_amd/layers/functional.py b/u2seg_amd/layers/functional.py
--- a/u2seg_amd/layers/functional.py
+++ b/u2seg_amd/layers/functional.py
@@ -281,9 +281,11 @@
 class _Conv2dFn(Function):
 
     @staticmethod
-    def forward(ctx, x, weight, bias, stride, pad, relu, want_stats, param_ref=None, round_bias=True, tail=None):
+    def forward(ctx, x, weight, bias, stride, pad, relu, want_stats, param_ref=None, round_bias=True, tail=None, gate_in=None,
+                gate_out=None):
         _check_act(x)
         ctx.tail = tail
+        ctx.gate_in, ctx.gate_out = gate_in, gate_out
         param = param_ref[0] if param_ref is not None else None
         wgrad_dst = param_ref[1] if param_ref is not None and len(param_ref) > 1 else None
         n, cin, kh, kw = weight.shape
@@ -313,6 +315,8 @@
         ctx.param = param
         bdst = param_ref[2] if param_ref is not None and len(param_ref) > 2 and bias is not None else None
         ctx.bias_dst = bdst if bdst is not None and bdst.is_contiguous() and bdst.dtype == torch.float32 and bdst.numel() == n else None
+        if gate_out is not None:
+            gate_out.bias_dst, gate_out.n = ctx.bias_dst, n
         ctx.set_materialize_grads(False)
         if want_stats:
             ctx.mark_non_differentiable(stats)
@@ -321,7 +325,7 @@
     @staticmethod
     def backward(ctx, dout, _dstats):
         if dout is None:
-            return (None,) * 10
+            return (None,) * 12
         x, weight, out = ctx.saved_tensors
         stride, pad, relu, has_bias = ctx.cfg
         need_dx, need_dw, need_db = ctx.needs_input_grad[:3]
@@ -330,13 +334,17 @@
         if lazy is not None:
             dx, dout = _conv_bwd_lazy_bn(ctx, geom, x, weight, *lazy)
             if dx is not None:
-                return (dx,) + (None,) * 9
-        dout = dout.contiguous()
-        dz, bias_done = _conv_bwd_relu(ctx, geom, dout, out) if relu else (dout, False)
+                return (dx,) + (None,) * 11
+        dz = _gate_take(ctx.gate_out, dout)
+        if dz is not None:
+            bias_done = True
+        else:
+            dout = dout.contiguous()
+            dz, bias_done = _conv_bwd_relu(ctx, geom, dout, out) if relu else (dout, False)
         dx, fused = _conv_bwd_data(ctx, geom, x, weight, dz) if need_dx else (None, False)
         dw = _conv_bwd_weight(ctx, geom, x, weight, dz) if need_dw and not fused else None
         db = _conv_bwd_bias(ctx, geom, dz) if has_bias and need_db and not bias_done else None
-        return (dx, dw, db) + (None,) * 7
+        return (dx, dw, db) + (None,) * 9
 
 
 def _conv_bwd_lazy_bn(ctx, geom, x, weight, lz_dz, lz_y, lz_k):
@@ -385,6 +393,13 @@
                   1, 1, 0, 0, 1, 1, 0, 0, ctx.variant)
     else:
         wd = weight_dgrad_layout(weight, cp, npad, ctx.param)
+        g = ctx.gate_in
+        if g is not None and RELU_GATE_FUSE and g.consumers == 1 and g.result is None and g.bias_dst is not None and g.n <= cp \
+                and x.is_contiguous() and _hip.call_status(
+                    "u2_conv_igemm_gated", dz, wd, dx, x, cp, g.bias_dst, g.n, b, ho, wo, npad, npad, h, w_, cp, cp, kh, kw,
+                    kh - 1 - pad, kw - 1 - pad, 1, stride, 0, ctx.variant) == 0:
+            g.result = dx
+            return deferred.post(deferred.RELU_GATE, x.device, x.shape, g), False
         _hip.call("u2_conv_igemm", dz, wd, dx, None, None, b, ho, wo, npad, npad, h, w_, cp, cp, kh, kw,
                   kh - 1 - pad, kw - 1 - pad, 1, stride, 0, 0, ctx.variant)
     return dx, False
@@ -484,8 +499,17 @@
                                  and (weight.shape[0], x.shape[3]) in _TAIL_SHAPES and weight.shape[1] == x.shape[3]
                                  and getattr(x, "_u2_twin", None) is not None):
         tail = None
+    gate_in = gate_out = None
+    if RELU_GATE_FUSE and torch.is_grad_enabled():
+        gate_in = getattr(x, "_u2_gate", None)
+        if gate_in is not None:
+            gate_in.consumers += 1
+        if relu and bslot is not None and not want_stats:
+            gate_out = _GateState()
     out, stats = _Conv2dFn.apply(x, weight, bias, stride, pad, relu, want_stats,
-                                 (param, slot, bslot) if param is not None else None, round_bias, tail)
+                                 (param, slot, bslot) if param is not None else None, round_bias, tail, gate_in, gate_out)
+    if gate_out is not None and gate_out.bias_dst is not None and out.requires_grad:
+        out._u2_gate = gate_out
     if LAZY_BN_APPLY and want_stats and slot is not None and bias is None and not relu and stride == 1 and pad == 0 \
             and x.requires_grad and tuple(weight.shape[2:]) == (1, 1) and 128 < weight.shape[0] <= 256 and x.shape[3] <= 64 \
             and x.shape[0] * x.shape[1] * x.shape[2] >= FUSED_BWD_MIN_PIXELS:
@@ -514,8 +538,8 @@
     r, k = x2d.shape
     n = weight.shape[0]
     param = weight if isinstance(weight, torch.nn.Parameter) else None
-    out = conv2d(x2d.view(1, r, 1, k), weight.view(n, weight.shape[1], 1, 1), bias, 1, 0, relu, False, param)
-    return out.view(r, -1)
+    out = conv2d(keep_gate_mark(x2d, x2d.view(1, r, 1, k)), weight.view(n, weight.shape[1], 1, 1), bias, 1, 0, relu, False, param)
+    return keep_gate_mark(out, out.view(r, -1))
 
 
 class _StemConvFn(Function):
@@ -1273,6 +1297,42 @@
 _TAIL_SHAPES = ((64, 256), (128, 512), (256, 1024))
 
 
+RELU_GATE_FUSE = os.environ.get("U2_RELU_GATE_FUSE", "1") != "0"
+
+
+def set_relu_gate_fuse(on):
+    global RELU_GATE_FUSE
+    RELU_GATE_FUSE = bool(on)
+
+
+class _GateState:
+    bias_dst = result = None
+    n = consumers = 0
+
+
+def keep_gate_mark(src, view):
+    g = getattr(src, "_u2_gate", None)
+    if g is not None and view.shape[-1] == src.shape[-1] and view.data_ptr() == src.data_ptr():
+        view._u2_gate = g
+    return view
+
+
+def _gate_take(gate, dout):
+    posted = deferred.take(deferred.RELU_GATE, dout)
+    pending = gate is not None and gate.result is not None
+    if posted is None and not pending:
+        return None
+    if not (pending and posted is gate and gate.result.numel() == dout.numel() and gate.result.shape[-1] == dout.shape[-1]):
+        n = deferred.drain().get(deferred.RELU_GATE, 0) + (1 if posted is not None else 0)
+        if gate is not None:
+            gate.result = None
+        raise RuntimeError("a ReLU gradient formed by the consumer's data gradient did not arrive as posted (result pending: %s): "
+                           "a further consumer of the conv output, or a changed gradient; %d deferred gated gradients dropped - "
+                           "set U2_RELU_GATE_FUSE=0 for such graphs" % (pending, n))
+    dz, gate.result = gate.result.view(dout.shape), None
+    return dz
+
+
 def set_tail_bwd_fuse(on):
     global TAIL_BWD_FUSE
     TAIL_BWD_FUSE = bool(on)
@@ -1333,8 +1393,10 @@
     left = _drain_deferred()
     if any(left.values()):
         raise RuntimeError("%d deferred batch-norm gradients were not consumed by their convolutions, %d deferred ROIAlign "
-                           "gathers not by their fan-out nodes, %d residual-tail gradients not by their tails"
-                           % (left[deferred.BN_APPLY], left[deferred.ROI_GATHER], left[deferred.TAIL]))
+                           "gathers not by their fan-out nodes, %d residual-tail gradients not by their tails, %d gated ReLU "
+                           "gradients not by their convolutions"
+                           % (left[deferred.BN_APPLY], left[deferred.ROI_GATHER], left[deferred.TAIL],
+                              left.get(deferred.RELU_GATE, 0)))
 
 
 ROI_ORDER_MIN = int(os.environ.get("U2_ROI_ORDER_MIN", "1000000000"))
diff --git a/u2seg_amd/modeling/roi_heads.py b/u2seg_amd/modeling/roi_heads.py
--- a/u2seg_amd/modeling/roi_heads.py
+++ b/u2seg_amd/modeling/roi_heads.py
@@ -90,7 +90,7 @@
         c, h, w = self._in
         fc1 = self.fcs[0]
         y = F.conv2d(x, fc1.weight.view(fc1.out_features, c, h, w), fc1.bias, 1, 0, relu=True, param=fc1.weight)
-        y = y.view(y.shape[0], -1)
+        y = F.keep_gate_mark(y, y.view(y.shape[0], -1))
         for fc in self.fcs[1:]:
             y = fc(y, relu=True)
         return y
```
